# reedrosenbluth/LASS

Hardware: AMD Instinct MI355X
Metric: clips/sec (10s@16kHz) (higher is better)
Workload: dtype f32; 1 GPU; ResUNet30 separate() fp32, batch=16/GPU, 10s@16kHz clips, fixed precomputed condition embedding, seeded random-init weights (BASELINE configs[1]); samples_per_clip=160000, parallelism=clip-sharded x1

## Files before the change

### include/lass_hip.h

```cpp
#ifndef LASS_HIP_H
#define LASS_HIP_H

#include <stddef.h>
#include <stdint.h>

#ifdef __cplusplus
extern "C" {
#endif

typedef struct lass_ctx lass_ctx;

#define LASS_OK 0
#define LASS_ERR_ARG (-1)
#define LASS_ERR_HIP (-2)
#define LASS_ERR_STATE (-3)
#define LASS_ERR_WORKSPACE (-4)

#define LASS_F32 0
#define LASS_I64 1

#define LASS_COMPUTE_F32 0
#define LASS_COMPUTE_BF16 1
#define LASS_COMPUTE_BF16X3 2

int lass_version(void);

int lass_create(lass_ctx** out, int device_id);
int lass_create_multistft(lass_ctx** out, int device_id, int n_fft, int n_windows, const int* win_lengths,
                          int mask_window);
int lass_destroy(lass_ctx* ctx);

const char* lass_last_error(const lass_ctx* ctx);

int lass_set_param(lass_ctx* ctx, const char* name, const void* data, const int64_t* shape, int ndim, int dtype);

int lass_finalize(lass_ctx* ctx, int compute_mode);

int lass_workspace_bytes(const lass_ctx* ctx, int B, int L, size_t* bytes);

int lass_separate(lass_ctx* ctx, const float* mixture, const float* condition, float* out, int B, int L,
                  void* workspace, size_t workspace_bytes, void* stream);

int lass_graph_stats(const lass_ctx* ctx, long* captures, long* replays);
int lass_set_graph_replay(lass_ctx* ctx, int enabled);

int lass_separate_components(lass_ctx* ctx, const float* const* mag, const float* cos_mask, const float* sin_mask,
                             const float* condition, float* out, int B, int L, void* workspace, size_t workspace_bytes,
                             void* stream);


int lass_stft_magphase(lass_ctx* ctx, const float* wav, int B, int L, float* mag, float* cos_out, float* sin_out,
                       float* real_out, float* imag_out, void* stream);

int lass_multi_stft(lass_ctx* ctx, const float* wav, int B, int L, int hop, int n_windows, const int* win_lengths,
                    float* const* mag, float* const* cos_out, float* const* sin_out, void* stream);

int lass_stft_components(lass_ctx* ctx, const float* wav, int B, int L, int n_fft, int hop, int n_windows,
                         const int* win_lengths, float* const* mag, float* const* cos_out, float* const* sin_out,
                         void* stream);

int lass_istft(lass_ctx* ctx, const float* real, const float* imag, int B, int T, int L, float* wav,
               float* frames_ws, void* stream);
int lass_istft_nfft(lass_ctx* ctx, const float* real, const float* imag, int B, int T, int L, int n_fft, int win_length,
                    float* wav, void* stream);

int lass_film(lass_ctx* ctx, const float* condition, int B, float* shift, void* stream);
int lass_film_width(const lass_ctx* ctx);
int lass_film_offset(const lass_ctx* ctx, const char* site);
int lass_film_raw(lass_ctx* ctx, const float* condition, int B, float* film, void* stream);

int lass_convblock(lass_ctx* ctx, const char* prefix, const float* x, int B, int H, int W, const float* shift,
                   float* y, float* scratch, void* stream);

int lass_encoder_block(lass_ctx* ctx, const char* name, const float* x, int B, int H, int W, const float* shift, float* y,
                       float* pool, float* scratch, void* stream);

int lass_front_end(lass_ctx* ctx, const float* wav, int B, int L, float* mag, float* cos_out, float* sin_out, float* x0,
                   void* stream);

int lass_workspace_tensor(const lass_ctx* ctx, int B, int L, const char* name, size_t* offset, int64_t shape[4],
                          int64_t strides[4]);

int lass_upconv(lass_ctx* ctx, const char* name, const float* x, int B, int h, int w, const float* shift, float* y,
                void* stream);

int lass_mask_apply(lass_ctx* ctx, const float* x12, const float* mag, const float* cos_in, const float* sin_in,
                    int B, int T, int Tpad, float* out_real, float* out_imag, void* stream);

int lass_sdr_stats(lass_ctx* ctx, const float* ref, const float* est, int B, int L, double* stats, void* stream);

int lass_mix_at_snr(lass_ctx* ctx, float* source, const float* noise, const float* snr_db, float* mixture, int B, int L,
                    double* scratch, void* stream);

int lass_segment_mix(lass_ctx* ctx, const float* waveforms, int B, int L, const int* mix_num, const float* comp_db, int max_comp,
                     const float* noise_db, float* mixture, float* segment, double* scratch, void* stream);


typedef struct lass_text_ctx lass_text_ctx;

int lass_text_create(lass_text_ctx** out, int device_id);
int lass_text_destroy(lass_text_ctx* ctx);
const char* lass_text_last_error(const lass_text_ctx* ctx);
int lass_text_set_param(lass_text_ctx* ctx, const char* name, const void* data, const int64_t* shape, int ndim);
int lass_text_finalize(lass_text_ctx* ctx);
int lass_text_layers(const lass_text_ctx* ctx);
int lass_text_workspace_bytes(const lass_text_ctx* ctx, int N, int S, size_t* bytes);
int lass_text_encode(lass_text_ctx* ctx, const int64_t* input_ids, const int64_t* attention_mask, int N, int S,
                     float* out, float* pooler_out, void* workspace, size_t workspace_bytes, void* stream);


int lass_set_profiling(lass_ctx* ctx, int enabled);
int lass_profile_count(const lass_ctx* ctx);
int lass_profile_get(lass_ctx* ctx, int i, const char** name, double* ms, int* launches);
int lass_profile_reset(lass_ctx* ctx);

#ifdef __cplusplus
}
#endif
#endif
```

### lass_amd/_lib.py

```python
from __future__ import annotations

import ctypes
import os
from ctypes import POINTER, c_char_p, c_double, c_int, c_int64, c_long, c_size_t, c_void_p

_HERE = os.path.dirname(os.path.abspath(__file__))
LIB_PATH = os.environ.get("LASS_HIP_LIB") or os.path.join(_HERE, "csrc", "liblass_hip.so")

_lib = None

SYMBOLS = [
    ("lass_version", c_int, []),
    ("lass_create", c_int, [POINTER(c_void_p), c_int]),
    ("lass_create_multistft", c_int, [POINTER(c_void_p), c_int, c_int, c_int, POINTER(c_int), c_int]),
    ("lass_destroy", c_int, [c_void_p]),
    ("lass_last_error", c_char_p, [c_void_p]),
    ("lass_set_param", c_int, [c_void_p, c_char_p, c_void_p, POINTER(c_int64), c_int, c_int]),
    ("lass_finalize", c_int, [c_void_p, c_int]),
    ("lass_workspace_bytes", c_int, [c_void_p, c_int, c_int, POINTER(c_size_t)]),
    ("lass_separate", c_int, [c_void_p, c_void_p, c_void_p, c_void_p, c_int, c_int, c_void_p, c_size_t, c_void_p]),
    ("lass_stft_magphase", c_int, [c_void_p, c_void_p, c_int, c_int, c_void_p, c_void_p, c_void_p, c_void_p,
                                   c_void_p, c_void_p]),
    ("lass_mix_at_snr", c_int, [c_void_p, c_void_p, c_void_p, c_void_p, c_void_p, c_int, c_int, c_void_p, c_void_p]),
    ("lass_segment_mix", c_int, [c_void_p, c_void_p, c_int, c_int, c_void_p, c_void_p, c_int, c_void_p, c_void_p, c_void_p,
                                 c_void_p, c_void_p]),
    ("lass_multi_stft", c_int, [c_void_p, c_void_p, c_int, c_int, c_int, c_int, POINTER(c_int), POINTER(c_void_p),
                                POINTER(c_void_p), POINTER(c_void_p), c_void_p]),
    ("lass_graph_stats", c_int, [c_void_p, POINTER(c_long), POINTER(c_long)]),
    ("lass_set_graph_replay", c_int, [c_void_p, c_int]),
    ("lass_separate_components", c_int, [c_void_p, POINTER(c_void_p), c_void_p, c_void_p, c_void_p, c_void_p, c_int,
                                         c_int, c_void_p, c_size_t, c_void_p]),
    ("lass_stft_components", c_int, [c_void_p, c_void_p, c_int, c_int, c_int, c_int, c_int, POINTER(c_int),
                                     POINTER(c_void_p), POINTER(c_void_p), POINTER(c_void_p), c_void_p]),
    ("lass_istft_nfft", c_int, [c_void_p, c_void_p, c_void_p, c_int, c_int, c_int, c_int, c_int, c_void_p, c_void_p]),
    ("lass_istft", c_int, [c_void_p, c_void_p, c_void_p, c_int, c_int, c_int, c_void_p, c_void_p, c_void_p]),
    ("lass_film", c_int, [c_void_p, c_void_p, c_int, c_void_p, c_void_p]),
    ("lass_film_width", c_int, [c_void_p]),
    ("lass_film_offset", c_int, [c_void_p, c_char_p]),
    ("lass_film_raw", c_int, [c_void_p, c_void_p, c_int, c_void_p, c_void_p]),
    ("lass_convblock", c_int, [c_void_p, c_char_p, c_void_p, c_int, c_int, c_int, c_void_p, c_void_p, c_void_p,
                               c_void_p]),
    ("lass_encoder_block", c_int, [c_void_p, c_char_p, c_void_p, c_int, c_int, c_int, c_void_p, c_void_p, c_void_p,
                                   c_void_p, c_void_p]),
    ("lass_front_end", c_int, [c_void_p, c_void_p, c_int, c_int, c_void_p, c_void_p, c_void_p, c_void_p, c_void_p]),
    ("lass_workspace_tensor", c_int, [c_void_p, c_int, c_int, c_char_p, POINTER(c_size_t), POINTER(c_int64),
                                      POINTER(c_int64)]),
    ("lass_upconv", c_int, [c_void_p, c_char_p, c_void_p, c_int, c_int, c_int, c_void_p, c_void_p, c_void_p]),
    ("lass_mask_apply", c_int, [c_void_p, c_void_p, c_void_p, c_void_p, c_void_p, c_int, c_int, c_int, c_void_p,
                                c_void_p, c_void_p]),
    ("lass_sdr_stats", c_int, [c_void_p, c_void_p, c_void_p, c_int, c_int, c_void_p, c_void_p]),
    ("lass_text_create", c_int, [POINTER(c_void_p), c_int]),
    ("lass_text_destroy", c_int, [c_void_p]),
    ("lass_text_last_error", c_char_p, [c_void_p]),
    ("lass_text_set_param", c_int, [c_void_p, c_char_p, c_void_p, POINTER(c_int64), c_int]),
    ("lass_text_finalize", c_int, [c_void_p]),
    ("lass_text_layers", c_int, [c_void_p]),
    ("lass_text_workspace_bytes", c_int, [c_void_p, c_int, c_int, POINTER(c_size_t)]),
    ("lass_text_encode", c_int, [c_void_p, c_void_p, c_void_p, c_int, c_int, c_void_p, c_void_p, c_void_p, c_size_t,
                                 c_void_p]),
    ("lass_set_profiling", c_int, [c_void_p, c_int]),
    ("lass_profile_count", c_int, [c_void_p]),
    ("lass_profile_get", c_int, [c_void_p, c_int, POINTER(c_char_p), POINTER(c_double), POINTER(c_int)]),
    ("lass_profile_reset", c_int, [c_void_p]),
]


class LassError(RuntimeError):
    pass


def load():
    global _lib
    if _lib is not None:
        return _lib
    import torch

    if not os.path.exists(LIB_PATH):
        raise LassError(
            f"{LIB_PATH} is missing - build it with `python -c 'import __graft_entry__ as g; g.build()'` "
            "(hipcc --offload-arch=gfx950).  lass_amd has no CPU fallback.")
    lib = ctypes.CDLL(LIB_PATH, mode=ctypes.RTLD_GLOBAL)
    for name, res, args in SYMBOLS:
        fn = getattr(lib, name)
        fn.restype = res
        fn.argtypes = args
    _lib = lib
    return lib


def check(ctx, rc: int, what: str):
    if rc < 0:
        msg = load().lass_last_error(ctx)
        raise LassError(f"{what} failed ({rc}): {msg.decode() if msg else '?'}")
    return rc
```

### lass_amd/arch.py

```python
from __future__ import annotations

from dataclasses import dataclass
from typing import Dict, List, Tuple

N_FFT = 1024
HOP = 160
N_BINS = N_FFT // 2 + 1
F_CROP = N_BINS - 1
T_DOWN = 32
K_MASK = 3
BN_EPS = 1e-5
LEAKY = 0.01
PRE_CH = 32


@dataclass(frozen=True)
class EncSpec:
    name: str
    cin: int
    cout: int
    down: Tuple[int, int]


@dataclass(frozen=True)
class DecSpec:
    name: str
    cin: int
    cout: int
    up: Tuple[int, int]


ENCODERS: Tuple[EncSpec, ...] = (
    EncSpec("encoder_block1", 32, 32, (2, 2)),
    EncSpec("encoder_block2", 32, 64, (2, 2)),
    EncSpec("encoder_block3", 64, 128, (2, 2)),
    EncSpec("encoder_block4", 128, 256, (2, 2)),
    EncSpec("encoder_block5", 256, 384, (2, 2)),
    EncSpec("encoder_block6", 384, 384, (1, 2)),
    EncSpec("conv_block7a", 384, 384, (1, 1)),
)

DECODERS: Tuple[DecSpec, ...] = (
    DecSpec("decoder_block1", 384, 384, (1, 2)),
    DecSpec("decoder_block2", 384, 384, (2, 2)),
    DecSpec("decoder_block3", 384, 256, (2, 2)),
    DecSpec("decoder_block4", 256, 128, (2, 2)),
    DecSpec("decoder_block5", 128, 64, (2, 2)),
    DecSpec("decoder_block6", 64, 32, (2, 2)),
)


def frames_for(length: int) -> int:
    return 1 + length // HOP


def padded_frames(t: int) -> int:
    return ((t + T_DOWN - 1) // T_DOWN) * T_DOWN


def _bn(prefix: str, c: int) -> List[Tuple[str, Tuple[int, ...], str]]:
    return [
        (prefix + ".weight", (c,), "bn_weight"),
        (prefix + ".bias", (c,), "bn_bias"),
        (prefix + ".running_mean", (c,), "bn_mean"),
        (prefix + ".running_var", (c,), "bn_var"),
        (prefix + ".num_batches_tracked", (), "bn_nbt"),
    ]


def _conv_block_res(prefix: str, cin: int, cout: int):
    out = []
    out += _bn(prefix + ".bn1", cin)
    out += _bn(prefix + ".bn2", cout)
    out.append((prefix + ".conv1.weight", (cout, cin, 3, 3), "conv_w"))
    out.append((prefix + ".conv2.weight", (cout, cout, 3, 3), "conv_w"))
    if cin != cout:
        out.append((prefix + ".shortcut.weight", (cout, cin, 1, 1), "conv_w"))
        out.append((prefix + ".shortcut.bias", (cout,), "bias"))
    return out


def film_sites() -> List[Tuple[str, int, bool]]:
    sites: List[Tuple[str, int, bool]] = []
    for e in ENCODERS:
        sites.append((f"{e.name}->conv_block1->beta1", e.cin, True))
        sites.append((f"{e.name}->conv_block1->beta2", e.cout, True))
    for d in DECODERS:
        sites.append((f"{d.name}->beta1", d.cin, True))
        sites.append((f"{d.name}->beta2", d.cin, False))
        sites.append((f"{d.name}->conv_block2->beta1", 2 * d.cout, True))
        sites.append((f"{d.name}->conv_block2->beta2", d.cout, True))
    return sites


def param_specs(input_channels: int = 1, output_channels: int = 1, condition_size: int = 512):
    specs: List[Tuple[str, Tuple[int, ...], str]] = []
    specs += _bn("base.bn0", N_BINS)
    specs.append(("base.pre_conv.weight", (PRE_CH, input_channels, 1, 1), "conv_w"))
    specs.append(("base.pre_conv.bias", (PRE_CH,), "bias"))
    for e in ENCODERS:
        specs += _conv_block_res(f"base.{e.name}.conv_block1", e.cin, e.cout)
    for d in DECODERS:
        specs.append((f"base.{d.name}.conv1.weight", (d.cin, d.cout, d.up[0], d.up[1]), "tconv_w"))
        specs += _bn(f"base.{d.name}.bn1", d.cin)
        specs += _conv_block_res(f"base.{d.name}.conv_block2", 2 * d.cout, d.cout)
        specs += _bn(f"base.{d.name}.bn2", d.cin)
    specs.append(("base.after_conv.weight", (output_channels * K_MASK, PRE_CH, 1, 1), "conv_w"))
    specs.append(("base.after_conv.bias", (output_channels * K_MASK,), "bias"))
    for name, c, _used in film_sites():
        specs.append((f"film.{name}.weight", (c, condition_size), "linear_w"))
        specs.append((f"film.{name}.bias", (c,), "linear_b"))
    return specs


def conv_layer_table(t_pad: int, f: int = F_CROP) -> List[Dict]:
    rows: List[Dict] = []
    h, w = t_pad, f
    rows.append(dict(name="pre_conv", kind="1x1", cin=1, cout=PRE_CH, h=h, w=w, macs=h * w * PRE_CH))
    skips = []
    for e in ENCODERS:
        rows.append(dict(name=e.name + ".conv1", kind="3x3", cin=e.cin, cout=e.cout, h=h, w=w,
                         macs=h * w * 9 * e.cin * e.cout))
        rows.append(dict(name=e.name + ".conv2", kind="3x3", cin=e.cout, cout=e.cout, h=h, w=w,
                         macs=h * w * 9 * e.cout * e.cout))
        if e.cin != e.cout:
            rows.append(dict(name=e.name + ".shortcut", kind="1x1", cin=e.cin, cout=e.cout, h=h, w=w,
                             macs=h * w * e.cin * e.cout))
        skips.append((h, w))
        h, w = h // e.down[0], w // e.down[1]
    skips.pop()
    for d in DECODERS:
        rows.append(dict(name=d.name + ".up", kind="tconv", cin=d.cin, cout=d.cout, h=h, w=w,
                         macs=h * w * d.cin * d.cout * d.up[0] * d.up[1]))
        h, w = h * d.up[0], w * d.up[1]
        assert (h, w) == skips.pop()
        rows.append(dict(name=d.name + ".conv1", kind="3x3", cin=2 * d.cout, cout=d.cout, h=h, w=w,
                         macs=h * w * 9 * 2 * d.cout * d.cout))
        rows.append(dict(name=d.name + ".conv2", kind="3x3", cin=d.cout, cout=d.cout, h=h, w=w,
                         macs=h * w * 9 * d.cout * d.cout))
        rows.append(dict(name=d.name + ".shortcut", kind="1x1", cin=2 * d.cout, cout=d.cout, h=h, w=w,
                         macs=h * w * 2 * d.cout * d.cout))
    rows.append(dict(name="after_conv", kind="1x1", cin=PRE_CH, cout=K_MASK, h=h, w=w, macs=h * w * PRE_CH * K_MASK))
    return rows


def wino4_routed(rows: List[Dict], min_cin: int = 32) -> set:
    if min_cin <= 0:
        return set()
    with_shortcut = {r["name"].rsplit(".", 1)[0] for r in rows if r["name"].endswith(".shortcut")}
    out = set()
    for r in rows:
        if r["kind"] != "3x3":
            continue
        block, conv = r["name"].rsplit(".", 1)
        geom = r["w"] % 32 == 0 and ((r["w"] % 64 == 0 and r["h"] % 8 == 0) or r["h"] % 16 == 0)
        if not (geom and r["cin"] >= min_cin and r["cin"] % 8 == 0 and r["cout"] % 32 == 0):
            continue
        if conv == "conv1":
            out.add(r["name"])
        if conv == "conv2" and (block in with_shortcut or block.startswith("encoder_block1")):
            out.add(r["name"])
    return out


def conv_macs_per_clip(length: int) -> int:
    return sum(r["macs"] for r in conv_layer_table(padded_frames(frames_for(length))))


def conv3x3_bytes_per_clip(length: int, bytes_per_elem: int = 4) -> int:
    tp = padded_frames(frames_for(length))
    h, w = tp, F_CROP
    elems = 0
    for i, e in enumerate(ENCODERS):
        hw = h * w
        cin_read = 1 if i == 0 else e.cin
        elems += cin_read * hw + e.cout * hw
        elems += e.cout * hw + cin_read * hw + e.cout * hw
        if i < 6:
            elems += e.cout * (h // e.down[0]) * (w // e.down[1])
        h, w = h // e.down[0], w // e.down[1]
    for d in DECODERS:
        h, w = h * d.up[0], w * d.up[1]
        hw = h * w
        elems += 2 * d.cout * hw + d.cout * hw
        elems += d.cout * hw + 2 * d.cout * hw + d.cout * hw
    return elems * bytes_per_elem


MS_N_FFT = 2048
MS_WIN_LENGTHS: Tuple[int, ...] = (256, 512, 2048)
MS_MASK_WINDOW = 512
MS_N_BINS = MS_N_FFT // 2 + 1
MS_F_CROP = MS_N_BINS - 1


def ms_encoders(win_lengths=MS_WIN_LENGTHS) -> Tuple[EncSpec, ...]:
    fused = PRE_CH * len(win_lengths)
    return (EncSpec("encoder_block2", fused, 64, (2, 2)),) + ENCODERS[2:]


def ms_film_sites(win_lengths=MS_WIN_LENGTHS) -> List[Tuple[str, int, bool]]:
    fused = PRE_CH * len(win_lengths)
    sites: List[Tuple[str, int, bool]] = []
    for w in win_lengths:
        sites.append((f"encoder_block1s->{w}->conv_block1->beta1", PRE_CH, True))
        sites.append((f"encoder_block1s->{w}->conv_block1->beta2", PRE_CH, True))
    for e in ms_encoders(win_lengths):
        sites.append((f"{e.name}->conv_block1->beta1", e.cin, True))
        sites.append((f"{e.name}->conv_block1->beta2", e.cout, True))
    for d in DECODERS:
        cat = 2 * d.cout if d.name != "decoder_block6" else d.cout + fused
        sites.append((f"{d.name}->beta1", d.cin, True))
        sites.append((f"{d.name}->beta2", d.cin, False))
        sites.append((f"{d.name}->conv_block2->beta1", cat, True))
        sites.append((f"{d.name}->conv_block2->beta2", d.cout, True))
    return sites


def ms_param_specs(input_channels: int = 1, output_channels: int = 1, condition_size: int = 512,
                   win_lengths=MS_WIN_LENGTHS):
    fused = PRE_CH * len(win_lengths)
    specs: List[Tuple[str, Tuple[int, ...], str]] = []
    specs += _bn("base.bn0", MS_N_BINS)
    for w in win_lengths:
        specs.append((f"base.pre_convs.{w}.weight", (PRE_CH, input_channels, 1, 1), "conv_w"))
        specs.append((f"base.pre_convs.{w}.bias", (PRE_CH,), "bias"))
    for w in win_lengths:
        specs += _conv_block_res(f"base.encoder_block1s.{w}.conv_block1", PRE_CH, PRE_CH)
    for e in ms_encoders(win_lengths):
        specs += _conv_block_res(f"base.{e.name}.conv_block1", e.cin, e.cout)
    for d in DECODERS:
        cat = 2 * d.cout if d.name != "decoder_block6" else d.cout + fused
        specs.append((f"base.{d.name}.conv1.weight", (d.cin, d.cout, d.up[0], d.up[1]), "tconv_w"))
        specs += _bn(f"base.{d.name}.bn1", d.cin)
        specs += _conv_block_res(f"base.{d.name}.conv_block2", cat, d.cout)
        specs += _bn(f"base.{d.name}.bn2", d.cin)
    specs.append(("base.after_conv.weight", (output_channels * K_MASK, PRE_CH, 1, 1), "conv_w"))
    specs.append(("base.after_conv.bias", (output_channels * K_MASK,), "bias"))
    for name, c, _used in ms_film_sites(win_lengths):
        specs.append((f"film.{name}.weight", (c, condition_size), "linear_w"))
        specs.append((f"film.{name}.bias", (c,), "linear_b"))
    return specs


def ms_conv_layer_table(t_pad: int, win_lengths=MS_WIN_LENGTHS) -> List[Dict]:
    fused = PRE_CH * len(win_lengths)
    rows: List[Dict] = []
    h, w = t_pad, MS_F_CROP
    for wl in win_lengths:
        rows.append(dict(name=f"pre_convs.{wl}", kind="1x1", cin=1, cout=PRE_CH, h=h, w=w, macs=h * w * PRE_CH))
        for k in (1, 2):
            rows.append(dict(name=f"encoder_block1s.{wl}.conv{k}", kind="3x3", cin=PRE_CH, cout=PRE_CH, h=h, w=w,
                             macs=h * w * 9 * PRE_CH * PRE_CH))
    skips = [(h, w)]
    h, w = h // 2, w // 2
    for e in ms_encoders(win_lengths):
        rows.append(dict(name=e.name + ".conv1", kind="3x3", cin=e.cin, cout=e.cout, h=h, w=w, macs=h * w * 9 * e.cin * e.cout))
        rows.append(dict(name=e.name + ".conv2", kind="3x3", cin=e.cout, cout=e.cout, h=h, w=w, macs=h * w * 9 * e.cout * e.cout))
        if e.cin != e.cout:
            rows.append(dict(name=e.name + ".shortcut", kind="1x1", cin=e.cin, cout=e.cout, h=h, w=w, macs=h * w * e.cin * e.cout))
        skips.append((h, w))
        h, w = h // e.down[0], w // e.down[1]
    skips.pop()
    for d in DECODERS:
        cat = 2 * d.cout if d.name != "decoder_block6" else d.cout + fused
        rows.append(dict(name=d.name + ".up", kind="tconv", cin=d.cin, cout=d.cout, h=h, w=w,
                         macs=h * w * d.cin * d.cout * d.up[0] * d.up[1]))
        h, w = h * d.up[0], w * d.up[1]
        assert (h, w) == skips.pop()
        rows.append(dict(name=d.name + ".conv1", kind="3x3", cin=cat, cout=d.cout, h=h, w=w, macs=h * w * 9 * cat * d.cout))
        rows.append(dict(name=d.name + ".conv2", kind="3x3", cin=d.cout, cout=d.cout, h=h, w=w, macs=h * w * 9 * d.cout * d.cout))
        rows.append(dict(name=d.name + ".shortcut", kind="1x1", cin=cat, cout=d.cout, h=h, w=w, macs=h * w * cat * d.cout))
    rows.append(dict(name="after_conv", kind="1x1", cin=PRE_CH, cout=K_MASK, h=h, w=w, macs=h * w * PRE_CH * K_MASK))
    return rows
```

### lass_amd/csrc/api.hip

```cpp
#include <hip/hip_runtime.h>

#include <algorithm>
#include <cmath>
#include <cstdio>
#include <cstdlib>
#include <cstring>
#include <map>
#include <string>
#include <vector>

#include "../../include/lass_hip.h"
#include "kernels.h"

namespace {

struct EncSpec { const char* name; int cin, cout, dh, dw; };
struct DecSpec { const char* name; int cin, cout, uh, uw; };
const EncSpec kEnc[7] = {{"encoder_block1", 32, 32, 2, 2},   {"encoder_block2", 32, 64, 2, 2},
                         {"encoder_block3", 64, 128, 2, 2},  {"encoder_block4", 128, 256, 2, 2},
                         {"encoder_block5", 256, 384, 2, 2}, {"encoder_block6", 384, 384, 1, 2},
                         {"conv_block7a", 384, 384, 1, 1}};
const DecSpec kDec[6] = {{"decoder_block1", 384, 384, 1, 2}, {"decoder_block2", 384, 384, 2, 2},
                         {"decoder_block3", 384, 256, 2, 2}, {"decoder_block4", 256, 128, 2, 2},
                         {"decoder_block5", 128, 64, 2, 2},  {"decoder_block6", 64, 32, 2, 2}};
constexpr int kPreCh = 32;
constexpr float kBnEps = 1e-5f;
constexpr int kMaxBranches = LASS_MAX_STFT_WINDOWS;

struct Raw {
    float* d = nullptr;
    std::vector<int64_t> shape;
    size_t n = 0;
};

struct Site {
    std::string film;
    std::string bn;
    int C = 0;
    int off = 0;
};

struct ResBlock {
    std::string prefix;
    int cin = 0, cout = 0;
    int width = 0;
    int s1 = -1, s2 = -1;
    float *w1 = nullptr, *w2 = nullptr, *wsc = nullptr;
    float *u1 = nullptr, *u2 = nullptr, *usc = nullptr;
    float *u1f = nullptr, *u2f = nullptr;
    void *b1 = nullptr, *b2 = nullptr, *bsc16 = nullptr;
    void *b1l = nullptr, *b2l = nullptr, *bscl = nullptr;
    const float* bsc = nullptr;
};

struct ProfEntry {
    const char* name;
    double ms = 0;
    int launches = 0;
};

thread_local std::string g_create_err;

}

struct Geometry {
    int variant = 0;
    int nbr = 1;
    int wins[kMaxBranches] = {1024, 0, 0, 0};
    int nfft = 1024, nbins = 513, fcrop = 512;
    int mask_br = 0;
    int magphase_sem = 0;
};

struct lass_ctx {
    int device = 0;
    std::string err;
    Geometry g;
    EncSpec E[7];
    DecSpec D[6];
    int dec_cat[6] = {0};
    std::string pre_name[kMaxBranches];
    std::map<std::string, Raw> raw;
    bool finalized = false;
    float2* tw2k = nullptr;
    std::vector<Site> sites;
    std::map<std::string, int> site_idx;
    int n_shift = 0;
    float *film_W = nullptr, *film_b = nullptr, *bn_scale = nullptr, *bn_base = nullptr;
    float *bn0_s = nullptr, *bn0_h = nullptr;
    std::vector<ResBlock> enc, dec;
    int dec_site[6] = {0};
    void* up16[6] = {nullptr};
    void* up16l[6] = {nullptr};
    std::vector<void*> owned;
    int compute_mode = LASS_COMPUTE_F32;
    int wino4_mincin = 32;
    bool fuse_catb = true;
    bool fuse_block = true;
    bool fuse_up = true;
    void* up_sc16 = nullptr;
    bool use_graph = true;
    struct GraphKey {
        const void *mix = nullptr, *cond = nullptr, *out = nullptr, *ws = nullptr;
        int B = 0, L = 0;
        unsigned long gen = 0;
        bool operator==(const GraphKey& o) const {
            return mix == o.mix && cond == o.cond && out == o.out && ws == o.ws && B == o.B && L == o.L && gen == o.gen;
        }
    };
    struct GraphEntry {
        GraphKey key;
        hipGraphExec_t exec = nullptr;
        size_t need = 0;
        int seen = 0;
        unsigned long used = 0;
        bool split = false;
    };
    std::map<std::pair<int, int>, bool> last_split;
    static constexpr int kGraphSlots = 4;
    GraphEntry g_slots[kGraphSlots];
    unsigned long g_tick = 0;
    std::vector<hipGraphExec_t> g_retired;
    hipStream_t g_stream = nullptr;
    int split_batch = 1;
    hipStream_t s2 = nullptr;
    hipEvent_t ev_fork = nullptr, ev_join = nullptr;
    unsigned long gen = 0;
    long g_replays = 0, g_captures = 0;
    bool profiling = false;
    std::vector<ProfEntry> prof;
    std::vector<hipEvent_t> ev_pool;
    struct Pending { int cls; hipEvent_t a, b; };
    std::vector<Pending> pending;
    size_t ev_used = 0;
};

namespace {

#define HIP_TRY(ctx, expr)                                                                                     \
    do {                                                                                                       \
        hipError_t _e = (expr);                                                                                \
        if (_e != hipSuccess) {                                                                                \
            (ctx)->err = std::string(#expr) + ": " + hipGetErrorString(_e);                                     \
            return LASS_ERR_HIP;                                                                               \
        }                                                                                                      \
    } while (0)

int fail(lass_ctx* ctx, int code, const std::string& msg) {
    if (ctx) ctx->err = msg;
    return code;
}

bool starts_with(const std::string& s, const char* p) { return s.rfind(p, 0) == 0; }
bool ends_with(const std::string& s, const char* p) {
    const size_t n = strlen(p);
    return s.size() >= n && s.compare(s.size() - n, n, p) == 0;
}

std::string film_to_bn(const std::string& film) {
    std::string s = "base.";
    for (size_t i = 0; i < film.size(); ++i) {
        if (film[i] == '-' && i + 1 < film.size() && film[i + 1] == '>') {
            s += '.';
            ++i;
        } else {
            s += film[i];
        }
    }
    const size_t p = s.rfind("beta");
    s.replace(p, 4, "bn");
    return s;
}

int add_site(lass_ctx* c, const std::string& film, int C) {
    Site s;
    s.film = film;
    s.bn = film_to_bn(film);
    s.C = C;
    s.off = c->n_shift;
    c->n_shift += C;
    c->site_idx[film] = (int)c->sites.size();
    c->sites.push_back(s);
    return (int)c->sites.size() - 1;
}

const ResBlock& trunk_block(const lass_ctx* c, int i) { return c->enc[c->g.nbr - 1 + i]; }

void build_arch(lass_ctx* c) {
    const Geometry& g = c->g;
    c->sites.clear();
    c->site_idx.clear();
    c->n_shift = 0;
    c->enc.clear();
    c->dec.clear();
    for (int i = 0; i < 7; ++i) c->E[i] = kEnc[i];
    for (int i = 0; i < 6; ++i) c->D[i] = kDec[i];
    c->E[1].cin = kPreCh * g.nbr;
    for (int k = 0; k < g.nbr; ++k) {
        ResBlock rb;
        std::string film;
        if (g.variant == 0) {
            rb.prefix = "base.encoder_block1.conv_block1";
            film = "encoder_block1->conv_block1";
            c->pre_name[k] = "base.pre_conv";
        } else {
            const std::string w = std::to_string(g.wins[k]);
            rb.prefix = "base.encoder_block1s." + w + ".conv_block1";
            film = "encoder_block1s->" + w + "->conv_block1";
            c->pre_name[k] = "base.pre_convs." + w;
        }
        rb.cin = rb.cout = kPreCh;
        rb.width = g.fcrop;
        rb.s1 = add_site(c, film + "->beta1", kPreCh);
        rb.s2 = add_site(c, film + "->beta2", kPreCh);
        c->enc.push_back(rb);
    }
    for (int i = 1; i < 7; ++i) {
        const EncSpec& e = c->E[i];
        ResBlock rb;
        rb.prefix = std::string("base.") + e.name + ".conv_block1";
        rb.cin = e.cin;
        rb.cout = e.cout;
        rb.width = g.fcrop >> i;
        rb.s1 = add_site(c, std::string(e.name) + "->conv_block1->beta1", e.cin);
        rb.s2 = add_site(c, std::string(e.name) + "->conv_block1->beta2", e.cout);
        c->enc.push_back(rb);
    }
    for (int i = 0; i < 6; ++i) {
        const auto& d = c->D[i];
        const int e = 5 - i;
        c->dec_cat[i] = d.cout + c->E[e].cout * (e == 0 ? g.nbr : 1);
        c->dec_site[i] = add_site(c, std::string(d.name) + "->beta1", d.cin);
        ResBlock rb;
        rb.prefix = std::string("base.") + d.name + ".conv_block2";
        rb.cin = c->dec_cat[i];
        rb.cout = d.cout;
        rb.width = g.fcrop >> e;
        rb.s1 = add_site(c, std::string(d.name) + "->conv_block2->beta1", rb.cin);
        rb.s2 = add_site(c, std::string(d.name) + "->conv_block2->beta2", d.cout);
        c->dec.push_back(rb);
    }
}

std::vector<int64_t> expected_shape(const lass_ctx* c, const std::string& name) {
    auto bn_field = [](const std::string& n) {
        return ends_with(n, ".weight") || ends_with(n, ".bias") || ends_with(n, ".running_mean") ||
               ends_with(n, ".running_var");
    };
    if (starts_with(name, "base.bn0.") && bn_field(name)) return {c->g.nbins};
    for (int k = 0; k < c->g.nbr; ++k) {
        if (name == c->pre_name[k] + ".weight") return {kPreCh, 1, 1, 1};
        if (name == c->pre_name[k] + ".bias") return {kPreCh};
    }
    if (name == "base.after_conv.weight") return {3, kPreCh, 1, 1};
    if (name == "base.after_conv.bias") return {3};
    auto res_block = [&](const ResBlock& rb) -> std::vector<int64_t> {
        const std::string& p = rb.prefix;
        if (!starts_with(name, (p + ".").c_str())) return {};
        const std::string f = name.substr(p.size() + 1);
        if (starts_with(f, "bn1.") && bn_field(f)) return {rb.cin};
        if (starts_with(f, "bn2.") && bn_field(f)) return {rb.cout};
        if (f == "conv1.weight") return {rb.cout, rb.cin, 3, 3};
        if (f == "conv2.weight") return {rb.cout, rb.cout, 3, 3};
        if (rb.cin != rb.cout && f == "shortcut.weight") return {rb.cout, rb.cin, 1, 1};
        if (rb.cin != rb.cout && f == "shortcut.bias") return {rb.cout};
        return {};
    };
    for (const auto& rb : c->enc) {
        auto s = res_block(rb);
        if (!s.empty()) return s;
    }
    for (int i = 0; i < 6; ++i) {
        auto s = res_block(c->dec[i]);
        if (!s.empty()) return s;
        const DecSpec& d = c->D[i];
        const std::string p = std::string("base.") + d.name;
        if (name == p + ".conv1.weight") return {d.cin, d.cout, d.uh, d.uw};
        if (starts_with(name, (p + ".bn1.").c_str()) && bn_field(name)) return {d.cin};
    }
    if (starts_with(name, "film.")) {
        for (const auto& s : c->sites) {
            if (name == "film." + s.film + ".weight") return {s.C, LASS_COND};
            if (name == "film." + s.film + ".bias") return {s.C};
        }
    }
    return {};
}

bool ignorable(const std::string& name) {
    if (starts_with(name, "base.stft.") || starts_with(name, "base.istft.")) return true;
    if (ends_with(name, "num_batches_tracked")) return true;
    for (const auto& d : kDec) {
        if (starts_with(name, (std::string("base.") + d.name + ".bn2.").c_str())) return true;
        if (starts_with(name, (std::string("film.") + d.name + "->beta2.").c_str())) return true;
    }
    return false;
}

const float* rawp(const lass_ctx* c, const std::string& name) {
    auto it = c->raw.find(name);
    return it == c->raw.end() ? nullptr : it->second.d;
}

template <typename T>
int dev_alloc(lass_ctx* c, T** p, size_t count) {
    void* v = nullptr;
    HIP_TRY(c, hipMalloc(&v, count * sizeof(T)));
    c->owned.push_back(v);
    *p = (T*)v;
    return 0;
}

void free_owned(lass_ctx* c) {
    for (void* p : c->owned) (void)hipFree(p);
    c->owned.clear();
}

enum ProfClass { P_STFT = 0, P_FILM, P_PRECONV, P_CONV3X3, P_TCONV, P_POOL, P_MASK, P_ISTFT, P_COUNT };
const char* kProfNames[P_COUNT] = {"stft_magphase", "film", "pre_conv", "conv3x3_mfma", "tconv_mfma",
                                   "avg_pool",      "mask_apply", "istft"};

constexpr size_t kProfPairs = 512;

struct ProfScope {
    lass_ctx* c;
    hipStream_t s;
    int cls;
    hipEvent_t b = nullptr;
    bool on = false;
    ProfScope(lass_ctx* ctx, hipStream_t st, int k) : c(ctx), s(st), cls(k) {
        if (!c->profiling || c->ev_used + 2 > c->ev_pool.size()) return;
        hipEvent_t a = c->ev_pool[c->ev_used++];
        b = c->ev_pool[c->ev_used++];
        (void)hipEventRecord(a, s);
        c->pending.push_back({cls, a, b});
        on = true;
    }
    ~ProfScope() {
        if (on) (void)hipEventRecord(b, s);
    }
};

void prof_collect(lass_ctx* c) {
    for (auto& p : c->pending) {
        float ms = 0;
        if (hipEventElapsedTime(&ms, p.a, p.b) == hipSuccess) {
            c->prof[p.cls].ms += ms;
            c->prof[p.cls].launches += 1;
        }
    }
    c->pending.clear();
    c->ev_used = 0;
}

struct CatCopies {
    void* act;
    void* raw;
    int noct;
    const float* scale;
    const float* shift;
};

struct MaskHead {
    const float* mag;
    const float* cosv;
    const float* sinv;
    float* oreal;
    float* oimag;
    int T;
    int nbins;
};

struct PreConv {
    const float* x0;
    const float* w;
    const float* b;
};

struct UpFuse {
    const void* x_act;
    int cin, h, w;
    const void* w16;
    const void* wsc16;
};

struct BlockFusions {
    float* pool_out = nullptr;
    int pool_h = 2;
    long pool_bs = 0;
    int cofs = 0;
    const PreConv* pre = nullptr;
    const MaskHead* head = nullptr;
    const CatCopies* skip_out = nullptr;
    const CatCopies* cat_in = nullptr;
    const Site* act_out = nullptr;
    const CatCopies* pool_copies = nullptr;
    const UpFuse* up = nullptr;
};

constexpr int kShortcutGemmMinCin = 256;

int run_resblock(lass_ctx* c, const ResBlock& rb, const float* x, long x_bs, int B, int H, int W, const float* shift,
                 float* a2, float* out, long out_bs, hipStream_t st, const BlockFusions& f = BlockFusions()) {
    const PreConv* pre = f.pre;
    const CatCopies *skip_out = f.skip_out, *cat_in = f.cat_in, *pool_copies = f.pool_copies;
    const float* x0 = pre ? pre->x0 : nullptr;
    const Site& s1 = c->sites[rb.s1];
    const Site& s2 = c->sites[rb.s2];
    const long HW = (long)H * W;
    ConvArgs p;
    p.in = x; p.in_bs = x_bs; p.Cin = rb.cin; p.w = rb.w1; p.Nw = rb.cout; p.N = rb.cout;
    p.pro_scale = c->bn_scale + s1.off; p.pro_shift = shift + s1.off; p.pro_shift_bs = c->n_shift;
    p.epi_scale = c->bn_scale + s2.off; p.epi_shift = shift + s2.off; p.epi_shift_bs = c->n_shift;
    p.out = a2; p.out_bs = rb.cout * HW; p.B = B; p.H = H; p.W = W;
    if (x0) {
        p.in = x0; p.in_bs = HW;
        p.pre_w = pre->w; p.pre_b = pre->b;
    }
    p.w_wino = rb.u1; p.w_wino4 = rb.u1f;
    p.w_bf16 = rb.b1; p.w_bf16_lo = rb.b1l;
    const bool bf1 = c->compute_mode != LASS_COMPUTE_F32 && rb.b1 && rb.b2 && lass_bf16_supported(p) &&
                     (!x0 || W % 32 == 0) && rb.cout % 16 == 0 && (rb.cin == rb.cout || (rb.bsc16 && rb.cin % 16 == 0));
    void* a2_hi = a2;
    void* a2_lo = c->compute_mode == LASS_COMPUTE_BF16X3 ? (void*)((char*)a2 + (size_t)B * rb.cout * HW * 2) : nullptr;
    if (bf1) { p.out_bf16 = a2_hi; p.out_bf16_lo = a2_lo; }
    if ((skip_out || cat_in) && (!bf1 || c->compute_mode != LASS_COMPUTE_BF16))
        return fail(c, LASS_ERR_STATE, "blocked bf16 concat copies need the bf16 kernels");
    if (cat_in) p.in_bf16 = cat_in->act;
    const ConvKind k1 = x0 ? CONV1_ACT_PRE : CONV1_ACT, k2 = x0 ? CONV2_IDENT_PRE : CONV2_IDENT;
    const bool wino1 = !bf1 && rb.u1 && lass_wino_supported(p);
    auto launch_conv1 = [&]() -> int {
        ProfScope ps(c, st, P_CONV3X3);
        if (bf1)
            HIP_TRY(c, lass_launch_conv_bf16(k1, p, st));
        else if (wino1 && rb.u1f && lass_wino4_supported(k1, p))
            HIP_TRY(c, lass_launch_wino4(k1, p, st));
        else if (wino1)
            HIP_TRY(c, lass_launch_wino(k1, p, st));
        else
            HIP_TRY(c, lass_launch_conv(k1, p, st));
        return 0;
    };
    ConvArgs q;
    q.in = a2; q.in_bs = rb.cout * HW; q.Cin = rb.cout; q.w = rb.w2; q.Nw = rb.cout; q.N = rb.cout;
    q.out = out; q.out_bs = out_bs; q.B = B; q.H = H; q.W = W;
    q.pool_out = f.pool_out; q.pool_h = f.pool_h; q.pool_bs = f.pool_bs;
    q.w_wino = rb.u2; q.w2_wino = rb.usc; q.w_wino4 = rb.u2f;
    if (const MaskHead* mh = f.head) {
        q.out = nullptr;
        q.mask_w = rawp(c, "base.after_conv.weight"); q.mask_b = rawp(c, "base.after_conv.bias");
        q.mask_mag = mh->mag; q.mask_cos = mh->cosv; q.mask_sin = mh->sinv;
        q.mask_re = mh->oreal; q.mask_im = mh->oimag; q.mask_T = mh->T; q.mask_nbins = mh->nbins;
    }
    q.w_bf16 = rb.b2; q.w2_bf16 = rb.bsc16; q.w_bf16_lo = rb.b2l; q.w2_bf16_lo = rb.bscl;
    const bool bf2 = bf1;
    if (bf2) { q.in_bf16 = a2_hi; q.in_bf16_lo = a2_lo; }
    if (cat_in) q.in2_bf16 = cat_in->raw;
    if (pool_copies) {
        if (!bf2 || c->compute_mode != LASS_COMPUTE_BF16 || !f.pool_out || f.pool_h != 2)
            return fail(c, LASS_ERR_STATE, "blocked bf16 pooled copies need the bf16 kernels and the fused 2x2 pool");
        q.pool_out = nullptr;
        q.pool_bf16 = pool_copies->raw; q.pool_bf16_act = pool_copies->act;
        q.pool_oct0 = f.cofs / 8; q.pool_noct = pool_copies->noct;
        q.pool_act_scale = pool_copies->scale + f.cofs; q.pool_act_shift = pool_copies->shift + f.cofs; q.act_shift_bs = c->n_shift;
    }
    if (const Site* act_out = f.act_out) {
        if (!bf2 || c->compute_mode != LASS_COMPUTE_BF16) return fail(c, LASS_ERR_STATE, "activated bf16 output needs the bf16 kernels");
        q.out_bf16 = out; q.out = nullptr; q.out_oct0 = 0; q.out_noct = 0;
        q.epi_scale = c->bn_scale + act_out->off; q.epi_shift = shift + act_out->off; q.epi_shift_bs = c->n_shift;
    }
    if (skip_out) {
        q.out = nullptr;
        q.out_bf16 = skip_out->raw; q.out_bf16_act = skip_out->act;
        q.out_oct0 = (rb.cout + f.cofs) / 8; q.out_noct = skip_out->noct;
        q.act_scale = skip_out->scale + rb.cout + f.cofs; q.act_shift = skip_out->shift + rb.cout + f.cofs; q.act_shift_bs = c->n_shift;
    }
    const bool wino2 = !bf2 && rb.u2 && lass_wino_supported(q);
    if (rb.cin == rb.cout) {
        q.res = x; q.res_bs = x_bs;
        if (x0) {
            q.res = x0; q.res_bs = HW;
            q.pre_w = pre->w; q.pre_b = pre->b;
        }
    }
    if (bf2 && x0 && c->fuse_block && c->compute_mode == LASS_COMPUTE_BF16 && skip_out && rb.cin == rb.cout &&
        lass_enc1_fused_bf16_supported(p, q)) {
        ProfScope ps(c, st, P_CONV3X3);
        HIP_TRY(c, lass_launch_enc1_fused_bf16(p, q, st));
        return 0;
    }
    if (rb.cin != rb.cout) { q.in2 = x; q.in2_bs = x_bs; q.Cin2 = rb.cin; q.w2 = rb.wsc; q.bias = rb.bsc; }
    if (const UpFuse* up = f.up) {
        ConvArgs uq;
        uq.in_bf16 = up->x_act; uq.Cin = up->cin; uq.H = up->h; uq.W = up->w; uq.B = B;
        uq.w_bf16 = up->w16; uq.w2_bf16 = up->wsc16;
        if (!(bf2 && !x0 && c->fuse_block && c->compute_mode == LASS_COMPUTE_BF16 && cat_in && f.head && rb.cin != rb.cout &&
              lass_dec6u_fused_bf16_supported(p, q, uq)))
            return fail(c, LASS_ERR_STATE, "decoder_block6 with its transposed conv inside needs the fused bf16 kernel");
        ProfScope ps(c, st, P_CONV3X3);
        HIP_TRY(c, lass_launch_dec6u_fused_bf16(p, q, uq, st));
        return 0;
    }
    if (bf2 && !x0 && c->fuse_block && c->compute_mode == LASS_COMPUTE_BF16 && cat_in && f.head && rb.cin != rb.cout &&
        lass_dec6_fused_bf16_supported(p, q)) {
        ProfScope ps(c, st, P_CONV3X3);
        HIP_TRY(c, lass_launch_dec6_fused_bf16(p, q, st));
        return 0;
    }
    const bool sc_gemm = c->compute_mode == LASS_COMPUTE_F32 && !bf2 && rb.cin != rb.cout && !f.head && rb.cin >= kShortcutGemmMinCin &&
                         wino2 && rb.u2f && lass_wino4_supported(CONV2_SHORTCUT, q) && lass_pw_gemm_supported(CONV2_SHORTCUT, q);
    if (sc_gemm) {
        const auto overlaps = [&](const float* a, long a_bs, long a_n, const float* b, long b_bs, long b_n) {
            return a < b + (size_t)(B - 1) * b_bs + b_n && b < a + (size_t)(B - 1) * a_bs + a_n;
        };
        if (overlaps(out, out_bs, rb.cout * HW, x, x_bs, rb.cin * HW) || overlaps(out, out_bs, rb.cout * HW, a2, rb.cout * HW, rb.cout * HW))
            return fail(c, LASS_ERR_STATE, "a block's output must not overlap its input or its intermediate");
        ProfScope ps(c, st, P_CONV3X3);
        HIP_TRY(c, lass_launch_pw_gemm(CONV2_SHORTCUT, q, st));
    }
    if (int r1 = launch_conv1()) return r1;
    ProfScope ps(c, st, P_CONV3X3);
    if (sc_gemm) {
        ConvArgs r = q;
        r.in2 = nullptr; r.in2_bs = 0; r.Cin2 = 0; r.w2 = nullptr; r.bias = nullptr;
        r.res = out; r.res_bs = out_bs;
        if (!lass_wino4_supported(CONV2_IDENT, r)) return fail(c, LASS_ERR_STATE, "conv2 with the shortcut as residual");
        HIP_TRY(c, lass_launch_wino4(CONV2_IDENT, r, st));
    } else if (rb.cin == rb.cout) {
        if (bf2)
            HIP_TRY(c, lass_launch_conv_bf16(k2, q, st));
        else if (wino2 && x0 && rb.u2f && lass_wino4_supported(k2, q))
            HIP_TRY(c, lass_launch_wino4(k2, q, st));
        else if (wino2)
            HIP_TRY(c, lass_launch_wino(k2, q, st));
        else
            HIP_TRY(c, lass_launch_conv(k2, q, st));
    } else {
        if (bf2)
            HIP_TRY(c, lass_launch_conv_bf16(CONV2_SHORTCUT, q, st));
        else if (wino2 && rb.u2f && lass_wino4_supported(CONV2_SHORTCUT, q))
            HIP_TRY(c, lass_launch_wino4(CONV2_SHORTCUT, q, st));
        else if (wino2)
            HIP_TRY(c, lass_launch_wino(CONV2_SHORTCUT, q, st));
        else
            HIP_TRY(c, lass_launch_conv(CONV2_SHORTCUT, q, st));
    }
    return 0;
}

constexpr int kTconvGemmMinCin = 128;

int run_upconv(lass_ctx* c, int di, const float* x, int B, int h, int w, const float* shift, float* out, long out_bs,
               hipStream_t st, const CatCopies* cb = nullptr, bool x_is_act_bf16 = false) {
    const DecSpec& d = c->D[di];
    const Site& s = c->sites[c->dec_site[di]];
    ConvArgs p;
    p.in = x; p.in_bs = (long)d.cin * h * w; p.Cin = d.cin;
    p.w = rawp(c, std::string("base.") + d.name + ".conv1.weight");
    p.N = p.Nw = d.cout * d.uh * d.uw;
    p.pro_scale = c->bn_scale + s.off; p.pro_shift = shift + s.off; p.pro_shift_bs = c->n_shift;
    p.out = out; p.out_bs = out_bs; p.B = B; p.H = h; p.W = w; p.up_h = d.uh;
    p.w_bf16 = c->up16[di]; p.w_bf16_lo = c->up16l[di];
    if (x_is_act_bf16) {
        if (c->compute_mode != LASS_COMPUTE_BF16 || !p.w_bf16 || !lass_bf16_supported(p))
            return fail(c, LASS_ERR_STATE, "activated bf16 input needs the bf16 kernels");
        p.in_bf16 = x;
    }
    if (cb) {
        if (c->compute_mode != LASS_COMPUTE_BF16 || !p.w_bf16 || !lass_bf16_supported(p))
            return fail(c, LASS_ERR_STATE, "blocked bf16 concat copies need the bf16 kernels");
        p.out = nullptr;
        p.out_bf16 = cb->raw; p.out_bf16_act = cb->act; p.out_oct0 = 0; p.out_noct = cb->noct;
        p.act_scale = cb->scale; p.act_shift = cb->shift; p.act_shift_bs = c->n_shift;
    }
    ProfScope ps(c, st, P_TCONV);
    if (c->compute_mode != LASS_COMPUTE_F32 && p.w_bf16 && lass_bf16_supported(p))
        HIP_TRY(c, lass_launch_conv_bf16(TCONV_ACT, p, st));
    else if (c->compute_mode == LASS_COMPUTE_F32 && d.cin >= kTconvGemmMinCin && lass_pw_gemm_supported(TCONV_ACT, p))
        HIP_TRY(c, lass_launch_pw_gemm(TCONV_ACT, p, st));
    else
        HIP_TRY(c, lass_launch_conv(TCONV_ACT, p, st));
    return 0;
}

struct Plan {
    int B, L, T, Tp;
    size_t total = 0;
    size_t mag, cosv, sinv, x0[kMaxBranches], shift, a2, cat[6], pool[6], center, decout[6], oreal, oimag;
    int eh[7], ew[7];
};

size_t bump(size_t& total, size_t floats) {
    const size_t off = total;
    total += (floats * sizeof(float) + 255) / 256 * 256;
    return off;
}

int make_plan(const lass_ctx* c, int B, int L, Plan* pl) {
    const Geometry& g = c->g;
    if (B <= 0 || L <= g.nfft / 2) return LASS_ERR_ARG;
    pl->B = B; pl->L = L;
    pl->T = 1 + L / LASS_HOP;
    pl->Tp = (pl->T + 31) / 32 * 32;
    const size_t clip_max = (size_t)c->dec_cat[5] * pl->Tp * g.fcrop * sizeof(float);
    if (clip_max > 0xFFFF0000ull) return LASS_ERR_ARG;
    size_t& t = pl->total;
    t = 0;
    const size_t spec = (size_t)B * pl->T * g.nbins;
    pl->mag = bump(t, spec); pl->cosv = bump(t, spec); pl->sinv = bump(t, spec);
    for (int k = 0; k < g.nbr; ++k) pl->x0[k] = bump(t, (size_t)B * pl->Tp * g.fcrop);
    pl->shift = bump(t, (size_t)B * c->n_shift);
    int h = pl->Tp, w = g.fcrop;
    size_t a2max = 0;
    for (int i = 0; i < 7; ++i) {
        pl->eh[i] = h; pl->ew[i] = w;
        const size_t o = (size_t)B * c->E[i].cout * h * w;
        if (o > a2max) a2max = o;
        h /= c->E[i].dh; w /= c->E[i].dw;
        if (i < 6) pl->pool[i] = bump(t, (size_t)B * c->E[i].cout * (i == 0 ? g.nbr : 1) * h * w);
    }
    pl->center = bump(t, (size_t)B * c->E[6].cout * pl->eh[6] * pl->ew[6]);
    for (int d = 0; d < 6; ++d) {
        const int e = 5 - d;
        const size_t hw = (size_t)pl->eh[e] * pl->ew[e];
        pl->cat[d] = bump(t, (size_t)B * c->dec_cat[d] * hw);
        pl->decout[d] = bump(t, (size_t)B * c->D[d].cout * hw);
    }
    pl->a2 = bump(t, a2max);
    pl->oreal = bump(t, spec); pl->oimag = bump(t, spec);
    return 0;
}

int use_device(lass_ctx* c) {
    if (!c) return LASS_ERR_ARG;
    HIP_TRY(c, hipSetDevice(c->device));
    return 0;
}

int check_ready(lass_ctx* c) {
    if (!c) return LASS_ERR_ARG;
    if (!c->finalized) return fail(c, LASS_ERR_STATE, "lass_finalize has not been called (or a parameter changed since)");
    return use_device(c);
}

void drop_graphs(lass_ctx* c) {
    for (auto& e : c->g_slots) {
        if (e.exec) (void)hipGraphExecDestroy(e.exec);
        e = lass_ctx::GraphEntry();
    }
    for (hipGraphExec_t x : c->g_retired) (void)hipGraphExecDestroy(x);
    c->g_retired.clear();
}

bool split_halves(const lass_ctx* c, int B) { return c->split_batch > 0 && !c->profiling && B >= 8 && (B % 2) == 0; }

const ResBlock* find_block(const lass_ctx* c, const std::string& prefix) {
    for (const auto& rb : c->enc) if (rb.prefix == prefix) return &rb;
    for (const auto& rb : c->dec) if (rb.prefix == prefix) return &rb;
    return nullptr;
}

}

extern "C" {

int lass_version(void) { return 10300; }

const char* lass_last_error(const lass_ctx* ctx) { return ctx ? ctx->err.c_str() : g_create_err.c_str(); }

static int create_impl(lass_ctx** out, int device_id, const Geometry& geom) {
    if (!out) return LASS_ERR_ARG;
    *out = nullptr;
    int ndev = 0;
    hipError_t e = hipGetDeviceCount(&ndev);
    if (e != hipSuccess || ndev <= 0) {
        g_create_err = std::string("no HIP device available: ") + hipGetErrorString(e) +
                       " (liblass_hip has no CPU fallback)";
        return LASS_ERR_HIP;
    }
    if (device_id < 0 || device_id >= ndev) {
        g_create_err = "device_id out of range";
        return LASS_ERR_ARG;
    }
    hipDeviceProp_t prop;
    e = hipGetDeviceProperties(&prop, device_id);
    if (e != hipSuccess) {
        g_create_err = std::string("hipGetDeviceProperties: ") + hipGetErrorString(e);
        return LASS_ERR_HIP;
    }
    if (std::string(prop.gcnArchName).rfind("gfx950", 0) != 0) {
        g_create_err = std::string("device is ") + prop.gcnArchName + "; liblass_hip is built for gfx950 only";
        return LASS_ERR_HIP;
    }
    lass_ctx* c = new lass_ctx();
    c->device = device_id;
    c->g = geom;
    if (const char* e = getenv("LASS_FUSE_CATB")) c->fuse_catb = atoi(e) != 0;
    if (const char* e = getenv("LASS_FUSE_BLOCK")) c->fuse_block = atoi(e) != 0;
    if (const char* e = getenv("LASS_FUSE_UP")) c->fuse_up = atoi(e) != 0;
    if (const char* e = getenv("LASS_WINO4")) c->wino4_mincin = atoi(e);
    if (const char* e = getenv("LASS_SPLIT")) c->split_batch = std::max(0, std::min(2, atoi(e)));
    if (const char* e = getenv("LASS_GRAPH")) c->use_graph = atoi(e) != 0;
    c->prof.resize(P_COUNT);
    for (int i = 0; i < P_COUNT; ++i) c->prof[i].name = kProfNames[i];
    build_arch(c);
    if (hipSetDevice(device_id) != hipSuccess) {
        g_create_err = "hipSetDevice failed";
        delete c;
        return LASS_ERR_HIP;
    }
    std::vector<float2> tw2k(2048);
    for (int k = 0; k < 2048; ++k) {
        const double a = 2.0 * M_PI * k / 2048.0;
        tw2k[k] = make_float2((float)std::cos(a), (float)std::sin(a));
    }
    if (hipMalloc((void**)&c->tw2k, sizeof(float2) * 2048) != hipSuccess ||
        hipMemcpy(c->tw2k, tw2k.data(), sizeof(float2) * 2048, hipMemcpyHostToDevice) != hipSuccess) {
        g_create_err = "allocating FFT tables failed";
        delete c;
        return LASS_ERR_HIP;
    }
    *out = c;
    return 0;
}

int lass_create(lass_ctx** out, int device_id) { return create_impl(out, device_id, Geometry()); }

int lass_create_multistft(lass_ctx** out, int device_id, int n_fft, int n_windows, const int* win_lengths,
                          int mask_window) {
    if (!out) return LASS_ERR_ARG;
    *out = nullptr;
    Geometry g;
    g.variant = 1;
    g.magphase_sem = 1;
    if (n_fft != 2048 || n_windows < 1 || n_windows > kMaxBranches || !win_lengths) {
        g_create_err = "lass_create_multistft: n_fft must be 2048 and 1 <= n_windows <= 4";
        return LASS_ERR_ARG;
    }
    g.nfft = n_fft; g.nbins = n_fft / 2 + 1; g.fcrop = n_fft / 2; g.nbr = n_windows; g.mask_br = -1;
    for (int k = 0; k < n_windows; ++k) {
        const int w = win_lengths[k];
        if (w < 32 || w > n_fft || (2048 % w) != 0) {
            g_create_err = "lass_create_multistft: window lengths must be powers of two in [32, n_fft]";
            return LASS_ERR_ARG;
        }
        for (int j = 0; j < k; ++j)
            if (g.wins[j] == w) {
                g_create_err = "lass_create_multistft: duplicate window length";
                return LASS_ERR_ARG;
            }
        g.wins[k] = w;
        if (w == mask_window) g.mask_br = k;
    }
    if (g.mask_br < 0) {
        g_create_err = "lass_create_multistft: mask_window is not one of the analysis windows";
        return LASS_ERR_ARG;
    }
    return create_impl(out, device_id, g);
}

int lass_destroy(lass_ctx* c) {
    if (!c) return LASS_ERR_ARG;
    (void)hipSetDevice(c->device);
    free_owned(c);
    for (auto& kv : c->raw) (void)hipFree(kv.second.d);
    for (auto e : c->ev_pool) (void)hipEventDestroy(e);
    (void)hipDeviceSynchronize();
    drop_graphs(c);
    if (c->g_stream) (void)hipStreamDestroy(c->g_stream);
    if (c->s2) (void)hipStreamDestroy(c->s2);
    if (c->ev_join) (void)hipEventDestroy(c->ev_join);
    if (c->ev_fork) (void)hipEventDestroy(c->ev_fork);
    (void)hipFree(c->tw2k);
    delete c;
    return 0;
}

int lass_set_param(lass_ctx* c, const char* name_c, const void* data, const int64_t* shape, int ndim, int dtype) {
    if (!c || !name_c || !data || ndim < 0 || (ndim > 0 && !shape)) return fail(c, LASS_ERR_ARG, "bad argument");
    const std::string name(name_c);
    std::vector<int64_t> want = expected_shape(c, name);
    if (want.empty()) {
        if (ignorable(name)) return 1;
        return fail(c, LASS_ERR_ARG, "unknown parameter '" + name + "'");
    }
    if (dtype != LASS_F32) return fail(c, LASS_ERR_ARG, "parameter '" + name + "' must be float32");
    std::vector<int64_t> got(shape, shape + ndim);
    if (got != want) {
        std::string m = "shape mismatch for '" + name + "': got (";
        for (auto v : got) m += std::to_string(v) + ",";
        m += ") want (";
        for (auto v : want) m += std::to_string(v) + ",";
        return fail(c, LASS_ERR_ARG, m + ")");
    }
    size_t n = 1;
    for (auto v : want) n *= (size_t)v;
    HIP_TRY(c, hipSetDevice(c->device));
    Raw& r = c->raw[name];
    if (!r.d) HIP_TRY(c, hipMalloc((void**)&r.d, n * sizeof(float)));
    r.shape = want;
    r.n = n;
    HIP_TRY(c, hipMemcpy(r.d, data, n * sizeof(float), hipMemcpyDefault));
    c->finalized = false;
    return 0;
}

int lass_finalize(lass_ctx* c, int compute_mode) {
    if (!c) return LASS_ERR_ARG;
    if (compute_mode != LASS_COMPUTE_F32 && compute_mode != LASS_COMPUTE_BF16 && compute_mode != LASS_COMPUTE_BF16X3)
        return fail(c, LASS_ERR_ARG, "unsupported compute mode");
    c->last_split.clear();
    c->compute_mode = compute_mode;
    HIP_TRY(c, hipSetDevice(c->device));
    HIP_TRY(c, hipDeviceSynchronize());
    drop_graphs(c);
    free_owned(c);
    c->finalized = false;
    hipStream_t st = nullptr;
    auto need = [&](const std::string& n) -> const float* {
        const float* p = rawp(c, n);
        if (!p && c->err.empty()) c->err = "missing parameter '" + n + "'";
        return p;
    };
    c->err.clear();
    if (dev_alloc(c, &c->bn_scale, c->n_shift) || dev_alloc(c, &c->bn_base, c->n_shift) ||
        dev_alloc(c, &c->film_W, (size_t)c->n_shift * LASS_COND) || dev_alloc(c, &c->film_b, c->n_shift) ||
        dev_alloc(c, &c->bn0_s, c->g.nbins) || dev_alloc(c, &c->bn0_h, c->g.nbins))
        return LASS_ERR_HIP;
    for (const auto& s : c->sites) {
        const float *g = need(s.bn + ".weight"), *b = need(s.bn + ".bias"), *m = need(s.bn + ".running_mean"),
                    *v = need(s.bn + ".running_var"), *fw = need("film." + s.film + ".weight"),
                    *fb = need("film." + s.film + ".bias");
        if (!g || !b || !m || !v || !fw || !fb) return LASS_ERR_STATE;
        HIP_TRY(c, lass_launch_bnfold(g, b, m, v, s.C, kBnEps, c->bn_scale + s.off, c->bn_base + s.off, st));
        HIP_TRY(c, hipMemcpyAsync(c->film_W + (size_t)s.off * LASS_COND, fw, (size_t)s.C * LASS_COND * sizeof(float),
                                  hipMemcpyDeviceToDevice, st));
        HIP_TRY(c, hipMemcpyAsync(c->film_b + s.off, fb, s.C * sizeof(float), hipMemcpyDeviceToDevice, st));
    }
    {
        const float *g = need("base.bn0.weight"), *b = need("base.bn0.bias"), *m = need("base.bn0.running_mean"),
                    *v = need("base.bn0.running_var");
        if (!g || !b || !m || !v) return LASS_ERR_STATE;
        HIP_TRY(c, lass_launch_bnfold(g, b, m, v, c->g.nbins, kBnEps, c->bn0_s, c->bn0_h, st));
    }
    for (int k = 0; k < c->g.nbr; ++k)
        if (!need(c->pre_name[k] + ".weight") || !need(c->pre_name[k] + ".bias")) return LASS_ERR_STATE;
    if (!need("base.after_conv.weight") || !need("base.after_conv.bias")) return LASS_ERR_STATE;
    auto prep = [&](ResBlock& rb) -> int {
        const float *w1 = need(rb.prefix + ".conv1.weight"), *w2 = need(rb.prefix + ".conv2.weight");
        if (!w1 || !w2) return LASS_ERR_STATE;
        if (dev_alloc(c, &rb.w1, (size_t)rb.cout * rb.cin * 9) || dev_alloc(c, &rb.w2, (size_t)rb.cout * rb.cout * 9))
            return LASS_ERR_HIP;
        HIP_TRY(c, lass_launch_relayout_conv(w1, rb.cout, rb.cin, 9, rb.w1, st));
        HIP_TRY(c, lass_launch_relayout_conv(w2, rb.cout, rb.cout, 9, rb.w2, st));
        rb.u1 = rb.u2 = rb.usc = nullptr;
        rb.u1f = rb.u2f = nullptr;
        rb.b1 = rb.b2 = rb.bsc16 = rb.b1l = rb.b2l = rb.bscl = nullptr;
        const bool bfm = c->compute_mode == LASS_COMPUTE_BF16 || c->compute_mode == LASS_COMPUTE_BF16X3;
        const bool split = c->compute_mode == LASS_COMPUTE_BF16X3;
        if (bfm && rb.cin % 16 == 0 && rb.cout % 16 == 0) {
            unsigned short *t1 = nullptr, *t2 = nullptr;
            if (dev_alloc(c, &t1, (size_t)rb.cout * rb.cin * 9) || dev_alloc(c, &t2, (size_t)rb.cout * rb.cout * 9))
                return LASS_ERR_HIP;
            HIP_TRY(c, lass_launch_weights_bf16(w1, rb.cout, rb.cin, 9, t1, 0, 0, st));
            HIP_TRY(c, lass_launch_weights_bf16(w2, rb.cout, rb.cout, 9, t2, 0, 0, st));
            rb.b1 = t1; rb.b2 = t2;
            if (split) {
                unsigned short *l1 = nullptr, *l2 = nullptr;
                if (dev_alloc(c, &l1, (size_t)rb.cout * rb.cin * 9) || dev_alloc(c, &l2, (size_t)rb.cout * rb.cout * 9))
                    return LASS_ERR_HIP;
                HIP_TRY(c, lass_launch_weights_bf16(w1, rb.cout, rb.cin, 9, l1, 1, 0, st));
                HIP_TRY(c, lass_launch_weights_bf16(w2, rb.cout, rb.cout, 9, l2, 1, 0, st));
                rb.b1l = l1; rb.b2l = l2;
            }
        }
        if (c->compute_mode == LASS_COMPUTE_F32) {
            if (dev_alloc(c, &rb.u1, (size_t)16 * rb.cout * rb.cin) || dev_alloc(c, &rb.u2, (size_t)16 * rb.cout * rb.cout))
                return LASS_ERR_HIP;
            HIP_TRY(c, lass_launch_wino_weights(w1, rb.cout, rb.cin, rb.u1, st));
            HIP_TRY(c, lass_launch_wino_weights(w2, rb.cout, rb.cout, rb.u2, st));
            const bool w4_level = rb.width % 32 == 0;
            if (w4_level && c->wino4_mincin > 0 && rb.cin >= c->wino4_mincin && rb.cin % 8 == 0 && rb.cout % 32 == 0) {
                if (dev_alloc(c, &rb.u1f, (size_t)36 * rb.cout * rb.cin)) return LASS_ERR_HIP;
                HIP_TRY(c, lass_launch_wino4_weights(w1, rb.cout, rb.cin, rb.u1f, st));
            }
            if (w4_level && c->wino4_mincin > 0 && rb.cout >= c->wino4_mincin && (rb.cin != rb.cout || rb.cout == kPreCh) && rb.cout % 32 == 0 &&
                rb.cin % 8 == 0) {
                if (dev_alloc(c, &rb.u2f, (size_t)36 * rb.cout * rb.cout)) return LASS_ERR_HIP;
                HIP_TRY(c, lass_launch_wino4_weights(w2, rb.cout, rb.cout, rb.u2f, st));
            }
        }
        rb.wsc = nullptr;
        rb.bsc = nullptr;
        if (rb.cin != rb.cout) {
            const float *ws = need(rb.prefix + ".shortcut.weight"), *bs = need(rb.prefix + ".shortcut.bias");
            if (!ws || !bs) return LASS_ERR_STATE;
            if (dev_alloc(c, &rb.wsc, (size_t)rb.cout * rb.cin)) return LASS_ERR_HIP;
            HIP_TRY(c, lass_launch_relayout_conv(ws, rb.cout, rb.cin, 1, rb.wsc, st));
            rb.bsc = bs;
            if (bfm && rb.b1) {
                unsigned short* t3 = nullptr;
                if (dev_alloc(c, &t3, (size_t)rb.cout * rb.cin)) return LASS_ERR_HIP;
                HIP_TRY(c, lass_launch_weights_bf16(ws, rb.cout, rb.cin, 1, t3, 0, 0, st));
                rb.bsc16 = t3;
                if (split) {
                    unsigned short* l3 = nullptr;
                    if (dev_alloc(c, &l3, (size_t)rb.cout * rb.cin)) return LASS_ERR_HIP;
                    HIP_TRY(c, lass_launch_weights_bf16(ws, rb.cout, rb.cin, 1, l3, 1, 0, st));
                    rb.bscl = l3;
                }
            }
            if (c->compute_mode == LASS_COMPUTE_F32) {
                if (dev_alloc(c, &rb.usc, (size_t)4 * rb.cout * rb.cin)) return LASS_ERR_HIP;
                HIP_TRY(c, lass_launch_wino_shortcut_weights(ws, rb.cout, rb.cin, rb.usc, st));
            }
        }
        return 0;
    };
    for (auto& rb : c->enc) { int r = prep(rb); if (r) return r; }
    for (auto& rb : c->dec) { int r = prep(rb); if (r) return r; }
    for (int i = 0; i < 6; ++i) {
        const auto& d = c->D[i];
        const float* wu = need(std::string("base.") + d.name + ".conv1.weight");
        if (!wu) return LASS_ERR_STATE;
        c->up16[i] = c->up16l[i] = nullptr;
        if (c->compute_mode != LASS_COMPUTE_F32 && d.cin % 16 == 0) {
            const int N = d.cout * d.uh * d.uw;
            unsigned short *t = nullptr, *l = nullptr;
            if (dev_alloc(c, &t, (size_t)N * d.cin)) return LASS_ERR_HIP;
            HIP_TRY(c, lass_launch_weights_bf16(wu, N, d.cin, 1, t, 0, 1, st));
            c->up16[i] = t;
            if (c->compute_mode == LASS_COMPUTE_BF16X3) {
                if (dev_alloc(c, &l, (size_t)N * d.cin)) return LASS_ERR_HIP;
                HIP_TRY(c, lass_launch_weights_bf16(wu, N, d.cin, 1, l, 1, 1, st));
                c->up16l[i] = l;
            }
        }
    }
    c->up_sc16 = nullptr;
    {
        const DecSpec& d = c->D[5];
        const ResBlock& rb = c->dec[5];
        if (c->compute_mode == LASS_COMPUTE_BF16 && c->g.variant == 0 && d.cin == 64 && d.cout == 32 && d.uh == 2 && d.uw == 2 &&
            rb.cin == 64 && rb.cout == 32 && c->up16[5]) {
            const float* wu = need(std::string("base.") + d.name + ".conv1.weight");
            const float* ws = need(rb.prefix + ".shortcut.weight");
            if (!wu || !ws) return LASS_ERR_STATE;
            float* tmp = nullptr;
            unsigned short* t16 = nullptr;
            if (dev_alloc(c, &tmp, (size_t)4 * rb.cout * d.cin) || dev_alloc(c, &t16, (size_t)4 * rb.cout * d.cin)) return LASS_ERR_HIP;
            HIP_TRY(c, lass_launch_compose_up_shortcut(ws, wu, d.cin, d.cout, rb.cin, rb.cout, tmp, st));
            HIP_TRY(c, lass_launch_weights_bf16(tmp, 4 * rb.cout, d.cin, 1, t16, 0, 0, st));
            c->up_sc16 = t16;
        }
    }
    HIP_TRY(c, hipStreamSynchronize(st));
    c->finalized = true;
    ++c->gen;
    return 0;
}

int lass_workspace_bytes(const lass_ctx* c, int B, int L, size_t* bytes) {
    if (!c || !bytes) return LASS_ERR_ARG;
    Plan pl;
    if (make_plan(c, B, L, &pl)) return LASS_ERR_ARG;
    *bytes = pl.total;
    if (split_halves(c, B)) {
        Plan ph;
        if (make_plan(c, B / 2, L, &ph)) return LASS_ERR_ARG;
        const size_t both = 2 * ((ph.total + 255) / 256 * 256);
        if (both > *bytes) *bytes = both;
    }
    return 0;
}

int lass_film_width(const lass_ctx* c) { return c ? c->n_shift : LASS_ERR_ARG; }

int lass_film_offset(const lass_ctx* c, const char* site) {
    if (!c || !site) return -1;
    auto it = c->site_idx.find(site);
    return it == c->site_idx.end() ? -1 : c->sites[it->second].off;
}

int lass_film(lass_ctx* c, const float* cond, int B, float* shift, void* stream) {
    int r = check_ready(c);
    if (r) return r;
    if (!cond || !shift || B <= 0) return fail(c, LASS_ERR_ARG, "lass_film: bad argument");
    HIP_TRY(c, lass_launch_film(cond, B, c->film_W, c->film_b, c->bn_base, c->n_shift, shift, (hipStream_t)stream));
    return 0;
}

int lass_film_raw(lass_ctx* c, const float* cond, int B, float* film, void* stream) {
    int r = check_ready(c);
    if (r) return r;
    if (!cond || !film || B <= 0) return fail(c, LASS_ERR_ARG, "lass_film_raw: bad argument");
    HIP_TRY(c, lass_launch_film(cond, B, c->film_W, c->film_b, nullptr, c->n_shift, film, (hipStream_t)stream));
    return 0;
}

int lass_stft_magphase(lass_ctx* c, const float* wav, int B, int L, float* mag, float* cos_out, float* sin_out,
                       float* real_out, float* imag_out, void* stream) {
    if (!c || !wav || B <= 0 || L <= LASS_NFFT / 2) return fail(c, LASS_ERR_ARG, "lass_stft_magphase: bad argument");
    if (int r = use_device(c)) return r;
    const int T = 1 + L / LASS_HOP;
    StftBranch br;
    br.wlen = LASS_NFFT; br.mag = mag; br.cosv = cos_out; br.sinv = sin_out; br.real = real_out; br.imag = imag_out;
    HIP_TRY(c, lass_launch_stft2(wav, B, L, LASS_NFFT, LASS_HOP, T, T, 1, &br, 0, nullptr, nullptr, c->tw2k,
                                 (hipStream_t)stream));
    return 0;
}

int lass_stft_components(lass_ctx* c, const float* wav, int B, int L, int n_fft, int hop, int n_windows,
                         const int* win_lengths, float* const* mag, float* const* cos_out, float* const* sin_out,
                         void* stream) {
    if (!c || !wav || !win_lengths || !mag || !cos_out || !sin_out || B <= 0 || hop <= 0 || n_windows <= 0 ||
        n_windows > LASS_MAX_STFT_WINDOWS || (n_fft != 1024 && n_fft != 2048) || L <= n_fft / 2)
        return fail(c, LASS_ERR_ARG, "lass_stft_components: bad argument (n_fft 1024 or 2048, at most 4 windows, L > n_fft/2)");
    StftBranch br[LASS_MAX_STFT_WINDOWS];
    for (int i = 0; i < n_windows; ++i) {
        const int w = win_lengths[i];
        if (w < 32 || w > n_fft || (2048 % w) != 0)
            return fail(c, LASS_ERR_ARG, "lass_stft_components: window lengths must be powers of two in [32, n_fft]");
        if (!mag[i] || !cos_out[i] || !sin_out[i]) return fail(c, LASS_ERR_ARG, "lass_stft_components: null output");
        br[i].wlen = w; br[i].mag = mag[i]; br[i].cosv = cos_out[i]; br[i].sinv = sin_out[i];
    }
    if (int r = use_device(c)) return r;
    const int T = 1 + L / hop;
    HIP_TRY(c, lass_launch_stft2(wav, B, L, n_fft, hop, T, T, n_windows, br, 1, nullptr, nullptr, c->tw2k,
                                 (hipStream_t)stream));
    return 0;
}

int lass_multi_stft(lass_ctx* c, const float* wav, int B, int L, int hop, int n_windows, const int* win_lengths,
                    float* const* mag, float* const* cos_out, float* const* sin_out, void* stream) {
    if (!c || !wav || !win_lengths || !mag || !cos_out || !sin_out || B <= 0 || hop <= 0 || n_windows <= 0 ||
        n_windows > LASS_MAX_STFT_WINDOWS)
        return fail(c, LASS_ERR_ARG, "lass_multi_stft: bad argument");
    for (int i = 0; i < n_windows; ++i) {
        const int N = win_lengths[i];
        if (N != 256 && N != 512 && N != 1024 && N != 2048)
            return fail(c, LASS_ERR_ARG, "lass_multi_stft: window lengths must be 256, 512, 1024 or 2048");
        if (L <= N / 2) return fail(c, LASS_ERR_ARG, "lass_multi_stft: waveform shorter than the reflect padding");
        if (!mag[i] || !cos_out[i] || !sin_out[i]) return fail(c, LASS_ERR_ARG, "lass_multi_stft: null output");
    }
    if (int r = use_device(c)) return r;
    HIP_TRY(c, lass_launch_multi_stft(wav, B, L, hop, n_windows, win_lengths, c->tw2k, mag, cos_out, sin_out,
                                      (hipStream_t)stream));
    return 0;
}

int lass_istft(lass_ctx* c, const float* real, const float* imag, int B, int T, int L, float* wav, float* frames_ws,
               void* stream) {
    (void)frames_ws;
    return lass_istft_nfft(c, real, imag, B, T, L, LASS_NFFT, LASS_NFFT, wav, stream);
}

int lass_istft_nfft(lass_ctx* c, const float* real, const float* imag, int B, int T, int L, int n_fft, int win_length,
                    float* wav, void* stream) {
    if (!c || !real || !imag || !wav || B <= 0 || T <= 0 || L <= 0 || (n_fft != 1024 && n_fft != 2048) ||
        win_length < 32 || win_length > n_fft || (2048 % win_length) != 0 ||
        (long)L + n_fft / 2 > (long)(T - 1) * LASS_HOP + n_fft)
        return fail(c, LASS_ERR_ARG, "lass_istft: bad argument");
    if (int r = use_device(c)) return r;
    HIP_TRY(c, lass_launch_istft2(real, imag, B, T, L, n_fft, win_length, LASS_HOP, c->tw2k, wav, (hipStream_t)stream));
    return 0;
}

int lass_convblock(lass_ctx* c, const char* prefix, const float* x, int B, int H, int W, const float* shift, float* y,
                   float* scratch, void* stream) {
    int r = check_ready(c);
    if (r) return r;
    if (!prefix || !x || !shift || !y || !scratch) return fail(c, LASS_ERR_ARG, "lass_convblock: bad argument");
    const ResBlock* rb = find_block(c, prefix);
    if (!rb) return fail(c, LASS_ERR_ARG, std::string("lass_convblock: unknown block '") + prefix + "'");
    const long HW = (long)H * W;
    return run_resblock(c, *rb, x, rb->cin * HW, B, H, W, shift, scratch, y, rb->cout * HW, (hipStream_t)stream);
}

int lass_encoder_block(lass_ctx* c, const char* name, const float* x, int B, int H, int W, const float* shift, float* y,
                       float* pool, float* scratch, void* stream) {
    int r = check_ready(c);
    if (r) return r;
    if (!name || !x || !shift || !y || !scratch || B <= 0 || H <= 0 || W <= 0)
        return fail(c, LASS_ERR_ARG, "lass_encoder_block: bad argument");
    for (size_t bi = 0; bi < c->enc.size(); ++bi) {
        const ResBlock& rb = c->enc[bi];
        if (rb.prefix != std::string(name) + ".conv_block1") continue;
        const EncSpec& e = c->E[bi < (size_t)c->g.nbr ? 0 : bi - c->g.nbr + 1];
        const long HW = (long)H * W;
        const bool pooled = e.dw == 2;
        if (pooled && (!pool || W % 2 != 0)) return fail(c, LASS_ERR_ARG, "lass_encoder_block: pool output needed, W even");
        const bool fuse = pooled && (H % e.dh) == 0;
        hipStream_t st = (hipStream_t)stream;
        BlockFusions f;
        if (fuse) { f.pool_out = pool; f.pool_h = e.dh; }
        r = run_resblock(c, rb, x, rb.cin * HW, B, H, W, shift, scratch, y, rb.cout * HW, st, f);
        if (r) return r;
        if (pooled && !fuse) HIP_TRY(c, lass_launch_pool(y, rb.cout * HW, B, rb.cout, H, W, e.dh, e.dw, pool, st));
        return 0;
    }
    return fail(c, LASS_ERR_ARG, std::string("lass_encoder_block: unknown encoder '") + name + "'");
}

int lass_front_end(lass_ctx* c, const float* wav, int B, int L, float* mag, float* cos_out, float* sin_out, float* x0,
                   void* stream) {
    int r = check_ready(c);
    if (r) return r;
    const Geometry& g = c->g;
    if (!wav || !x0 || B <= 0 || L <= g.nfft / 2) return fail(c, LASS_ERR_ARG, "lass_front_end: bad argument");
    const int T = 1 + L / LASS_HOP, Tp = (T + 31) / 32 * 32;
    StftBranch br[kMaxBranches];
    for (int k = 0; k < g.nbr; ++k) {
        br[k].wlen = g.wins[k];
        br[k].x0 = x0 + (size_t)k * B * Tp * g.fcrop;
        if (k == g.mask_br) { br[k].mag = mag; br[k].cosv = cos_out; br[k].sinv = sin_out; }
    }
    HIP_TRY(c, lass_launch_stft2(wav, B, L, g.nfft, LASS_HOP, T, Tp, g.nbr, br, g.magphase_sem, c->bn0_s, c->bn0_h,
                                 c->tw2k, (hipStream_t)stream));
    return 0;
}

int lass_workspace_tensor(const lass_ctx* c, int B, int L, const char* name_c, size_t* offset, int64_t shape[4],
                          int64_t strides[4]) {
    if (!c || !name_c || !offset || !shape || !strides) return LASS_ERR_ARG;
    if (auto it = c->last_split.find({B, L}); it != c->last_split.end() && it->second) return LASS_ERR_STATE;
    Plan pl;
    if (make_plan(c, B, L, &pl)) return LASS_ERR_ARG;
    const Geometry& g = c->g;
    const std::string name(name_c);
    auto put = [&](size_t off, int64_t C, int64_t H, int64_t W, int64_t bs) {
        *offset = off;
        shape[0] = B; shape[1] = C; shape[2] = H; shape[3] = W;
        strides[0] = bs; strides[1] = H * W; strides[2] = W; strides[3] = 1;
        return 0;
    };
    const int64_t spec = (int64_t)pl.T * g.nbins;
    if (name == "mag") return put(pl.mag, 1, pl.T, g.nbins, spec);
    if (name == "cos") return put(pl.cosv, 1, pl.T, g.nbins, spec);
    if (name == "sin") return put(pl.sinv, 1, pl.T, g.nbins, spec);
    if (name == "out_real") return put(pl.oreal, 1, pl.T, g.nbins, spec);
    if (name == "out_imag") return put(pl.oimag, 1, pl.T, g.nbins, spec);
    for (int k = 0; k < g.nbr; ++k)
        if (name == (g.variant == 0 ? std::string("x0") : "x0." + std::to_string(g.wins[k])))
            return put(pl.x0[k], 1, pl.Tp, g.fcrop, (int64_t)pl.Tp * g.fcrop);
    for (int i = 0; i < 7; ++i) {
        const EncSpec& e = c->E[i];
        const int64_t H = pl.eh[i], W = pl.ew[i];
        const int64_t C = (int64_t)e.cout * (i == 0 ? g.nbr : 1);
        if (name == e.name) {
            if (i == 6) return put(pl.center, C, H, W, C * H * W);
            const int d = 5 - i;
            return put(pl.cat[d] + (size_t)c->D[d].cout * H * W * sizeof(float), C, H, W, (int64_t)c->dec_cat[d] * H * W);
        }
        if (i < 6 && name == std::string(e.name) + ".pool")
            return put(pl.pool[i], C, H / e.dh, W / e.dw, C * (H / e.dh) * (W / e.dw));
    }
    for (int d = 0; d < 6; ++d) {
        const int64_t H = pl.eh[5 - d], W = pl.ew[5 - d], C = c->D[d].cout;
        if (name == std::string(c->D[d].name) + ".up") return put(pl.cat[d], C, H, W, (int64_t)c->dec_cat[d] * H * W);
        if (name == c->D[d].name) return put(pl.decout[d], C, H, W, C * H * W);
    }
    return LASS_ERR_ARG;
}

int lass_upconv(lass_ctx* c, const char* name, const float* x, int B, int h, int w, const float* shift, float* y,
                void* stream) {
    int r = check_ready(c);
    if (r) return r;
    if (!name || !x || !shift || !y) return fail(c, LASS_ERR_ARG, "lass_upconv: bad argument");
    for (int i = 0; i < 6; ++i)
        if (std::string("base.") + c->D[i].name == name)
            return run_upconv(c, i, x, B, h, w, shift, y, (long)c->D[i].cout * h * c->D[i].uh * w * c->D[i].uw,
                              (hipStream_t)stream);
    return fail(c, LASS_ERR_ARG, std::string("lass_upconv: unknown decoder '") + name + "'");
}

int lass_mask_apply(lass_ctx* c, const float* x12, const float* mag, const float* cos_in, const float* sin_in, int B,
                    int T, int Tpad, float* out_real, float* out_imag, void* stream) {
    int r = check_ready(c);
    if (r) return r;
    if (!x12 || !mag || !cos_in || !sin_in || !out_real || !out_imag)
        return fail(c, LASS_ERR_ARG, "lass_mask_apply: bad argument");
    HIP_TRY(c, lass_launch_mask(x12, rawp(c, "base.after_conv.weight"), rawp(c, "base.after_conv.bias"), mag, cos_in,
                                sin_in, B, T, Tpad, c->g.fcrop, out_real, out_imag, (hipStream_t)stream));
    return 0;
}

int lass_sdr_stats(lass_ctx* c, const float* ref, const float* est, int B, int L, double* stats, void* stream) {
    if (!c || !ref || !est || !stats || B <= 0 || L <= 0) return fail(c, LASS_ERR_ARG, "lass_sdr_stats: bad argument");
    if (int r = use_device(c)) return r;
    HIP_TRY(c, lass_launch_sdr(ref, est, B, L, stats, (hipStream_t)stream));
    return 0;
}

int lass_mix_at_snr(lass_ctx* c, float* source, const float* noise, const float* snr_db, float* mixture, int B, int L,
                    double* scratch, void* stream) {
    if (!c || !source || !noise || !snr_db || !mixture || !scratch || B <= 0 || L <= 0)
        return fail(c, LASS_ERR_ARG, "lass_mix_at_snr: bad argument");
    if (int r = use_device(c)) return r;
    HIP_TRY(c, lass_launch_mix_at_snr(source, noise, snr_db, mixture, B, L, scratch, (hipStream_t)stream));
    return 0;
}

int lass_segment_mix(lass_ctx* c, const float* waveforms, int B, int L, const int* mix_num, const float* comp_db, int max_comp,
                     const float* noise_db, float* mixture, float* segment, double* scratch, void* stream) {
    if (!c || !waveforms || !mix_num || !comp_db || !noise_db || !mixture || !segment || !scratch || B <= 0 || L <= 0)
        return fail(c, LASS_ERR_ARG, "lass_segment_mix: bad argument");
    if (max_comp < 1 || max_comp > 7) return fail(c, LASS_ERR_ARG, "lass_segment_mix: max_comp (max_mix_num - 1) must be 1 ... 7");
    if (mixture == waveforms || segment == waveforms || mixture == segment)
        return fail(c, LASS_ERR_ARG, "lass_segment_mix: waveforms, mixture and segment must be three different buffers");
    if (int r = use_device(c)) return r;
    HIP_TRY(c, lass_launch_segment_mix(waveforms, B, L, mix_num, comp_db, max_comp, noise_db, mixture, segment, scratch,
                                       (hipStream_t)stream));
    return 0;
}

struct Components {
    const float* mag[kMaxBranches];
    const float* cosv;
    const float* sinv;
};

static int separate_impl(lass_ctx* c, const float* mixture, const Components* comp, const float* condition, float* out,
                         int B, int L, void* workspace, size_t workspace_bytes, void* stream, const char* who) {
    int r = check_ready(c);
    if (r) return r;
    const Geometry& g = c->g;
    if ((!mixture && !comp) || !condition || !out || !workspace) return fail(c, LASS_ERR_ARG, std::string(who) + ": null pointer");
    Plan pl;
    if (make_plan(c, B, L, &pl))
        return fail(c, LASS_ERR_ARG, std::string(who) + ": need B >= 1 and " + std::to_string(g.nfft / 2) +
                                         " < L, with decoder_block6's concat (" + std::to_string(c->dec_cat[5]) +
                                         " ch x frames x " + std::to_string(g.fcrop) +
                                         " bins, f32) below 4 GiB per clip (longer clips: ResUNet30.chunk_inference)");
    if (workspace_bytes < pl.total)
        return fail(c, LASS_ERR_WORKSPACE, "workspace too small: need " + std::to_string(pl.total) + " bytes");
    if (((uintptr_t)workspace & 255) != 0) return fail(c, LASS_ERR_ARG, "workspace must be 256-byte aligned");
    hipStream_t st = (hipStream_t)stream;
    char* ws = (char*)workspace;
    auto F = [&](size_t off) { return (float*)(ws + off); };
    const int T = pl.T, Tp = pl.Tp, nbr = g.nbr;
    float* shift = F(pl.shift);
    const float *mag_m = F(pl.mag), *cos_m = F(pl.cosv), *sin_m = F(pl.sinv);
    if (mixture) {
        ProfScope ps(c, st, P_STFT);
        StftBranch br[kMaxBranches];
        for (int k = 0; k < nbr; ++k) {
            br[k].wlen = g.wins[k];
            br[k].x0 = F(pl.x0[k]);
            if (k == g.mask_br) { br[k].mag = F(pl.mag); br[k].cosv = F(pl.cosv); br[k].sinv = F(pl.sinv); }
        }
        HIP_TRY(c, lass_launch_stft2(mixture, B, L, g.nfft, LASS_HOP, T, Tp, nbr, br, g.magphase_sem, c->bn0_s, c->bn0_h,
                                     c->tw2k, st));
    } else {
        ProfScope ps(c, st, P_STFT);
        for (int k = 0; k < nbr; ++k) {
            if (!comp->mag[k]) return fail(c, LASS_ERR_ARG, std::string(who) + ": null magnitude");
            HIP_TRY(c, lass_launch_x0_from_mag(comp->mag[k], B, T, Tp, g.fcrop, c->bn0_s, c->bn0_h, F(pl.x0[k]), st));
        }
        if (!comp->cosv || !comp->sinv) return fail(c, LASS_ERR_ARG, std::string(who) + ": null phase");
        mag_m = comp->mag[g.mask_br]; cos_m = comp->cosv; sin_m = comp->sinv;
    }
    {
        ProfScope ps(c, st, P_FILM);
        HIP_TRY(c, lass_launch_film(condition, B, c->film_W, c->film_b, c->bn_base, c->n_shift, shift, st));
    }
    CatCopies cb[6];
    bool use_cb[6] = {false, false, false, false, false, false};
    for (int d = 1; d < 6; ++d) {
        const int e = 5 - d;
        const ResBlock& rd = c->dec[d];
        const ResBlock& re = c->enc[nbr - 1 + e];
        const long hw = (long)pl.eh[e] * pl.ew[e];
        use_cb[d] = c->fuse_catb && c->compute_mode == LASS_COMPUTE_BF16 && c->D[d].uh == 2 && c->D[d].uw == 2 &&
                    rd.cout % 16 == 0 && rd.b1 && rd.b2 && rd.bsc16 && c->up16[d] && re.b1 && re.b2;
        cb[d].act = F(pl.cat[d]);
        cb[d].raw = (char*)F(pl.cat[d]) + (size_t)B * rd.cin * hw * 2;
        cb[d].noct = rd.cin / 8;
        cb[d].scale = c->bn_scale + c->sites[rd.s1].off;
        cb[d].shift = shift + c->sites[rd.s1].off;
    }
    CatCopies pc[4];
    bool use_pc[4] = {false, false, false, false};
    for (int i = 0; i < 4; ++i) {
        const ResBlock& nx = c->enc[nbr - 1 + i + 1];
        const long hwo = (long)pl.eh[i + 1] * pl.ew[i + 1];
        use_pc[i] = c->fuse_catb && c->compute_mode == LASS_COMPUTE_BF16 && c->E[i].dh == 2 && pl.ew[i] % 32 == 0 &&
                    use_cb[5 - i] && use_cb[5 - (i + 1)] && nx.cin != nx.cout && nx.cin % 16 == 0 && nx.b1 && nx.b2 && nx.bsc16;
        pc[i].act = F(pl.pool[i]);
        pc[i].raw = (char*)F(pl.pool[i]) + (size_t)B * nx.cin * hwo * 2;
        pc[i].noct = nx.cin / 8;
        pc[i].scale = c->bn_scale + c->sites[nx.s1].off;
        pc[i].shift = shift + c->sites[nx.s1].off;
    }
    const float* x = nullptr;
    for (int i = 0; i < 7; ++i) {
        const int H = pl.eh[i], W = pl.ew[i];
        const long HW = (long)H * W;
        const EncSpec& e = c->E[i];
        const int nb = i == 0 ? nbr : 1;
        float* o = nullptr;
        long o_bs = 0;
        for (int k = 0; k < nb; ++k) {
            const ResBlock& rb = c->enc[i == 0 ? k : nbr - 1 + i];
            BlockFusions f;
            f.cofs = k * e.cout;
            if (i < 6) {
                const int d = 5 - i;
                o = F(pl.cat[d]) + (size_t)(c->D[d].cout + f.cofs) * HW;
                o_bs = (long)c->dec_cat[d] * HW;
                const long Ho = H / e.dh, Wo = W / e.dw;
                f.pool_out = F(pl.pool[i]) + (size_t)f.cofs * Ho * Wo;
                f.pool_h = e.dh;
                f.pool_bs = (long)e.cout * nb * Ho * Wo;
            } else {
                o = F(pl.center);
                o_bs = rb.cout * HW;
            }
            PreConv pre{};
            if (i == 0) {
                pre = PreConv{F(pl.x0[k]), rawp(c, c->pre_name[k] + ".weight"), rawp(c, c->pre_name[k] + ".bias")};
                f.pre = &pre;
            }
            if (i < 5 && use_cb[5 - i]) f.skip_out = &cb[5 - i];
            if (i >= 1 && i <= 4 && use_pc[i - 1]) f.cat_in = &pc[i - 1];
            if (i < 4 && use_pc[i]) f.pool_copies = &pc[i];
            r = run_resblock(c, rb, x, rb.cin * HW, B, H, W, shift, F(pl.a2), o, o_bs, st, f);
            if (r) return r;
        }
        x = i < 6 ? F(pl.pool[i]) : o;
    }
    bool x_act = false;
    for (int d = 0; d < 6; ++d) {
        const int e = 5 - d;
        const int H = pl.eh[e], W = pl.ew[e];
        const long HW = (long)H * W;
        const int h = H / c->D[d].uh, w = W / c->D[d].uw;
        const ResBlock& rb = c->dec[d];
        BlockFusions f;
        const UpFuse upf{x, c->D[d].cin, h, w, c->up16[d], c->up_sc16};
        const bool fuse_up = d == 5 && c->fuse_up && c->fuse_block && use_cb[d] && x_act && c->up_sc16 &&
                             c->compute_mode == LASS_COMPUTE_BF16 && rb.cout == 32 && rb.cin == 64 && W == g.fcrop && W % 32 == 0 &&
                             H % 2 == 0 && (unsigned long long)H * W * 8ull < 0x10000000ull;
        if (fuse_up) {
            f.up = &upf;
        } else {
            r = run_upconv(c, d, x, B, h, w, shift, F(pl.cat[d]), rb.cin * HW, st, use_cb[d] ? &cb[d] : nullptr, x_act);
            if (r) return r;
        }
        x_act = d < 5 && c->fuse_catb && c->compute_mode == LASS_COMPUTE_BF16 && rb.b1 && rb.b2 && rb.bsc16 &&
                rb.cout % 16 == 0 && c->up16[d + 1];
        if (x_act) f.act_out = &c->sites[c->dec_site[d + 1]];
        if (use_cb[d]) f.cat_in = &cb[d];
        const MaskHead head{mag_m, cos_m, sin_m, F(pl.oreal), F(pl.oimag), T, g.nbins};
        if (d == 5) f.head = &head;
        r = run_resblock(c, rb, F(pl.cat[d]), rb.cin * HW, B, H, W, shift, F(pl.a2), F(pl.decout[d]), rb.cout * HW, st, f);
        if (r) return r;
        x = F(pl.decout[d]);
    }
    {
        ProfScope ps(c, st, P_ISTFT);
        HIP_TRY(c, lass_launch_istft2(F(pl.oreal), F(pl.oimag), B, T, L, g.nfft, g.wins[g.mask_br], LASS_HOP, c->tw2k, out, st));
    }
    return 0;
}

static int separate_any(lass_ctx* c, const float* mixture, const float* condition, float* out, int B, int L, void* workspace,
                        size_t workspace_bytes, hipStream_t stream, bool capturing) {
    Plan ph;
    if (!c->finalized || !split_halves(c, B) || !mixture || !condition || !out || !workspace || (!capturing && c->split_batch < 2) ||
        make_plan(c, B / 2, L, &ph) || 2 * ((ph.total + 255) / 256 * 256) > workspace_bytes) {
        c->last_split[{B, L}] = false;
        return separate_impl(c, mixture, nullptr, condition, out, B, L, workspace, workspace_bytes, stream, "lass_separate");
    }
    c->last_split[{B, L}] = true;
    HIP_TRY(c, hipSetDevice(c->device));
    if (!c->ev_fork) HIP_TRY(c, hipEventCreateWithFlags(&c->ev_fork, hipEventDisableTiming));
    if (!c->s2) {
        HIP_TRY(c, hipStreamCreateWithFlags(&c->s2, hipStreamNonBlocking));
        HIP_TRY(c, hipEventCreateWithFlags(&c->ev_join, hipEventDisableTiming));
    }
    const int h = B / 2;
    const size_t half_ws = (ph.total + 255) / 256 * 256;
    HIP_TRY(c, hipEventRecord(c->ev_fork, stream));
    HIP_TRY(c, hipStreamWaitEvent(c->s2, c->ev_fork, 0));
    int r = separate_impl(c, mixture, nullptr, condition, out, h, L, workspace, half_ws, stream, "lass_separate");
    const int r2 = separate_impl(c, mixture + (size_t)h * L, nullptr, condition + (size_t)h * LASS_COND, out + (size_t)h * L, h, L,
                                 (char*)workspace + half_ws, half_ws, c->s2, "lass_separate");
    if (!r) r = r2;
    HIP_TRY(c, hipEventRecord(c->ev_join, c->s2));
    HIP_TRY(c, hipStreamWaitEvent(stream, c->ev_join, 0));
    return r;
}

int lass_separate(lass_ctx* c, const float* mixture, const float* condition, float* out, int B, int L, void* workspace,
                  size_t workspace_bytes, void* stream) {
    if (!c) return LASS_ERR_ARG;
    if (!mixture) return fail(c, LASS_ERR_ARG, "lass_separate: null pointer");
    lass_ctx::GraphKey key;
    key.mix = mixture; key.cond = condition; key.out = out; key.ws = workspace; key.B = B; key.L = L; key.gen = c->gen;
    if (c->use_graph && !c->profiling && c->finalized) {
        ++c->g_tick;
        lass_ctx::GraphEntry* slot = nullptr;
        for (auto& e : c->g_slots)
            if (e.seen > 0 && e.key == key) slot = &e;
        if (!slot) {
            for (auto& e : c->g_slots)
                if (!slot || (!e.exec && slot->exec) || (!e.exec == !slot->exec && e.used < slot->used)) slot = &e;
            if (slot->exec) {
                c->g_retired.push_back(slot->exec);
                if (c->g_retired.size() > 8) {
                    HIP_TRY(c, hipSetDevice(c->device));
                    HIP_TRY(c, hipDeviceSynchronize());
                    for (hipGraphExec_t x : c->g_retired) (void)hipGraphExecDestroy(x);
                    c->g_retired.clear();
                }
            }
            *slot = lass_ctx::GraphEntry();
            slot->key = key;
        }
        slot->used = c->g_tick;
        ++slot->seen;
        if (slot->exec) {
            if (workspace_bytes < slot->need)
                return fail(c, LASS_ERR_WORKSPACE, "workspace too small: need " + std::to_string(slot->need) + " bytes");
            HIP_TRY(c, hipSetDevice(c->device));
            HIP_TRY(c, hipGraphLaunch(slot->exec, (hipStream_t)stream));
            ++c->g_replays;
            c->last_split[{B, L}] = slot->split;
            return 0;
        }
        if (slot->seen >= 3) {
            {
                int r0 = check_ready(c);
                if (r0) return r0;
                Plan pl0;
                if (!condition || !out || !workspace || make_plan(c, B, L, &pl0) || workspace_bytes < pl0.total ||
                    ((uintptr_t)workspace & 255) != 0)
                    return separate_any(c, mixture, condition, out, B, L, workspace, workspace_bytes, (hipStream_t)stream, false);
                slot->need = pl0.total;
                if (split_halves(c, B)) {
                    Plan ph0;
                    if (!make_plan(c, B / 2, L, &ph0) && 2 * ((ph0.total + 255) / 256 * 256) <= workspace_bytes)
                        slot->need = std::max(slot->need, 2 * ((ph0.total + 255) / 256 * 256));
                }
            }
            HIP_TRY(c, hipSetDevice(c->device));
            if (!c->g_stream) HIP_TRY(c, hipStreamCreateWithFlags(&c->g_stream, hipStreamNonBlocking));
            bool ok = false;
            if (hipStreamBeginCapture(c->g_stream, hipStreamCaptureModeThreadLocal) == hipSuccess) {
                const int r = separate_any(c, mixture, condition, out, B, L, workspace, workspace_bytes, c->g_stream, true);
                hipGraph_t graph = nullptr;
                const hipError_t e = hipStreamEndCapture(c->g_stream, &graph);
                if (r == 0 && e == hipSuccess && graph && hipGraphInstantiate(&slot->exec, graph, nullptr, nullptr, 0) == hipSuccess) {
                    ok = true;
                    if (auto it = c->last_split.find({B, L}); it != c->last_split.end()) slot->split = it->second;
                } else {
                    slot->exec = nullptr;
                }
                if (graph) (void)hipGraphDestroy(graph);
            }
            if (ok) {
                ++c->g_captures;
                HIP_TRY(c, hipGraphLaunch(slot->exec, (hipStream_t)stream));
                return 0;
            }
            (void)hipGetLastError();
            c->use_graph = false;
            c->err.clear();
        }
    }
    return separate_any(c, mixture, condition, out, B, L, workspace, workspace_bytes, (hipStream_t)stream, false);
}

int lass_set_graph_replay(lass_ctx* c, int enabled) {
    if (!c) return LASS_ERR_ARG;
    c->use_graph = enabled != 0;
    return 0;
}

int lass_graph_stats(const lass_ctx* c, long* captures, long* replays) {
    if (!c) return LASS_ERR_ARG;
    if (captures) *captures = c->g_captures;
    if (replays) *replays = c->g_replays;
    return c->use_graph ? 1 : 0;
}

int lass_separate_components(lass_ctx* c, const float* const* mag, const float* cos_mask, const float* sin_mask,
                             const float* condition, float* out, int B, int L, void* workspace, size_t workspace_bytes,
                             void* stream) {
    if (!c) return LASS_ERR_ARG;
    if (!mag || !cos_mask || !sin_mask) return fail(c, LASS_ERR_ARG, "lass_separate_components: null pointer");
    Components comp;
    for (int k = 0; k < kMaxBranches; ++k) comp.mag[k] = k < c->g.nbr ? mag[k] : nullptr;
    comp.cosv = cos_mask; comp.sinv = sin_mask;
    return separate_impl(c, nullptr, &comp, condition, out, B, L, workspace, workspace_bytes, stream,
                         "lass_separate_components");
}

int lass_set_profiling(lass_ctx* c, int enabled) {
    if (!c) return LASS_ERR_ARG;
    if (enabled && c->ev_pool.size() < 2 * kProfPairs) {
        HIP_TRY(c, hipSetDevice(c->device));
        c->pending.reserve(kProfPairs);
        while (c->ev_pool.size() < 2 * kProfPairs) {
            hipEvent_t e;
            HIP_TRY(c, hipEventCreate(&e));
            c->ev_pool.push_back(e);
        }
    }
    c->profiling = enabled != 0;
    return 0;
}
int lass_profile_count(const lass_ctx* c) { return c ? P_COUNT : LASS_ERR_ARG; }
int lass_profile_get(lass_ctx* c, int i, const char** name, double* ms, int* launches) {
    if (!c || i < 0 || i >= P_COUNT) return LASS_ERR_ARG;
    prof_collect(c);
    if (name) *name = c->prof[i].name;
    if (ms) *ms = c->prof[i].ms;
    if (launches) *launches = c->prof[i].launches;
    return 0;
}
int lass_profile_reset(lass_ctx* c) {
    if (!c) return LASS_ERR_ARG;
    prof_collect(c);
    for (auto& p : c->prof) { p.ms = 0; p.launches = 0; }
    return 0;
}

}
```

### lass_amd/csrc/kernels.h

```cpp
#pragma once
#include <hip/hip_runtime.h>
#include <stddef.h>
#include <stdint.h>

constexpr int LASS_NFFT = 1024;
constexpr int LASS_HOP = 160;
constexpr int LASS_NBINS = 513;
constexpr int LASS_FCROP = 512;
constexpr int LASS_COND = 512;
constexpr int LASS_MAX_STFT_WINDOWS = 4;

struct ConvArgs {
    const float* in = nullptr;
    long in_bs = 0;
    int Cin = 0;
    const float* w = nullptr;
    int Nw = 0;
    const float* pro_scale = nullptr;
    const float* pro_shift = nullptr;
    int pro_shift_bs = 0;
    const float* in2 = nullptr;
    long in2_bs = 0;
    int Cin2 = 0;
    const float* w2 = nullptr;
    const float* bias = nullptr;
    const float* res = nullptr;
    long res_bs = 0;
    const float* epi_scale = nullptr;
    const float* epi_shift = nullptr;
    int epi_shift_bs = 0;
    float* out = nullptr;
    long out_bs = 0;
    int B = 0, H = 0, W = 0;
    int N = 0;
    int up_h = 1;
    const float* w_wino = nullptr;
    const float* w2_wino = nullptr;
    const float* w_wino4 = nullptr;
    const void* w_bf16 = nullptr;
    const void* w2_bf16 = nullptr;
    const void* w_bf16_lo = nullptr;
    const void* w2_bf16_lo = nullptr;
    void* out_bf16 = nullptr;
    void* out_bf16_lo = nullptr;
    const void* in_bf16 = nullptr;
    const void* in_bf16_lo = nullptr;
    void* out_bf16_act = nullptr;
    const float* act_scale = nullptr;
    const float* act_shift = nullptr;
    int act_shift_bs = 0;
    int out_oct0 = 0;
    int out_noct = 0;
    const void* in2_bf16 = nullptr;
    void* pool_bf16 = nullptr;
    void* pool_bf16_act = nullptr;
    int pool_oct0 = 0;
    int pool_noct = 0;
    const float* pool_act_scale = nullptr;
    const float* pool_act_shift = nullptr;
    const float* pre_w = nullptr;
    const float* pre_b = nullptr;
    const float* mask_w = nullptr;
    const float* mask_b = nullptr;
    const float* mask_mag = nullptr;
    const float* mask_cos = nullptr;
    const float* mask_sin = nullptr;
    float* mask_re = nullptr;
    float* mask_im = nullptr;
    int mask_T = 0;
    int mask_nbins = LASS_NBINS;
    float* pool_out = nullptr;
    long pool_bs = 0;
    int pool_h = 2;
    int gx = 0, gy = 0;
    int xcd_map = 0;
};

enum ConvKind { CONV1_ACT = 0, CONV2_IDENT = 1, CONV2_SHORTCUT = 2, TCONV_ACT = 3, CONV1_ACT_PRE = 4, CONV2_IDENT_PRE = 5 };

hipError_t lass_launch_conv(ConvKind kind, const ConvArgs& p, hipStream_t stream);

bool lass_wino_supported(const ConvArgs& p);
hipError_t lass_launch_wino(ConvKind kind, const ConvArgs& p, hipStream_t stream);
hipError_t lass_launch_wino_weights(const float* w, int Cout, int Cin, float* U, hipStream_t stream);
hipError_t lass_launch_wino_shortcut_weights(const float* w, int Cout, int Cin, float* U, hipStream_t stream);

bool lass_wino4_supported(ConvKind kind, const ConvArgs& p);
hipError_t lass_launch_wino4(ConvKind kind, const ConvArgs& p, hipStream_t stream);
hipError_t lass_launch_wino4_weights(const float* w, int Cout, int Cin, float* U, hipStream_t stream);

bool lass_pw_gemm_supported(ConvKind kind, const ConvArgs& p);
hipError_t lass_launch_pw_gemm(ConvKind kind, const ConvArgs& p, hipStream_t stream);

bool lass_bf16_supported(const ConvArgs& p);
hipError_t lass_launch_conv_bf16(ConvKind kind, const ConvArgs& p, hipStream_t stream);
hipError_t lass_launch_weights_bf16(const float* w, int Cout, int Cin, int taps, void* dst, int lo, int transposed,
                                    hipStream_t stream);

bool lass_enc1_fused_bf16_supported(const ConvArgs& p, const ConvArgs& q);
hipError_t lass_launch_enc1_fused_bf16(const ConvArgs& p, const ConvArgs& q, hipStream_t stream);
bool lass_dec6_fused_bf16_supported(const ConvArgs& p, const ConvArgs& q);
hipError_t lass_launch_dec6_fused_bf16(const ConvArgs& p, const ConvArgs& q, hipStream_t stream);

bool lass_dec6u_fused_bf16_supported(const ConvArgs& p, const ConvArgs& q, const ConvArgs& u);
hipError_t lass_launch_dec6u_fused_bf16(const ConvArgs& p, const ConvArgs& q, const ConvArgs& u, hipStream_t stream);
hipError_t lass_launch_compose_up_shortcut(const float* wsc, const float* wt, int Cin, int Cup, int Ccat, int Nsc, float* out,
                                           hipStream_t stream);

hipError_t lass_launch_multi_stft(const float* wav, int B, int L, int hop, int nwin, const int* n_fft,
                                  const float2* tw2k, float* const* mag, float* const* cosv, float* const* sinv,
                                  hipStream_t stream);
struct StftBranch {
    int wlen = 0;
    float *mag = nullptr, *cosv = nullptr, *sinv = nullptr, *real = nullptr, *imag = nullptr, *x0 = nullptr;
};
hipError_t lass_launch_stft2(const float* wav, int B, int L, int n_fft, int hop, int T, int Tpad, int nbr,
                             const StftBranch* br, int magphase_sem, const float* s0, const float* h0,
                             const float2* tw2k, hipStream_t stream);
hipError_t lass_launch_istft2(const float* real, const float* imag, int B, int T, int L, int n_fft, int wlen, int hop,
                              const float2* tw2k, float* wav, hipStream_t stream);

hipError_t lass_launch_film(const float* cond, int B, const float* Wf, const float* bf, const float* base, int n,
                            float* out, hipStream_t stream);
hipError_t lass_launch_pool(const float* in, long in_bs, int B, int C, int H, int W, int ph, int pw, float* out,
                            hipStream_t stream);
hipError_t lass_launch_mask(const float* x12, const float* wa, const float* ba, const float* mag, const float* cosv,
                            const float* sinv, int B, int T, int Tpad, int fcrop, float* out_real, float* out_imag,
                            hipStream_t stream);
hipError_t lass_launch_x0_from_mag(const float* mag, int B, int T, int Tpad, int fcrop, const float* s0,
                                   const float* h0, float* x0, hipStream_t stream);
hipError_t lass_launch_sdr(const float* ref, const float* est, int B, int L, double* stats, hipStream_t stream);
hipError_t lass_launch_mix_at_snr(float* source, const float* noise, const float* snr_db, float* mixture, int B, int L,
                                  double* ws, hipStream_t stream);
hipError_t lass_launch_segment_mix(const float* waveforms, int B, int L, const int* mix_num, const float* comp_db, int max_comp,
                                   const float* noise_db, float* mixture, float* segment, double* ws, hipStream_t stream);
hipError_t lass_launch_relayout_conv(const float* src, int Cout, int Cin, int taps, float* dst, hipStream_t stream);
hipError_t lass_launch_bnfold(const float* g, const float* beta, const float* mean, const float* var, int C, float eps,
                              float* scale, float* base, hipStream_t stream);
```

### lass_amd/csrc/wino4.hip

```cpp
#include <hip/hip_runtime.h>
#include "kernels.h"
#include "pixel_ops.h"
#include "wino_common.h"

namespace {

constexpr int F_PRO = 1, F_PHASEB = 2, F_BIAS = 4, F_RES = 8, F_EPIACT = 16, F_PRECONV = 64, F_RESPRE = 128, F_MASK = 1024;
constexpr int NTHREADS = 256;
constexpr int KC = 8;
constexpr int NXI = 36;
constexpr int U_F = NXI * 256;
constexpr int V_F = NXI * 4 * 32 * 2;

typedef float f32x2v __attribute__((ext_vector_type(2)));

__device__ __forceinline__ void bt6(const float (&d)[6], float (&r)[6]) {
    const float t0 = fmaf(-4.f, d[2], d[4]);
    const float t1 = fmaf(-4.f, d[1], d[3]);
    const float t2 = d[4] - d[2];
    const float u = d[3] - d[1];
    r[0] = fmaf(4.f, d[0], fmaf(-5.f, d[2], d[4]));
    r[1] = t0 + t1;
    r[2] = t0 - t1;
    r[3] = fmaf(2.f, u, t2);
    r[4] = fmaf(-2.f, u, t2);
    r[5] = fmaf(4.f, d[1], fmaf(-5.f, d[3], d[5]));
}

__device__ __forceinline__ void at6(const float (&m)[6], float (&y)[4]) {
    const float s12 = m[1] + m[2], d12 = m[1] - m[2], s34 = m[3] + m[4], d34 = m[3] - m[4];
    y[0] = m[0] + s12 + s34;
    y[1] = fmaf(2.f, d34, d12);
    y[2] = fmaf(4.f, s34, s12);
    y[3] = fmaf(8.f, d34, d12) + m[5];
}

template <int TC, int FLAGS>
__global__ __launch_bounds__(NTHREADS, 2) void wino4_kernel(ConvArgs p) {
    constexpr bool PRO = (FLAGS & F_PRO) != 0, EPI = (FLAGS & F_EPIACT) != 0, SC = (FLAGS & F_PHASEB) != 0;
    constexpr bool PRE = (FLAGS & F_PRECONV) != 0;
    constexpr bool RESPRE = (FLAGS & F_RESPRE) != 0;
    constexpr bool MASK = (FLAGS & F_MASK) != 0;
    constexpr bool RES = (FLAGS & F_RES) != 0;
    static_assert(!SC || (FLAGS & F_BIAS) != 0, "the shortcut conv has a bias");
    static_assert(!PRE || PRO, "pre_conv is folded into the prologue's affine");
    static_assert(!RESPRE || ((FLAGS & F_RES) != 0 && !SC && !EPI), "conv2 with the identity residual");
    static_assert(!MASK || SC, "the output head sits behind decoder_block6's conv2 + shortcut");
    static_assert(!RES || (!SC && !EPI), "conv2 with a residual in place of the fused shortcut");
    constexpr int TR = 32 / TC;
    constexpr int OR_ = 4 * TR, OC = 4 * TC;
    constexpr int NCO = 32;
    __shared__ __attribute__((aligned(16))) float lds[U_F + V_F + 2 * NCO + (MASK ? 100 : 0)];
    float* lu = lds;
    float* lv = lds + U_F;
    float* lds_es = lv + V_F;
    float* lds_eh = lds_es + NCO;
    float* lds_mw = lds_eh + NCO;

    const int tid = threadIdx.x;
    const int lane = tid & 63, wave = __builtin_amdgcn_readfirstlane(tid >> 6);
    const int wco = wave >> 1, wwt = wave & 1;
    int bx_, by_, b;
    block_coords(p, bx_, by_, b);
    const int n0 = by_ * NCO;
    const int tiles_x = p.W / OC;
    const int y0 = (bx_ / tiles_x) * OR_, x0 = (bx_ % tiles_x) * OC;
    const int HW = p.H * p.W;
    const float* in_b = p.in + (size_t)b * p.in_bs;
    const float* sc = PRO ? p.pro_scale : nullptr;
    const float* sh = PRO ? p.pro_shift + (size_t)b * p.pro_shift_bs : nullptr;

    if (EPI && tid < NCO) {
        lds_es[tid] = p.epi_scale[n0 + tid];
        lds_eh[tid] = p.epi_shift[(size_t)b * p.epi_shift_bs + n0 + tid];
    }
    if (SC && tid < NCO) lds_es[tid] = p.bias[n0 + tid];
    if (RESPRE && tid < 32) {
        lds_es[tid] = p.pre_w[n0 + tid];
        lds_eh[tid] = p.pre_b[n0 + tid];
    }
    if (MASK && tid < 99) lds_mw[tid] = tid < 96 ? p.mask_w[tid] : p.mask_b[tid - 96];

    f32x4 acc[NXI];
#pragma unroll
    for (int xi = 0; xi < NXI; ++xi)
#pragma unroll
        for (int r = 0; r < 4; ++r) acc[xi][r] = 0.f;

    const int kq = lane >> 4, l15 = lane & 15;
    const float* afrag = lu + (wco >> 1) * U_F + (wco & 1) * 128 + (kq * 16 + l15) * 2;
    const float* bfrag = lv + (kq * 32 + ((wwt * 16 + l15) ^ ((kq & 1) << 4))) * 2;
    const unsigned slab_pitch = (unsigned)(p.Nw / 32) * (unsigned)(U_F * 4);
    const unsigned slab_n0 = (unsigned)(n0 / 32) * (unsigned)(U_F * 4);
    const unsigned lu_addr = (unsigned)(size_t)(__attribute__((address_space(3))) float*)lu;
    const unsigned ulane = (unsigned)lane * 16u;
    const v4i32 uw = make_rsrc_words(p.w_wino4, (unsigned)(NXI * p.Cin * p.Nw) * 4u);

    const int pt = tid & 31, c8 = (tid & 255) >> 5;
    const int pty = pt / TC, ptx = pt % TC;
    const int gy0 = y0 + 4 * pty - 1, gx0 = x0 + 4 * ptx - 1;
    const bool left = gx0 < 0, right = gx0 + 5 >= p.W;
    unsigned vo_c[6], vo_l[6], vo_r[6], rowok = 0;
#pragma unroll
    for (int i = 0; i < 6; ++i) {
        const int gy = gy0 + i;
        const int row = (PRE ? 0 : c8 * HW) + min(max(gy, 0), p.H - 1) * p.W;
        vo_c[i] = 4u * (unsigned)(row + gx0 + 1);
        vo_l[i] = 4u * (unsigned)(row + (left ? 0 : gx0));
        vo_r[i] = 4u * (unsigned)(row + (right ? p.W - 1 : gx0 + 5));
        rowok |= (gy >= 0 && gy < p.H ? 1u : 0u) << i;
    }
    const __amdgpu_buffer_rsrc_t in_rsrc =
        __builtin_amdgcn_make_buffer_rsrc(const_cast<float*>(in_b), 0, (int)((unsigned)(PRE ? 1 : p.Cin) * (unsigned)HW * 4u), 0x00020000);
    const bool edge = left || right || rowok != 0x3fu;
    float4 pc[6];
    float pl[6], pr[6], ps = 1.f, ph = 0.f;
    const unsigned tvo = (unsigned)c8 * 4u;
    const auto tab_rsrc = [&](const float* t, int n) {
        return __builtin_amdgcn_make_buffer_rsrc(const_cast<float*>(t), 0, n * 4, 0x00020000);
    };
    const __amdgpu_buffer_rsrc_t sc_rsrc = tab_rsrc(PRO ? sc : p.in, p.Cin), sh_rsrc = tab_rsrc(PRO ? sh : p.in, p.Cin);
    const __amdgpu_buffer_rsrc_t pw_rsrc = tab_rsrc(PRE ? p.pre_w : p.in, 32), pb_rsrc = tab_rsrc(PRE ? p.pre_b : p.in, 32);
    auto pload = [&](int ch) {
        const unsigned soff = PRE ? 0u : (unsigned)(ch * KC * HW) * 4u;
        if (!PRE || ch == 0)
#pragma unroll
        for (int i = 0; i < 6; ++i) {
            pc[i] = __builtin_bit_cast(float4, __builtin_amdgcn_raw_buffer_load_b128(in_rsrc, (int)vo_c[i], (int)soff, 0));
            pl[i] = __builtin_bit_cast(float, __builtin_amdgcn_raw_buffer_load_b32(in_rsrc, (int)vo_l[i], (int)soff, 0));
            pr[i] = __builtin_bit_cast(float, __builtin_amdgcn_raw_buffer_load_b32(in_rsrc, (int)vo_r[i], (int)soff, 0));
        }
        const unsigned toff = (unsigned)(ch * KC) * 4u;
        if (PRO) {
            ps = __builtin_bit_cast(float, __builtin_amdgcn_raw_buffer_load_b32(sc_rsrc, (int)tvo, (int)toff, 0));
            ph = __builtin_bit_cast(float, __builtin_amdgcn_raw_buffer_load_b32(sh_rsrc, (int)tvo, (int)toff, 0));
        }
        if (PRE) {
            const float pw = __builtin_bit_cast(float, __builtin_amdgcn_raw_buffer_load_b32(pw_rsrc, (int)tvo, (int)toff, 0));
            const float pb = __builtin_bit_cast(float, __builtin_amdgcn_raw_buffer_load_b32(pb_rsrc, (int)tvo, (int)toff, 0));
            ph = fmaf(pb, ps, ph);
            ps = pw * ps;
        }
    };
    constexpr int NLOAD = (PRE ? 0 : 6 * 3) + (PRO ? 2 : 0) + (PRE ? 2 : 0);
    float* vdst = lv + ((c8 & 3) * 32 + (pt ^ ((c8 & 1) << 4))) * 2 + (c8 >> 2);
    auto pprocess = [&]() {
        float d[6][6];
#pragma unroll
        for (int i = 0; i < 6; ++i) {
            const float v[6] = {pl[i], pc[i].x, pc[i].y, pc[i].z, pc[i].w, pr[i]};
#pragma unroll
            for (int jx = 0; jx < 6; ++jx) d[i][jx] = PRO ? leaky(fmaf(v[jx], ps, ph)) : v[jx];
        }
        if (__builtin_amdgcn_ballot_w64(edge) != 0) {
            const bool r0 = (rowok & 1u) != 0, r5 = (rowok & 32u) != 0;
#pragma unroll
            for (int jx = 0; jx < 6; ++jx) {
                d[0][jx] = r0 ? d[0][jx] : 0.f;
                d[5][jx] = r5 ? d[5][jx] : 0.f;
            }
#pragma unroll
            for (int i = 0; i < 6; ++i) {
                d[i][0] = left ? 0.f : d[i][0];
                d[i][5] = right ? 0.f : d[i][5];
            }
        }
        float tt[6][6];
#pragma unroll
        for (int jx = 0; jx < 6; ++jx) {
            const float col[6] = {d[0][jx], d[1][jx], d[2][jx], d[3][jx], d[4][jx], d[5][jx]};
            float r[6];
            bt6(col, r);
#pragma unroll
            for (int i = 0; i < 6; ++i) tt[i][jx] = r[i];
        }
#pragma unroll
        for (int i = 0; i < 6; ++i) {
            float r[6];
            bt6(tt[i], r);
#pragma unroll
            for (int jx = 0; jx < 6; ++jx) vdst[(i * 6 + jx) * 256] = r[jx];
        }
    };

    const int nch = p.Cin / KC;
    pload(0);
    lds_barrier();
    for (int ch = 0; ch < nch; ++ch) {
        lds_barrier();
        __builtin_amdgcn_s_setprio(2);
#pragma unroll
        for (int i = 0; i < 6; ++i) {
            asm volatile("" : "+v"(pc[i].x), "+v"(pc[i].y), "+v"(pc[i].z), "+v"(pc[i].w), "+v"(pl[i]), "+v"(pr[i]));
        }
        if (PRO) asm volatile("" : "+v"(ps), "+v"(ph));
#pragma unroll
        for (int i = 0; i < 9; ++i) {
            const unsigned piece = (unsigned)(wave * 9 + i) * 1024u;
            lds_dma_16B(uw, ulane, (unsigned)ch * slab_pitch + slab_n0 + piece, lu_addr + piece);
        }
        __builtin_amdgcn_sched_barrier(0);
        pprocess();
        __builtin_amdgcn_sched_barrier(0);
        const bool pf = ch + 1 < nch;
        if (pf) pload(ch + 1);
        __builtin_amdgcn_sched_barrier(0);
        if (pf)
            wait_vmcnt<NLOAD>();
        else
            wait_vmcnt<0>();
        lds_barrier();
        __builtin_amdgcn_s_setprio(0);
        constexpr int PFD = 2;
        f32x2v av[PFD + 1][2], bv[PFD + 1][2];
        auto rd = [&](int s) {
#pragma unroll
            for (int q = 0; q < 2; ++q) {
                av[s % (PFD + 1)][q] = *reinterpret_cast<const f32x2v*>(afrag + (2 * s + q) * 256);
                bv[s % (PFD + 1)][q] = *reinterpret_cast<const f32x2v*>(bfrag + (2 * s + q) * 256);
            }
        };
#pragma unroll
        for (int s = 0; s < PFD; ++s) rd(s);
#pragma unroll
        for (int s = 0; s < NXI / 2; ++s) {
            if (s + PFD < NXI / 2) rd(s + PFD);
            __builtin_amdgcn_sched_barrier(0);
            const f32x2v a0 = av[s % (PFD + 1)][0], a1 = av[s % (PFD + 1)][1];
            const f32x2v b0 = bv[s % (PFD + 1)][0], b1 = bv[s % (PFD + 1)][1];
            acc[2 * s] = __builtin_amdgcn_mfma_f32_16x16x4f32(a0.x, b0.x, acc[2 * s], 0, 0, 0);
            acc[2 * s + 1] = __builtin_amdgcn_mfma_f32_16x16x4f32(a1.x, b1.x, acc[2 * s + 1], 0, 0, 0);
            acc[2 * s] = __builtin_amdgcn_mfma_f32_16x16x4f32(a0.y, b0.y, acc[2 * s], 0, 0, 0);
            acc[2 * s + 1] = __builtin_amdgcn_mfma_f32_16x16x4f32(a1.y, b1.y, acc[2 * s + 1], 0, 0, 0);
            __builtin_amdgcn_sched_barrier(0);
        }
    }

    const int ot = wwt * 16 + l15;
    const int oy = y0 + 4 * (ot / TC), ox = x0 + 4 * (ot % TC);
    f32x4 ysp[16];
#pragma unroll
    for (int r = 0; r < 4; ++r) {
        const int nl = wco * 16 + kq * 4 + r;
        float tmp[4][6];
#pragma unroll
        for (int jx = 0; jx < 6; ++jx) {
            const float m[6] = {acc[0 + jx][r], acc[6 + jx][r], acc[12 + jx][r], acc[18 + jx][r], acc[24 + jx][r], acc[30 + jx][r]};
            float y[4];
            at6(m, y);
#pragma unroll
            for (int a = 0; a < 4; ++a) tmp[a][jx] = y[a];
        }
        const float es = (EPI || SC) ? lds_es[nl] : 0.f, eh = EPI ? lds_eh[nl] : 0.f;
#pragma unroll
        for (int a = 0; a < 4; ++a) {
            float y[4];
            at6(tmp[a], y);
#pragma unroll
            for (int c = 0; c < 4; ++c) {
                float v = y[c];
                if (EPI) v = leaky(fmaf(v, es, eh));
                if (SC) v += es;
                ysp[a * 4 + c][r] = v;
            }
        }
    }
    if constexpr (RESPRE) {
        const float* xr = p.res + (size_t)b * p.res_bs + (size_t)min(oy, p.H - 4) * p.W + ox;
        float4 xv[4];
#pragma unroll
        for (int a = 0; a < 4; ++a) xv[a] = *reinterpret_cast<const float4*>(xr + (size_t)a * p.W);
#pragma unroll
        for (int r = 0; r < 4; ++r) {
            const float pw = lds_es[wco * 16 + kq * 4 + r], pb = lds_eh[wco * 16 + kq * 4 + r];
#pragma unroll
            for (int a = 0; a < 4; ++a) {
                ysp[a * 4 + 0][r] += fmaf(xv[a].x, pw, pb);
                ysp[a * 4 + 1][r] += fmaf(xv[a].y, pw, pb);
                ysp[a * 4 + 2][r] += fmaf(xv[a].z, pw, pb);
                ysp[a * 4 + 3][r] += fmaf(xv[a].w, pw, pb);
            }
        }
    }
    if constexpr (RES && !RESPRE) {
        float4 rv[4][4];
#pragma unroll
        for (int r = 0; r < 4; ++r) {
            const float* rr = p.res + (size_t)b * p.res_bs + (size_t)(n0 + wco * 16 + kq * 4 + r) * HW + (size_t)min(oy, p.H - 4) * p.W + ox;
#pragma unroll
            for (int a = 0; a < 4; ++a) rv[r][a] = *reinterpret_cast<const float4*>(rr + (size_t)a * p.W);
        }
#pragma unroll
        for (int r = 0; r < 4; ++r)
#pragma unroll
            for (int a = 0; a < 4; ++a) {
                ysp[a * 4 + 0][r] += rv[r][a].x;
                ysp[a * 4 + 1][r] += rv[r][a].y;
                ysp[a * 4 + 2][r] += rv[r][a].z;
                ysp[a * 4 + 3][r] += rv[r][a].w;
            }
    }
    if constexpr (SC) {
        const float* x2 = p.in2 + (size_t)b * p.in2_bs + (size_t)min(oy, p.H - 4) * p.W + ox;
        const float* wsc = p.w2 + n0 + wco * 16 + l15;
        const int nks = p.Cin2 / 4;
        constexpr int NSB = 4;
        float4 xb[NSB][4];
        float wa[NSB];
        auto ldk = [&](int ks, int buf) {
            const float* xp = x2 + (size_t)(4 * ks + kq) * HW;
#pragma unroll
            for (int a = 0; a < 4; ++a) xb[buf][a] = *reinterpret_cast<const float4*>(xp + (size_t)a * p.W);
            wa[buf] = wsc[(size_t)(4 * ks + kq) * p.Nw];
        };
        auto mmk = [&](int buf) {
#pragma unroll
            for (int a = 0; a < 4; ++a) {
                ysp[a * 4 + 0] = __builtin_amdgcn_mfma_f32_16x16x4f32(wa[buf], xb[buf][a].x, ysp[a * 4 + 0], 0, 0, 0);
                ysp[a * 4 + 1] = __builtin_amdgcn_mfma_f32_16x16x4f32(wa[buf], xb[buf][a].y, ysp[a * 4 + 1], 0, 0, 0);
                ysp[a * 4 + 2] = __builtin_amdgcn_mfma_f32_16x16x4f32(wa[buf], xb[buf][a].z, ysp[a * 4 + 2], 0, 0, 0);
                ysp[a * 4 + 3] = __builtin_amdgcn_mfma_f32_16x16x4f32(wa[buf], xb[buf][a].w, ysp[a * 4 + 3], 0, 0, 0);
            }
        };
        ldk(0, 0);
        ldk(1, 1);
        ldk(2, 2);
        for (int ks = 0; ks < nks; ks += NSB) {
#pragma unroll
            for (int u = 0; u < NSB; ++u) {
                ldk(min(ks + u + 3, nks - 1), (u + 3) % NSB);
                __builtin_amdgcn_sched_barrier(0);
                mmk(u);
                __builtin_amdgcn_sched_barrier(0);
            }
        }
    }
    if constexpr (MASK) {
        float* part = lds;
        lds_barrier();
#pragma unroll
        for (int q = 0; q < 3; ++q) {
            float w4[4];
#pragma unroll
            for (int r = 0; r < 4; ++r) w4[r] = lds_mw[q * 32 + wco * 16 + kq * 4 + r];
#pragma unroll
            for (int a = 0; a < 4; ++a) {
                float4 o;
                float* op = &o.x;
#pragma unroll
                for (int c = 0; c < 4; ++c) {
                    const f32x4 v = ysp[a * 4 + c];
                    op[c] = v[0] * w4[0] + v[1] * w4[1] + v[2] * w4[2] + v[3] * w4[3];
                }
                *reinterpret_cast<float4*>(part + ((wco * 4 + kq) * 3 + q) * 512 + ot * 16 + a * 4) = o;
            }
        }
        lds_barrier();
        const int px = tid * 2;
        const int mt = px >> 4, ms = px & 15;
        const int my = y0 + 4 * (mt / TC) + (ms >> 2), mx = x0 + 4 * (mt % TC) + (ms & 3);
        float lg[3][2];
#pragma unroll
        for (int q = 0; q < 3; ++q) {
            float2 sum = make_float2(lds_mw[96 + q], lds_mw[96 + q]);
#pragma unroll
            for (int src = 0; src < 8; ++src) {
                const float2 v = *reinterpret_cast<const float2*>(part + (src * 3 + q) * 512 + px);
                sum.x += v.x;
                sum.y += v.y;
            }
            lg[q][0] = sum.x;
            lg[q][1] = sum.y;
        }
        if (my < p.mask_T) {
            mask_pixel(p, b, my, mx, lg[0][0], lg[1][0], lg[2][0]);
            mask_pixel(p, b, my, mx + 1, lg[0][1], lg[1][1], lg[2][1]);
        }
        return;
    }
#pragma unroll
    for (int r = 0; r < 4; ++r) {
        const int n = n0 + wco * 16 + kq * 4 + r;
        float* dst = p.out + (size_t)b * p.out_bs + (size_t)n * HW + (size_t)oy * p.W + ox;
#pragma unroll
        for (int a = 0; a < 4; ++a) {
            const float4 o = make_float4(ysp[a * 4 + 0][r], ysp[a * 4 + 1][r], ysp[a * 4 + 2][r], ysp[a * 4 + 3][r]);
            if (oy + a < p.H) *reinterpret_cast<float4*>(dst + (size_t)a * p.W) = o;
        }
        if ((SC || RES) && p.pool_out) {
            const int Ho = p.H / 2, Wo = p.W / 2;
            float* pd = p.pool_out + (size_t)b * (p.pool_bs ? (size_t)p.pool_bs : (size_t)p.N * Ho * Wo) + (size_t)n * Ho * Wo +
                        (size_t)(oy >> 1) * Wo + (ox >> 1);
#pragma unroll
            for (int i = 0; i < 2; ++i) {
                float2 o;
                float s0 = ysp[(2 * i) * 4 + 0][r] + ysp[(2 * i) * 4 + 1][r];
                s0 += ysp[(2 * i + 1) * 4 + 0][r];
                s0 += ysp[(2 * i + 1) * 4 + 1][r];
                float s1 = ysp[(2 * i) * 4 + 2][r] + ysp[(2 * i) * 4 + 3][r];
                s1 += ysp[(2 * i + 1) * 4 + 2][r];
                s1 += ysp[(2 * i + 1) * 4 + 3][r];
                o.x = s0 * 0.25f;
                o.y = s1 * 0.25f;
                if (oy + 2 * i + 1 < p.H) *reinterpret_cast<float2*>(pd + (size_t)i * Wo) = o;
            }
        }
    }
}

__global__ __launch_bounds__(256) void wino4_weights_kernel(const float* __restrict__ w, int Cout, int Cin, float* __restrict__ U) {
    const long i = (long)blockIdx.x * 256 + threadIdx.x;
    if (i >= (long)Cout * Cin) return;
    const int co = (int)(i % Cout), ci = (int)(i / Cout);
    const float* g = w + ((size_t)co * Cin + ci) * 9;
    const double G[6][3] = {{0.25, 0, 0},           {-1.0 / 6, -1.0 / 6, -1.0 / 6}, {-1.0 / 6, 1.0 / 6, -1.0 / 6},
                            {1.0 / 24, 1.0 / 12, 1.0 / 6}, {1.0 / 24, -1.0 / 12, 1.0 / 6},  {0, 0, 1}};
    double t[6][3];
    for (int a = 0; a < 6; ++a)
        for (int c = 0; c < 3; ++c) t[a][c] = G[a][0] * (double)g[0 * 3 + c] + G[a][1] * (double)g[1 * 3 + c] + G[a][2] * (double)g[2 * 3 + c];
    float* slab = U + ((size_t)(ci / 8) * (Cout / 32) + co / 32) * U_F;
    const int e = (((co & 31) >> 4) * 4 + (ci & 3)) * 32 + (co & 15) * 2 + ((ci & 7) >> 2);
    for (int a = 0; a < 6; ++a)
        for (int c = 0; c < 6; ++c) {
            const double u = t[a][0] * G[c][0] + t[a][1] * G[c][1] + t[a][2] * G[c][2];
            slab[(a * 6 + c) * 256 + e] = (float)u;
        }
}

template <int TC, int FLAGS>
hipError_t launch_wino4_tc(const ConvArgs& p0, hipStream_t stream) {
    ConvArgs p = p0;
    constexpr int OR_ = 4 * (32 / TC), OC = 4 * TC;
    p.gx = (p.W / OC) * ((p.H + OR_ - 1) / OR_);
    p.gy = p.N / 32;
    p.xcd_map = ((long)p.gx * p.B) % 8 == 0;
    hipLaunchKernelGGL((wino4_kernel<TC, FLAGS>), dim3((unsigned)((long)p.gx * p.gy * p.B)), dim3(NTHREADS), 0, stream, p);
    return hipGetLastError();
}

template <int FLAGS>
hipError_t launch_wino4(const ConvArgs& p, hipStream_t stream) {
    if (p.W % 64 == 0 && p.H % 8 == 0) return launch_wino4_tc<16, FLAGS>(p, stream);
    if (p.H % 16 == 0) return launch_wino4_tc<8, FLAGS>(p, stream);
    return hipErrorInvalidValue;
}

}

bool lass_wino4_supported(ConvKind kind, const ConvArgs& p) {
    if (!(p.w_wino4 && ((p.W % 64 == 0 && p.H % 8 == 0) || (p.W % 32 == 0 && p.H % 16 == 0)) && p.Cin % KC == 0 && p.N % 32 == 0 &&
          p.Nw % 32 == 0 && (unsigned long long)p.Cin * p.H * p.W * 4ull < 0xFFFF0000ull))
        return false;
    switch (kind) {
        case CONV1_ACT:
            return true;
        case CONV1_ACT_PRE:
            return p.pre_w && p.pre_b && p.Cin == 32;
        case CONV2_IDENT_PRE:
            return p.res && p.pre_w && p.pre_b && p.N == 32 && p.Nw == 32 && (!p.pool_out || p.pool_h == 2);
        case CONV2_IDENT:
            return p.res && !p.mask_re && (!p.pool_out || p.pool_h == 2);
        case CONV2_SHORTCUT:
            if (!(p.in2 && p.w2 && p.bias && p.Cin2 % 16 == 0 && (!p.pool_out || p.pool_h == 2))) return false;
            if (p.mask_re)
                return p.N == 32 && p.Nw == 32 && p.W + 1 == p.mask_nbins && p.mask_w && p.mask_b && p.mask_mag && p.mask_cos && p.mask_sin &&
                       p.mask_im && p.mask_T > 0 && p.mask_T <= p.H && !p.pool_out;
            return true;
        default:
            return false;
    }
}

hipError_t lass_launch_wino4(ConvKind kind, const ConvArgs& p, hipStream_t stream) {
    if (!lass_wino4_supported(kind, p) || !p.in || (!p.out && !p.mask_re)) return hipErrorInvalidValue;
    switch (kind) {
        case CONV1_ACT:
        case CONV1_ACT_PRE:
            if (!p.pro_scale || !p.pro_shift || !p.epi_scale || !p.epi_shift) return hipErrorInvalidValue;
            return kind == CONV1_ACT ? launch_wino4<F_PRO | F_EPIACT>(p, stream) : launch_wino4<F_PRO | F_EPIACT | F_PRECONV>(p, stream);
        case CONV2_IDENT:
            return launch_wino4<F_RES>(p, stream);
        case CONV2_IDENT_PRE:
            return launch_wino4<F_RES | F_RESPRE>(p, stream);
        case CONV2_SHORTCUT:
            return p.mask_re ? launch_wino4<F_PHASEB | F_BIAS | F_MASK>(p, stream) : launch_wino4<F_PHASEB | F_BIAS>(p, stream);
        default:
            return hipErrorInvalidValue;
    }
}

hipError_t lass_launch_wino4_weights(const float* w, int Cout, int Cin, float* U, hipStream_t stream) {
    const long n = (long)Cout * Cin;
    hipLaunchKernelGGL(wino4_weights_kernel, dim3((unsigned)((n + 255) / 256)), dim3(256), 0, stream, w, Cout, Cin, U);
    return hipGetLastError();
}
```

Before: 1017 clips/s.

## Extend Winograd F(4,3) conv to narrow-width levels with split-K partial sums

Enables the Winograd F(4x4,3x3) MFMA conv path for feature maps whose width is 16 mod 32 (the deep, narrow ResUNet levels). These convs are split along input channels into 4 partial-sum slices written to a new workspace region, which a later pass reduces with the epilogue. The intent is to raise occupancy and parallelism on small spatial grids with many channels, where the old path fell back to the slower F(2,3) Winograd kernel. In exchange it adds workspace, extra partial-sum memory traffic and a reduction step, plus a runtime knob for the split count.

New measurement: 1037 clips/s (median of 6 runs). +1.9%, better.

```diff
diff --git a/include/lass_hip.h b/include/lass_hip.h
--- a/include/lass_hip.h
+++ b/include/lass_hip.h
@@ -43,6 +43,7 @@
 
 int lass_graph_stats(const lass_ctx* ctx, long* captures, long* replays);
 int lass_set_graph_replay(lass_ctx* ctx, int enabled);
+int lass_set_wino4_splits(lass_ctx* ctx, int splits);
 
 int lass_separate_components(lass_ctx* ctx, const float* const* mag, const float* cos_mask, const float* sin_mask,
                              const float* condition, float* out, int B, int L, void* workspace, size_t workspace_bytes,
diff --git a/lass_amd/_lib.py b/lass_amd/_lib.py
--- a/lass_amd/_lib.py
+++ b/lass_amd/_lib.py
@@ -28,6 +28,7 @@
                                 POINTER(c_void_p), POINTER(c_void_p), c_void_p]),
     ("lass_graph_stats", c_int, [c_void_p, POINTER(c_long), POINTER(c_long)]),
     ("lass_set_graph_replay", c_int, [c_void_p, c_int]),
+    ("lass_set_wino4_splits", c_int, [c_void_p, c_int]),
     ("lass_separate_components", c_int, [c_void_p, POINTER(c_void_p), c_void_p, c_void_p, c_void_p, c_void_p, c_int,
                                          c_int, c_void_p, c_size_t, c_void_p]),
     ("lass_stft_components", c_int, [c_void_p, c_void_p, c_int, c_int, c_int, c_int, c_int, POINTER(c_int),
diff --git a/lass_amd/arch.py b/lass_amd/arch.py
--- a/lass_amd/arch.py
+++ b/lass_amd/arch.py
@@ -148,13 +148,20 @@
     if min_cin <= 0:
         return set()
     with_shortcut = {r["name"].rsplit(".", 1)[0] for r in rows if r["name"].endswith(".shortcut")}
+    block_cin = {r["name"].rsplit(".", 1)[0]: r["cin"] for r in rows if r["name"].endswith(".conv1")}
     out = set()
     for r in rows:
         if r["kind"] != "3x3":
             continue
         block, conv = r["name"].rsplit(".", 1)
         geom = r["w"] % 32 == 0 and ((r["w"] % 64 == 0 and r["h"] % 8 == 0) or r["h"] % 16 == 0)
-        if not (geom and r["cin"] >= min_cin and r["cin"] % 8 == 0 and r["cout"] % 32 == 0):
+        narrow = r["w"] % 32 == 16 and r["h"] % 32 == 0
+        if not ((geom or narrow) and r["cin"] >= min_cin and r["cin"] % 8 == 0 and r["cout"] % 32 == 0):
+            continue
+        if narrow:
+            cin1 = block_cin.get(block, r["cin"])
+            if r["w"] == 16 and r["cout"] % 64 == 0 and cin1 % 16 == 0 and min(cin1, r["cout"]) >= min_cin and not block.startswith("encoder_block1"):
+                out.add(r["name"])
             continue
         if conv == "conv1":
             out.add(r["name"])
diff --git a/lass_amd/csrc/api.hip b/lass_amd/csrc/api.hip
--- a/lass_amd/csrc/api.hip
+++ b/lass_amd/csrc/api.hip
@@ -95,6 +95,9 @@
     std::vector<void*> owned;
     int compute_mode = LASS_COMPUTE_F32;
     int wino4_mincin = 32;
+    int ksplit_force = 0;
+    float* stage_part = nullptr;
+    size_t stage_part_floats = 0;
     bool fuse_catb = true;
     bool fuse_block = true;
     bool fuse_up = true;
@@ -396,7 +399,17 @@
     const Site* act_out = nullptr;
     const CatCopies* pool_copies = nullptr;
     const UpFuse* up = nullptr;
+    float* kpart = nullptr;
 };
+
+constexpr int kWino4Splits = 4;
+int wino4_splits(const lass_ctx* c, const ResBlock& rb, int B, int H, int W) {
+    (void)B;
+    if (c->compute_mode != LASS_COMPUTE_F32 || c->wino4_mincin <= 0 || !lass_wino4_narrow(H, W) || rb.width % 32 != 16) return 0;
+    if (rb.cin < c->wino4_mincin || rb.cout < c->wino4_mincin || rb.cin % 8 != 0 || rb.cout % 32 != 0) return 0;
+    return c->ksplit_force ? c->ksplit_force : kWino4Splits;
+}
+size_t wino4_split_floats(const ResBlock& rb, int S, int B, int H, int W) { return S > 1 ? (size_t)S * B * rb.cout * H * W : 0; }
 
 constexpr int kShortcutGemmMinCin = 256;
 
@@ -429,12 +442,26 @@
     if (cat_in) p.in_bf16 = cat_in->act;
     const ConvKind k1 = x0 ? CONV1_ACT_PRE : CONV1_ACT, k2 = x0 ? CONV2_IDENT_PRE : CONV2_IDENT;
     const bool wino1 = !bf1 && rb.u1 && lass_wino_supported(p);
+    const int ksplit = bf1 || x0 ? 0 : wino4_splits(c, rb, B, H, W);
+    const bool w4_geom = rb.width % 32 == 0 ? !lass_wino4_narrow(H, W) : ksplit > 0;
+    if (ksplit > 1) {
+        if (!f.kpart) return fail(c, LASS_ERR_STATE, "split-K needs its partial workspace");
+        const auto overlaps = [&](const float* a, size_t a_n, const float* b, long b_bs, long b_n) {
+            return a < b + (size_t)(B - 1) * b_bs + b_n && b < a + a_n;
+        };
+        const size_t kn = wino4_split_floats(rb, ksplit, B, H, W);
+        if (overlaps(f.kpart, kn, x, x_bs, rb.cin * HW) || overlaps(f.kpart, kn, a2, rb.cout * HW, rb.cout * HW) ||
+            overlaps(f.kpart, kn, out, out_bs, rb.cout * HW))
+            return fail(c, LASS_ERR_STATE, "the split-K partials must not overlap the block's input, intermediate or output");
+    }
+    Wino4Split sk;
+    if (ksplit > 1) { sk.n = ksplit; sk.part = f.kpart; }
     auto launch_conv1 = [&]() -> int {
         ProfScope ps(c, st, P_CONV3X3);
         if (bf1)
             HIP_TRY(c, lass_launch_conv_bf16(k1, p, st));
-        else if (wino1 && rb.u1f && lass_wino4_supported(k1, p))
-            HIP_TRY(c, lass_launch_wino4(k1, p, st));
+        else if (wino1 && rb.u1f && w4_geom && lass_wino4_supported(k1, p, sk))
+            HIP_TRY(c, lass_launch_wino4(k1, p, st, sk));
         else if (wino1)
             HIP_TRY(c, lass_launch_wino(k1, p, st));
         else
@@ -445,7 +472,7 @@
     q.in = a2; q.in_bs = rb.cout * HW; q.Cin = rb.cout; q.w = rb.w2; q.Nw = rb.cout; q.N = rb.cout;
     q.out = out; q.out_bs = out_bs; q.B = B; q.H = H; q.W = W;
     q.pool_out = f.pool_out; q.pool_h = f.pool_h; q.pool_bs = f.pool_bs;
-    q.w_wino = rb.u2; q.w2_wino = rb.usc; q.w_wino4 = rb.u2f;
+    q.w_wino = rb.u2; q.w2_wino = rb.usc; q.w_wino4 = w4_geom ? rb.u2f : nullptr;
     if (const MaskHead* mh = f.head) {
         q.out = nullptr;
         q.mask_w = rawp(c, "base.after_conv.weight"); q.mask_b = rawp(c, "base.after_conv.bias");
@@ -508,7 +535,7 @@
         return 0;
     }
     const bool sc_gemm = c->compute_mode == LASS_COMPUTE_F32 && !bf2 && rb.cin != rb.cout && !f.head && rb.cin >= kShortcutGemmMinCin &&
-                         wino2 && rb.u2f && lass_wino4_supported(CONV2_SHORTCUT, q) && lass_pw_gemm_supported(CONV2_SHORTCUT, q);
+                         wino2 && q.w_wino4 && (ksplit > 0 || lass_wino4_supported(CONV2_SHORTCUT, q)) && lass_pw_gemm_supported(CONV2_SHORTCUT, q);
     if (sc_gemm) {
         const auto overlaps = [&](const float* a, long a_bs, long a_n, const float* b, long b_bs, long b_n) {
             return a < b + (size_t)(B - 1) * b_bs + b_n && b < a + (size_t)(B - 1) * a_bs + a_n;
@@ -524,13 +551,13 @@
         ConvArgs r = q;
         r.in2 = nullptr; r.in2_bs = 0; r.Cin2 = 0; r.w2 = nullptr; r.bias = nullptr;
         r.res = out; r.res_bs = out_bs;
-        if (!lass_wino4_supported(CONV2_IDENT, r)) return fail(c, LASS_ERR_STATE, "conv2 with the shortcut as residual");
-        HIP_TRY(c, lass_launch_wino4(CONV2_IDENT, r, st));
+        if (!lass_wino4_supported(CONV2_IDENT, r, sk)) return fail(c, LASS_ERR_STATE, "conv2 with the shortcut as residual");
+        HIP_TRY(c, lass_launch_wino4(CONV2_IDENT, r, st, sk));
     } else if (rb.cin == rb.cout) {
         if (bf2)
             HIP_TRY(c, lass_launch_conv_bf16(k2, q, st));
-        else if (wino2 && x0 && rb.u2f && lass_wino4_supported(k2, q))
-            HIP_TRY(c, lass_launch_wino4(k2, q, st));
+        else if (wino2 && (x0 || ksplit > 0) && q.w_wino4 && lass_wino4_supported(k2, q, sk))
+            HIP_TRY(c, lass_launch_wino4(k2, q, st, sk));
         else if (wino2)
             HIP_TRY(c, lass_launch_wino(k2, q, st));
         else
@@ -538,7 +565,7 @@
     } else {
         if (bf2)
             HIP_TRY(c, lass_launch_conv_bf16(CONV2_SHORTCUT, q, st));
-        else if (wino2 && rb.u2f && lass_wino4_supported(CONV2_SHORTCUT, q))
+        else if (wino2 && q.w_wino4 && lass_wino4_supported(CONV2_SHORTCUT, q))
             HIP_TRY(c, lass_launch_wino4(CONV2_SHORTCUT, q, st));
         else if (wino2)
             HIP_TRY(c, lass_launch_wino(CONV2_SHORTCUT, q, st));
@@ -587,6 +614,8 @@
     int B, L, T, Tp;
     size_t total = 0;
     size_t mag, cosv, sinv, x0[kMaxBranches], shift, a2, cat[6], pool[6], center, decout[6], oreal, oimag;
+    size_t kpart = 0;
+    bool has_kpart = false;
     int eh[7], ew[7];
 };
 
@@ -628,6 +657,17 @@
     }
     pl->a2 = bump(t, a2max);
     pl->oreal = bump(t, spec); pl->oimag = bump(t, spec);
+    size_t kmax = 0;
+    for (int i = 1; i < 7; ++i) {
+        const ResBlock& rb = trunk_block(c, i);
+        kmax = std::max(kmax, wino4_split_floats(rb, wino4_splits(c, rb, B, pl->eh[i], pl->ew[i]), B, pl->eh[i], pl->ew[i]));
+    }
+    for (int d = 0; d < 6; ++d) {
+        const ResBlock& rb = c->dec[d];
+        kmax = std::max(kmax, wino4_split_floats(rb, wino4_splits(c, rb, B, pl->eh[5 - d], pl->ew[5 - d]), B, pl->eh[5 - d], pl->ew[5 - d]));
+    }
+    pl->has_kpart = kmax > 0;
+    if (kmax) pl->kpart = bump(t, kmax);
     return 0;
 }
 
@@ -653,6 +693,19 @@
 }
 
 bool split_halves(const lass_ctx* c, int B) { return c->split_batch > 0 && !c->profiling && B >= 8 && (B % 2) == 0; }
+
+int stage_kpart(lass_ctx* c, const ResBlock& rb, int B, int H, int W, BlockFusions* f) {
+    const size_t need = wino4_split_floats(rb, wino4_splits(c, rb, B, H, W), B, H, W);
+    if (need > c->stage_part_floats) {
+        if (c->stage_part) HIP_TRY(c, hipFree(c->stage_part));
+        c->stage_part = nullptr;
+        c->stage_part_floats = 0;
+        HIP_TRY(c, hipMalloc((void**)&c->stage_part, need * sizeof(float)));
+        c->stage_part_floats = need;
+    }
+    if (need) f->kpart = c->stage_part;
+    return 0;
+}
 
 const ResBlock* find_block(const lass_ctx* c, const std::string& prefix) {
     for (const auto& rb : c->enc) if (rb.prefix == prefix) return &rb;
@@ -772,6 +825,7 @@
     if (c->ev_join) (void)hipEventDestroy(c->ev_join);
     if (c->ev_fork) (void)hipEventDestroy(c->ev_fork);
     (void)hipFree(c->tw2k);
+    (void)hipFree(c->stage_part);
     delete c;
     return 0;
 }
@@ -879,13 +933,13 @@
                 return LASS_ERR_HIP;
             HIP_TRY(c, lass_launch_wino_weights(w1, rb.cout, rb.cin, rb.u1, st));
             HIP_TRY(c, lass_launch_wino_weights(w2, rb.cout, rb.cout, rb.u2, st));
-            const bool w4_level = rb.width % 32 == 0;
-            if (w4_level && c->wino4_mincin > 0 && rb.cin >= c->wino4_mincin && rb.cin % 8 == 0 && rb.cout % 32 == 0) {
+            const bool w4_level = rb.width % 32 == 0, w4_narrow = rb.width % 32 == 16;
+            if ((w4_level || w4_narrow) && c->wino4_mincin > 0 && rb.cin >= c->wino4_mincin && rb.cin % 8 == 0 && rb.cout % 32 == 0) {
                 if (dev_alloc(c, &rb.u1f, (size_t)36 * rb.cout * rb.cin)) return LASS_ERR_HIP;
                 HIP_TRY(c, lass_launch_wino4_weights(w1, rb.cout, rb.cin, rb.u1f, st));
             }
-            if (w4_level && c->wino4_mincin > 0 && rb.cout >= c->wino4_mincin && (rb.cin != rb.cout || rb.cout == kPreCh) && rb.cout % 32 == 0 &&
-                rb.cin % 8 == 0) {
+            if (c->wino4_mincin > 0 && rb.cout >= c->wino4_mincin && rb.cout % 32 == 0 && rb.cin % 8 == 0 &&
+                (w4_level ? rb.cin != rb.cout || rb.cout == kPreCh : w4_narrow && rb.cin >= c->wino4_mincin)) {
                 if (dev_alloc(c, &rb.u2f, (size_t)36 * rb.cout * rb.cout)) return LASS_ERR_HIP;
                 HIP_TRY(c, lass_launch_wino4_weights(w2, rb.cout, rb.cout, rb.u2f, st));
             }
@@ -1074,7 +1128,9 @@
     const ResBlock* rb = find_block(c, prefix);
     if (!rb) return fail(c, LASS_ERR_ARG, std::string("lass_convblock: unknown block '") + prefix + "'");
     const long HW = (long)H * W;
-    return run_resblock(c, *rb, x, rb->cin * HW, B, H, W, shift, scratch, y, rb->cout * HW, (hipStream_t)stream);
+    BlockFusions f;
+    if ((r = stage_kpart(c, *rb, B, H, W, &f))) return r;
+    return run_resblock(c, *rb, x, rb->cin * HW, B, H, W, shift, scratch, y, rb->cout * HW, (hipStream_t)stream, f);
 }
 
 int lass_encoder_block(lass_ctx* c, const char* name, const float* x, int B, int H, int W, const float* shift, float* y,
@@ -1094,6 +1150,7 @@
         hipStream_t st = (hipStream_t)stream;
         BlockFusions f;
         if (fuse) { f.pool_out = pool; f.pool_h = e.dh; }
+        if ((r = stage_kpart(c, rb, B, H, W, &f))) return r;
         r = run_resblock(c, rb, x, rb.cin * HW, B, H, W, shift, scratch, y, rb.cout * HW, st, f);
         if (r) return r;
         if (pooled && !fuse) HIP_TRY(c, lass_launch_pool(y, rb.cout * HW, B, rb.cout, H, W, e.dh, e.dw, pool, st));
@@ -1325,6 +1382,7 @@
             if (i < 5 && use_cb[5 - i]) f.skip_out = &cb[5 - i];
             if (i >= 1 && i <= 4 && use_pc[i - 1]) f.cat_in = &pc[i - 1];
             if (i < 4 && use_pc[i]) f.pool_copies = &pc[i];
+            if (pl.has_kpart) f.kpart = F(pl.kpart);
             r = run_resblock(c, rb, x, rb.cin * HW, B, H, W, shift, F(pl.a2), o, o_bs, st, f);
             if (r) return r;
         }
@@ -1354,6 +1412,7 @@
         if (use_cb[d]) f.cat_in = &cb[d];
         const MaskHead head{mag_m, cos_m, sin_m, F(pl.oreal), F(pl.oimag), T, g.nbins};
         if (d == 5) f.head = &head;
+        if (pl.has_kpart) f.kpart = F(pl.kpart);
         r = run_resblock(c, rb, F(pl.cat[d]), rb.cin * HW, B, H, W, shift, F(pl.a2), F(pl.decout[d]), rb.cout * HW, st, f);
         if (r) return r;
         x = F(pl.decout[d]);
@@ -1479,6 +1538,13 @@
     return 0;
 }
 
+int lass_set_wino4_splits(lass_ctx* c, int splits) {
+    if (!c || (splits != 0 && splits != 1 && splits != 2 && splits != 4)) return fail(c, LASS_ERR_ARG, "lass_set_wino4_splits: 0, 1, 2 or 4");
+    c->ksplit_force = splits;
+    ++c->gen;
+    return 0;
+}
+
 int lass_graph_stats(const lass_ctx* c, long* captures, long* replays) {
     if (!c) return LASS_ERR_ARG;
     if (captures) *captures = c->g_captures;
diff --git a/lass_amd/csrc/kernels.h b/lass_amd/csrc/kernels.h
--- a/lass_amd/csrc/kernels.h
+++ b/lass_amd/csrc/kernels.h
@@ -76,6 +76,12 @@
     int xcd_map = 0;
 };
 
+inline bool lass_wino4_narrow(int H, int W) { return W % 32 == 16 && H % 32 == 0; }
+struct Wino4Split {
+    int n = 1;
+    float* part = nullptr;
+};
+
 enum ConvKind { CONV1_ACT = 0, CONV2_IDENT = 1, CONV2_SHORTCUT = 2, TCONV_ACT = 3, CONV1_ACT_PRE = 4, CONV2_IDENT_PRE = 5 };
 
 hipError_t lass_launch_conv(ConvKind kind, const ConvArgs& p, hipStream_t stream);
@@ -85,8 +91,8 @@
 hipError_t lass_launch_wino_weights(const float* w, int Cout, int Cin, float* U, hipStream_t stream);
 hipError_t lass_launch_wino_shortcut_weights(const float* w, int Cout, int Cin, float* U, hipStream_t stream);
 
-bool lass_wino4_supported(ConvKind kind, const ConvArgs& p);
-hipError_t lass_launch_wino4(ConvKind kind, const ConvArgs& p, hipStream_t stream);
+bool lass_wino4_supported(ConvKind kind, const ConvArgs& p, const Wino4Split& sk = Wino4Split());
+hipError_t lass_launch_wino4(ConvKind kind, const ConvArgs& p, hipStream_t stream, const Wino4Split& sk = Wino4Split());
 hipError_t lass_launch_wino4_weights(const float* w, int Cout, int Cin, float* U, hipStream_t stream);
 
 bool lass_pw_gemm_supported(ConvKind kind, const ConvArgs& p);
diff --git a/lass_amd/csrc/wino4.hip b/lass_amd/csrc/wino4.hip
--- a/lass_amd/csrc/wino4.hip
+++ b/lass_amd/csrc/wino4.hip
@@ -6,6 +6,7 @@
 namespace {
 
 constexpr int F_PRO = 1, F_PHASEB = 2, F_BIAS = 4, F_RES = 8, F_EPIACT = 16, F_PRECONV = 64, F_RESPRE = 128, F_MASK = 1024;
+constexpr int F_SPLITK = 2048;
 constexpr int NTHREADS = 256;
 constexpr int KC = 8;
 constexpr int NXI = 36;
@@ -37,373 +38,66 @@
 
 template <int TC, int FLAGS>
 __global__ __launch_bounds__(NTHREADS, 2) void wino4_kernel(ConvArgs p) {
-    constexpr bool PRO = (FLAGS & F_PRO) != 0, EPI = (FLAGS & F_EPIACT) != 0, SC = (FLAGS & F_PHASEB) != 0;
-    constexpr bool PRE = (FLAGS & F_PRECONV) != 0;
-    constexpr bool RESPRE = (FLAGS & F_RESPRE) != 0;
-    constexpr bool MASK = (FLAGS & F_MASK) != 0;
-    constexpr bool RES = (FLAGS & F_RES) != 0;
-    static_assert(!SC || (FLAGS & F_BIAS) != 0, "the shortcut conv has a bias");
-    static_assert(!PRE || PRO, "pre_conv is folded into the prologue's affine");
-    static_assert(!RESPRE || ((FLAGS & F_RES) != 0 && !SC && !EPI), "conv2 with the identity residual");
-    static_assert(!MASK || SC, "the output head sits behind decoder_block6's conv2 + shortcut");
-    static_assert(!RES || (!SC && !EPI), "conv2 with a residual in place of the fused shortcut");
-    constexpr int TR = 32 / TC;
-    constexpr int OR_ = 4 * TR, OC = 4 * TC;
-    constexpr int NCO = 32;
-    __shared__ __attribute__((aligned(16))) float lds[U_F + V_F + 2 * NCO + (MASK ? 100 : 0)];
-    float* lu = lds;
-    float* lv = lds + U_F;
-    float* lds_es = lv + V_F;
-    float* lds_eh = lds_es + NCO;
-    float* lds_mw = lds_eh + NCO;
-
-    const int tid = threadIdx.x;
-    const int lane = tid & 63, wave = __builtin_amdgcn_readfirstlane(tid >> 6);
-    const int wco = wave >> 1, wwt = wave & 1;
-    int bx_, by_, b;
-    block_coords(p, bx_, by_, b);
-    const int n0 = by_ * NCO;
-    const int tiles_x = p.W / OC;
-    const int y0 = (bx_ / tiles_x) * OR_, x0 = (bx_ % tiles_x) * OC;
-    const int HW = p.H * p.W;
-    const float* in_b = p.in + (size_t)b * p.in_bs;
-    const float* sc = PRO ? p.pro_scale : nullptr;
-    const float* sh = PRO ? p.pro_shift + (size_t)b * p.pro_shift_bs : nullptr;
-
-    if (EPI && tid < NCO) {
-        lds_es[tid] = p.epi_scale[n0 + tid];
-        lds_eh[tid] = p.epi_shift[(size_t)b * p.epi_shift_bs + n0 + tid];
-    }
-    if (SC && tid < NCO) lds_es[tid] = p.bias[n0 + tid];
-    if (RESPRE && tid < 32) {
-        lds_es[tid] = p.pre_w[n0 + tid];
-        lds_eh[tid] = p.pre_b[n0 + tid];
-    }
-    if (MASK && tid < 99) lds_mw[tid] = tid < 96 ? p.mask_w[tid] : p.mask_b[tid - 96];
-
-    f32x4 acc[NXI];
-#pragma unroll
-    for (int xi = 0; xi < NXI; ++xi)
-#pragma unroll
-        for (int r = 0; r < 4; ++r) acc[xi][r] = 0.f;
-
-    const int kq = lane >> 4, l15 = lane & 15;
-    const float* afrag = lu + (wco >> 1) * U_F + (wco & 1) * 128 + (kq * 16 + l15) * 2;
-    const float* bfrag = lv + (kq * 32 + ((wwt * 16 + l15) ^ ((kq & 1) << 4))) * 2;
-    const unsigned slab_pitch = (unsigned)(p.Nw / 32) * (unsigned)(U_F * 4);
-    const unsigned slab_n0 = (unsigned)(n0 / 32) * (unsigned)(U_F * 4);
-    const unsigned lu_addr = (unsigned)(size_t)(__attribute__((address_space(3))) float*)lu;
-    const unsigned ulane = (unsigned)lane * 16u;
-    const v4i32 uw = make_rsrc_words(p.w_wino4, (unsigned)(NXI * p.Cin * p.Nw) * 4u);
-
-    const int pt = tid & 31, c8 = (tid & 255) >> 5;
-    const int pty = pt / TC, ptx = pt % TC;
-    const int gy0 = y0 + 4 * pty - 1, gx0 = x0 + 4 * ptx - 1;
-    const bool left = gx0 < 0, right = gx0 + 5 >= p.W;
-    unsigned vo_c[6], vo_l[6], vo_r[6], rowok = 0;
-#pragma unroll
-    for (int i = 0; i < 6; ++i) {
-        const int gy = gy0 + i;
-        const int row = (PRE ? 0 : c8 * HW) + min(max(gy, 0), p.H - 1) * p.W;
-        vo_c[i] = 4u * (unsigned)(row + gx0 + 1);
-        vo_l[i] = 4u * (unsigned)(row + (left ? 0 : gx0));
-        vo_r[i] = 4u * (unsigned)(row + (right ? p.W - 1 : gx0 + 5));
-        rowok |= (gy >= 0 && gy < p.H ? 1u : 0u) << i;
-    }
-    const __amdgpu_buffer_rsrc_t in_rsrc =
-        __builtin_amdgcn_make_buffer_rsrc(const_cast<float*>(in_b), 0, (int)((unsigned)(PRE ? 1 : p.Cin) * (unsigned)HW * 4u), 0x00020000);
-    const bool edge = left || right || rowok != 0x3fu;
-    float4 pc[6];
-    float pl[6], pr[6], ps = 1.f, ph = 0.f;
-    const unsigned tvo = (unsigned)c8 * 4u;
-    const auto tab_rsrc = [&](const float* t, int n) {
-        return __builtin_amdgcn_make_buffer_rsrc(const_cast<float*>(t), 0, n * 4, 0x00020000);
-    };
-    const __amdgpu_buffer_rsrc_t sc_rsrc = tab_rsrc(PRO ? sc : p.in, p.Cin), sh_rsrc = tab_rsrc(PRO ? sh : p.in, p.Cin);
-    const __amdgpu_buffer_rsrc_t pw_rsrc = tab_rsrc(PRE ? p.pre_w : p.in, 32), pb_rsrc = tab_rsrc(PRE ? p.pre_b : p.in, 32);
-    auto pload = [&](int ch) {
-        const unsigned soff = PRE ? 0u : (unsigned)(ch * KC * HW) * 4u;
-        if (!PRE || ch == 0)
-#pragma unroll
-        for (int i = 0; i < 6; ++i) {
-            pc[i] = __builtin_bit_cast(float4, __builtin_amdgcn_raw_buffer_load_b128(in_rsrc, (int)vo_c[i], (int)soff, 0));
-            pl[i] = __builtin_bit_cast(float, __builtin_amdgcn_raw_buffer_load_b32(in_rsrc, (int)vo_l[i], (int)soff, 0));
-            pr[i] = __builtin_bit_cast(float, __builtin_amdgcn_raw_buffer_load_b32(in_rsrc, (int)vo_r[i], (int)soff, 0));
-        }
-        const unsigned toff = (unsigned)(ch * KC) * 4u;
-        if (PRO) {
-            ps = __builtin_bit_cast(float, __builtin_amdgcn_raw_buffer_load_b32(sc_rsrc, (int)tvo, (int)toff, 0));
-            ph = __builtin_bit_cast(float, __builtin_amdgcn_raw_buffer_load_b32(sh_rsrc, (int)tvo, (int)toff, 0));
-        }
-        if (PRE) {
-            const float pw = __builtin_bit_cast(float, __builtin_amdgcn_raw_buffer_load_b32(pw_rsrc, (int)tvo, (int)toff, 0));
-            const float pb = __builtin_bit_cast(float, __builtin_amdgcn_raw_buffer_load_b32(pb_rsrc, (int)tvo, (int)toff, 0));
-            ph = fmaf(pb, ps, ph);
-            ps = pw * ps;
-        }
-    };
-    constexpr int NLOAD = (PRE ? 0 : 6 * 3) + (PRO ? 2 : 0) + (PRE ? 2 : 0);
-    float* vdst = lv + ((c8 & 3) * 32 + (pt ^ ((c8 & 1) << 4))) * 2 + (c8 >> 2);
-    auto pprocess = [&]() {
-        float d[6][6];
-#pragma unroll
-        for (int i = 0; i < 6; ++i) {
-            const float v[6] = {pl[i], pc[i].x, pc[i].y, pc[i].z, pc[i].w, pr[i]};
-#pragma unroll
-            for (int jx = 0; jx < 6; ++jx) d[i][jx] = PRO ? leaky(fmaf(v[jx], ps, ph)) : v[jx];
-        }
-        if (__builtin_amdgcn_ballot_w64(edge) != 0) {
-            const bool r0 = (rowok & 1u) != 0, r5 = (rowok & 32u) != 0;
-#pragma unroll
-            for (int jx = 0; jx < 6; ++jx) {
-                d[0][jx] = r0 ? d[0][jx] : 0.f;
-                d[5][jx] = r5 ? d[5][jx] : 0.f;
-            }
-#pragma unroll
-            for (int i = 0; i < 6; ++i) {
-                d[i][0] = left ? 0.f : d[i][0];
-                d[i][5] = right ? 0.f : d[i][5];
-            }
-        }
-        float tt[6][6];
-#pragma unroll
-        for (int jx = 0; jx < 6; ++jx) {
-            const float col[6] = {d[0][jx], d[1][jx], d[2][jx], d[3][jx], d[4][jx], d[5][jx]};
-            float r[6];
-            bt6(col, r);
-#pragma unroll
-            for (int i = 0; i < 6; ++i) tt[i][jx] = r[i];
-        }
-#pragma unroll
-        for (int i = 0; i < 6; ++i) {
-            float r[6];
-            bt6(tt[i], r);
-#pragma unroll
-            for (int jx = 0; jx < 6; ++jx) vdst[(i * 6 + jx) * 256] = r[jx];
-        }
-    };
-
-    const int nch = p.Cin / KC;
-    pload(0);
-    lds_barrier();
-    for (int ch = 0; ch < nch; ++ch) {
-        lds_barrier();
-        __builtin_amdgcn_s_setprio(2);
-#pragma unroll
-        for (int i = 0; i < 6; ++i) {
-            asm volatile("" : "+v"(pc[i].x), "+v"(pc[i].y), "+v"(pc[i].z), "+v"(pc[i].w), "+v"(pl[i]), "+v"(pr[i]));
-        }
-        if (PRO) asm volatile("" : "+v"(ps), "+v"(ph));
-#pragma unroll
-        for (int i = 0; i < 9; ++i) {
-            const unsigned piece = (unsigned)(wave * 9 + i) * 1024u;
-            lds_dma_16B(uw, ulane, (unsigned)ch * slab_pitch + slab_n0 + piece, lu_addr + piece);
-        }
-        __builtin_amdgcn_sched_barrier(0);
-        pprocess();
-        __builtin_amdgcn_sched_barrier(0);
-        const bool pf = ch + 1 < nch;
-        if (pf) pload(ch + 1);
-        __builtin_amdgcn_sched_barrier(0);
-        if (pf)
-            wait_vmcnt<NLOAD>();
-        else
-            wait_vmcnt<0>();
-        lds_barrier();
-        __builtin_amdgcn_s_setprio(0);
-        constexpr int PFD = 2;
-        f32x2v av[PFD + 1][2], bv[PFD + 1][2];
-        auto rd = [&](int s) {
-#pragma unroll
-            for (int q = 0; q < 2; ++q) {
-                av[s % (PFD + 1)][q] = *reinterpret_cast<const f32x2v*>(afrag + (2 * s + q) * 256);
-                bv[s % (PFD + 1)][q] = *reinterpret_cast<const f32x2v*>(bfrag + (2 * s + q) * 256);
-            }
-        };
-#pragma unroll
-        for (int s = 0; s < PFD; ++s) rd(s);
-#pragma unroll
-        for (int s = 0; s < NXI / 2; ++s) {
-            if (s + PFD < NXI / 2) rd(s + PFD);
-            __builtin_amdgcn_sched_barrier(0);
-            const f32x2v a0 = av[s % (PFD + 1)][0], a1 = av[s % (PFD + 1)][1];
-            const f32x2v b0 = bv[s % (PFD + 1)][0], b1 = bv[s % (PFD + 1)][1];
-            acc[2 * s] = __builtin_amdgcn_mfma_f32_16x16x4f32(a0.x, b0.x, acc[2 * s], 0, 0, 0);
-            acc[2 * s + 1] = __builtin_amdgcn_mfma_f32_16x16x4f32(a1.x, b1.x, acc[2 * s + 1], 0, 0, 0);
-            acc[2 * s] = __builtin_amdgcn_mfma_f32_16x16x4f32(a0.y, b0.y, acc[2 * s], 0, 0, 0);
-            acc[2 * s + 1] = __builtin_amdgcn_mfma_f32_16x16x4f32(a1.y, b1.y, acc[2 * s + 1], 0, 0, 0);
-            __builtin_amdgcn_sched_barrier(0);
-        }
-    }
-
-    const int ot = wwt * 16 + l15;
-    const int oy = y0 + 4 * (ot / TC), ox = x0 + 4 * (ot % TC);
-    f32x4 ysp[16];
-#pragma unroll
-    for (int r = 0; r < 4; ++r) {
-        const int nl = wco * 16 + kq * 4 + r;
-        float tmp[4][6];
-#pragma unroll
-        for (int jx = 0; jx < 6; ++jx) {
-            const float m[6] = {acc[0 + jx][r], acc[6 + jx][r], acc[12 + jx][r], acc[18 + jx][r], acc[24 + jx][r], acc[30 + jx][r]};
-            float y[4];
-            at6(m, y);
-#pragma unroll
-            for (int a = 0; a < 4; ++a) tmp[a][jx] = y[a];
-        }
-        const float es = (EPI || SC) ? lds_es[nl] : 0.f, eh = EPI ? lds_eh[nl] : 0.f;
-#pragma unroll
-        for (int a = 0; a < 4; ++a) {
-            float y[4];
-            at6(tmp[a], y);
-#pragma unroll
-            for (int c = 0; c < 4; ++c) {
-                float v = y[c];
-                if (EPI) v = leaky(fmaf(v, es, eh));
-                if (SC) v += es;
-                ysp[a * 4 + c][r] = v;
-            }
-        }
-    }
-    if constexpr (RESPRE) {
-        const float* xr = p.res + (size_t)b * p.res_bs + (size_t)min(oy, p.H - 4) * p.W + ox;
-        float4 xv[4];
-#pragma unroll
-        for (int a = 0; a < 4; ++a) xv[a] = *reinterpret_cast<const float4*>(xr + (size_t)a * p.W);
-#pragma unroll
-        for (int r = 0; r < 4; ++r) {
-            const float pw = lds_es[wco * 16 + kq * 4 + r], pb = lds_eh[wco * 16 + kq * 4 + r];
-#pragma unroll
-            for (int a = 0; a < 4; ++a) {
-                ysp[a * 4 + 0][r] += fmaf(xv[a].x, pw, pb);
-                ysp[a * 4 + 1][r] += fmaf(xv[a].y, pw, pb);
-                ysp[a * 4 + 2][r] += fmaf(xv[a].z, pw, pb);
-                ysp[a * 4 + 3][r] += fmaf(xv[a].w, pw, pb);
-            }
-        }
-    }
-    if constexpr (RES && !RESPRE) {
-        float4 rv[4][4];
-#pragma unroll
-        for (int r = 0; r < 4; ++r) {
-            const float* rr = p.res + (size_t)b * p.res_bs + (size_t)(n0 + wco * 16 + kq * 4 + r) * HW + (size_t)min(oy, p.H - 4) * p.W + ox;
-#pragma unroll
-            for (int a = 0; a < 4; ++a) rv[r][a] = *reinterpret_cast<const float4*>(rr + (size_t)a * p.W);
-        }
-#pragma unroll
-        for (int r = 0; r < 4; ++r)
-#pragma unroll
-            for (int a = 0; a < 4; ++a) {
-                ysp[a * 4 + 0][r] += rv[r][a].x;
-                ysp[a * 4 + 1][r] += rv[r][a].y;
-                ysp[a * 4 + 2][r] += rv[r][a].z;
-                ysp[a * 4 + 3][r] += rv[r][a].w;
-            }
-    }
-    if constexpr (SC) {
-        const float* x2 = p.in2 + (size_t)b * p.in2_bs + (size_t)min(oy, p.H - 4) * p.W + ox;
-        const float* wsc = p.w2 + n0 + wco * 16 + l15;
-        const int nks = p.Cin2 / 4;
-        constexpr int NSB = 4;
-        float4 xb[NSB][4];
-        float wa[NSB];
-        auto ldk = [&](int ks, int buf) {
-            const float* xp = x2 + (size_t)(4 * ks + kq) * HW;
-#pragma unroll
-            for (int a = 0; a < 4; ++a) xb[buf][a] = *reinterpret_cast<const float4*>(xp + (size_t)a * p.W);
-            wa[buf] = wsc[(size_t)(4 * ks + kq) * p.Nw];
-        };
-        auto mmk = [&](int buf) {
-#pragma unroll
-            for (int a = 0; a < 4; ++a) {
-                ysp[a * 4 + 0] = __builtin_amdgcn_mfma_f32_16x16x4f32(wa[buf], xb[buf][a].x, ysp[a * 4 + 0], 0, 0, 0);
-                ysp[a * 4 + 1] = __builtin_amdgcn_mfma_f32_16x16x4f32(wa[buf], xb[buf][a].y, ysp[a * 4 + 1], 0, 0, 0);
-                ysp[a * 4 + 2] = __builtin_amdgcn_mfma_f32_16x16x4f32(wa[buf], xb[buf][a].z, ysp[a * 4 + 2], 0, 0, 0);
-                ysp[a * 4 + 3] = __builtin_amdgcn_mfma_f32_16x16x4f32(wa[buf], xb[buf][a].w, ysp[a * 4 + 3], 0, 0, 0);
-            }
-        };
-        ldk(0, 0);
-        ldk(1, 1);
-        ldk(2, 2);
-        for (int ks = 0; ks < nks; ks += NSB) {
-#pragma unroll
-            for (int u = 0; u < NSB; ++u) {
-                ldk(min(ks + u + 3, nks - 1), (u + 3) % NSB);
-                __builtin_amdgcn_sched_barrier(0);
-                mmk(u);
-                __builtin_amdgcn_sched_barrier(0);
-            }
-        }
-    }
-    if constexpr (MASK) {
-        float* part = lds;
-        lds_barrier();
-#pragma unroll
-        for (int q = 0; q < 3; ++q) {
-            float w4[4];
-#pragma unroll
-            for (int r = 0; r < 4; ++r) w4[r] = lds_mw[q * 32 + wco * 16 + kq * 4 + r];
-#pragma unroll
-            for (int a = 0; a < 4; ++a) {
-                float4 o;
-                float* op = &o.x;
-#pragma unroll
-                for (int c = 0; c < 4; ++c) {
-                    const f32x4 v = ysp[a * 4 + c];
-                    op[c] = v[0] * w4[0] + v[1] * w4[1] + v[2] * w4[2] + v[3] * w4[3];
-                }
-                *reinterpret_cast<float4*>(part + ((wco * 4 + kq) * 3 + q) * 512 + ot * 16 + a * 4) = o;
-            }
-        }
-        lds_barrier();
-        const int px = tid * 2;
-        const int mt = px >> 4, ms = px & 15;
-        const int my = y0 + 4 * (mt / TC) + (ms >> 2), mx = x0 + 4 * (mt % TC) + (ms & 3);
-        float lg[3][2];
-#pragma unroll
-        for (int q = 0; q < 3; ++q) {
-            float2 sum = make_float2(lds_mw[96 + q], lds_mw[96 + q]);
-#pragma unroll
-            for (int src = 0; src < 8; ++src) {
-                const float2 v = *reinterpret_cast<const float2*>(part + (src * 3 + q) * 512 + px);
-                sum.x += v.x;
-                sum.y += v.y;
-            }
-            lg[q][0] = sum.x;
-            lg[q][1] = sum.y;
-        }
-        if (my < p.mask_T) {
-            mask_pixel(p, b, my, mx, lg[0][0], lg[1][0], lg[2][0]);
-            mask_pixel(p, b, my, mx + 1, lg[0][1], lg[1][1], lg[2][1]);
-        }
-        return;
-    }
-#pragma unroll
-    for (int r = 0; r < 4; ++r) {
-        const int n = n0 + wco * 16 + kq * 4 + r;
-        float* dst = p.out + (size_t)b * p.out_bs + (size_t)n * HW + (size_t)oy * p.W + ox;
-#pragma unroll
-        for (int a = 0; a < 4; ++a) {
-            const float4 o = make_float4(ysp[a * 4 + 0][r], ysp[a * 4 + 1][r], ysp[a * 4 + 2][r], ysp[a * 4 + 3][r]);
-            if (oy + a < p.H) *reinterpret_cast<float4*>(dst + (size_t)a * p.W) = o;
-        }
-        if ((SC || RES) && p.pool_out) {
-            const int Ho = p.H / 2, Wo = p.W / 2;
-            float* pd = p.pool_out + (size_t)b * (p.pool_bs ? (size_t)p.pool_bs : (size_t)p.N * Ho * Wo) + (size_t)n * Ho * Wo +
-                        (size_t)(oy >> 1) * Wo + (ox >> 1);
-#pragma unroll
-            for (int i = 0; i < 2; ++i) {
-                float2 o;
-                float s0 = ysp[(2 * i) * 4 + 0][r] + ysp[(2 * i) * 4 + 1][r];
-                s0 += ysp[(2 * i + 1) * 4 + 0][r];
-                s0 += ysp[(2 * i + 1) * 4 + 1][r];
-                float s1 = ysp[(2 * i) * 4 + 2][r] + ysp[(2 * i) * 4 + 3][r];
-                s1 += ysp[(2 * i + 1) * 4 + 2][r];
-                s1 += ysp[(2 * i + 1) * 4 + 3][r];
-                o.x = s0 * 0.25f;
-                o.y = s1 * 0.25f;
-                if (oy + 2 * i + 1 < p.H) *reinterpret_cast<float2*>(pd + (size_t)i * Wo) = o;
-            }
+    const Wino4Split sk;
+#include "wino4_body.h"
+}
+template <int TC, int FLAGS0>
+__global__ __launch_bounds__(NTHREADS, 2) void wino4_splitk_kernel(ConvArgs p, Wino4Split sk) {
+    constexpr int FLAGS = FLAGS0 | F_SPLITK;
+#include "wino4_body.h"
+}
+
+template <int FLAGS>
+__global__ __launch_bounds__(256) void wino4_combine_kernel(ConvArgs p, Wino4Split sk) {
+    constexpr bool EPI = (FLAGS & F_EPIACT) != 0, RES = (FLAGS & F_RES) != 0;
+    static_assert(EPI != RES && (FLAGS & ~(F_EPIACT | F_RES)) == 0, "conv1 or the identity conv2");
+    const int W4 = p.W / 4, H2 = p.H / 2, HW = p.H * p.W;
+    const long idx = (long)blockIdx.x * 256 + threadIdx.x;
+    if (idx >= (long)p.B * p.N * H2 * W4) return;
+    const int xq = (int)(idx % W4), yh = (int)(idx / W4 % H2), n = (int)(idx / ((long)W4 * H2) % p.N), b = (int)(idx / ((long)W4 * H2 * p.N));
+    const size_t pix = (size_t)(2 * yh) * p.W + 4 * xq;
+    const size_t split_pitch = (size_t)p.B * p.N * HW;
+    const float* pp = sk.part + ((size_t)b * p.N + n) * HW + pix;
+    float4 v[2];
+#pragma unroll
+    for (int i = 0; i < 2; ++i) v[i] = *reinterpret_cast<const float4*>(pp + (size_t)i * p.W);
+    for (int s = 1; s < sk.n; ++s)
+#pragma unroll
+        for (int i = 0; i < 2; ++i) {
+            const float4 t = *reinterpret_cast<const float4*>(pp + (size_t)s * split_pitch + (size_t)i * p.W);
+            v[i].x += t.x; v[i].y += t.y; v[i].z += t.z; v[i].w += t.w;
+        }
+    if (EPI) {
+        const float es = p.epi_scale[n], eh = p.epi_shift[(size_t)b * p.epi_shift_bs + n];
+#pragma unroll
+        for (int i = 0; i < 2; ++i) {
+            v[i].x = leaky(fmaf(v[i].x, es, eh)); v[i].y = leaky(fmaf(v[i].y, es, eh));
+            v[i].z = leaky(fmaf(v[i].z, es, eh)); v[i].w = leaky(fmaf(v[i].w, es, eh));
+        }
+    }
+    if (RES) {
+        const float* rr = p.res + (size_t)b * p.res_bs + (size_t)n * HW + pix;
+        float4 t[2];
+#pragma unroll
+        for (int i = 0; i < 2; ++i) t[i] = *reinterpret_cast<const float4*>(rr + (size_t)i * p.W);
+#pragma unroll
+        for (int i = 0; i < 2; ++i) { v[i].x += t[i].x; v[i].y += t[i].y; v[i].z += t[i].z; v[i].w += t[i].w; }
+    }
+    float* dst = p.out + (size_t)b * p.out_bs + (size_t)n * HW + pix;
+#pragma unroll
+    for (int i = 0; i < 2; ++i) *reinterpret_cast<float4*>(dst + (size_t)i * p.W) = v[i];
+    if (RES && p.pool_out) {
+        const int Wo = p.W / 2, Ho = p.H / p.pool_h;
+        float* pd = p.pool_out + (size_t)b * (p.pool_bs ? (size_t)p.pool_bs : (size_t)p.N * Ho * Wo) + (size_t)n * Ho * Wo + 2 * xq;
+        if (p.pool_h == 2) {
+            float s0 = v[0].x + v[0].y, s1 = v[0].z + v[0].w;
+            s0 += v[1].x; s0 += v[1].y;
+            s1 += v[1].z; s1 += v[1].w;
+            *reinterpret_cast<float2*>(pd + (size_t)yh * Wo) = make_float2(s0 * 0.25f, s1 * 0.25f);
+        } else {
+#pragma unroll
+            for (int i = 0; i < 2; ++i)
+                *reinterpret_cast<float2*>(pd + (size_t)(2 * yh + i) * Wo) = make_float2((v[i].x + v[i].y) * 0.5f, (v[i].z + v[i].w) * 0.5f);
         }
     }
 }
@@ -441,16 +135,37 @@
 template <int FLAGS>
 hipError_t launch_wino4(const ConvArgs& p, hipStream_t stream) {
     if (p.W % 64 == 0 && p.H % 8 == 0) return launch_wino4_tc<16, FLAGS>(p, stream);
-    if (p.H % 16 == 0) return launch_wino4_tc<8, FLAGS>(p, stream);
+    if (p.W % 32 == 0 && p.H % 16 == 0) return launch_wino4_tc<8, FLAGS>(p, stream);
+    if constexpr (FLAGS == (F_PRO | F_EPIACT) || FLAGS == F_RES)
+        if (lass_wino4_narrow(p.H, p.W)) return launch_wino4_tc<4, FLAGS>(p, stream);
     return hipErrorInvalidValue;
 }
 
-}
-
-bool lass_wino4_supported(ConvKind kind, const ConvArgs& p) {
-    if (!(p.w_wino4 && ((p.W % 64 == 0 && p.H % 8 == 0) || (p.W % 32 == 0 && p.H % 16 == 0)) && p.Cin % KC == 0 && p.N % 32 == 0 &&
+template <int MAIN, int COMB>
+hipError_t launch_wino4_split(const ConvArgs& p0, const Wino4Split& sk, hipStream_t stream) {
+    ConvArgs p = p0;
+    p.gx = (p.W / 16) * (p.H / 32);
+    p.gy = p.N / 32;
+    p.xcd_map = ((long)p.gx * p.B * sk.n) % 8 == 0;
+    hipLaunchKernelGGL((wino4_splitk_kernel<4, MAIN>), dim3((unsigned)((long)p.gx * p.gy * p.B * sk.n)), dim3(NTHREADS), 0, stream, p, sk);
+    if (hipError_t e = hipGetLastError()) return e;
+    const long items = (long)p.B * p.N * (p.H / 2) * (p.W / 4);
+    hipLaunchKernelGGL((wino4_combine_kernel<COMB>), dim3((unsigned)((items + 255) / 256)), dim3(256), 0, stream, p, sk);
+    return hipGetLastError();
+}
+
+}
+
+bool lass_wino4_supported(ConvKind kind, const ConvArgs& p, const Wino4Split& sk) {
+    const bool narrow = lass_wino4_narrow(p.H, p.W);
+    if (!(p.w_wino4 && ((p.W % 64 == 0 && p.H % 8 == 0) || (p.W % 32 == 0 && p.H % 16 == 0) || narrow) && p.Cin % KC == 0 && p.N % 32 == 0 &&
           p.Nw % 32 == 0 && (unsigned long long)p.Cin * p.H * p.W * 4ull < 0xFFFF0000ull))
         return false;
+    if (narrow) {
+        if (sk.n != 1 && !(sk.n >= 2 && sk.n <= p.Cin / KC && sk.part && p.N == p.Nw)) return false;
+        return kind == CONV1_ACT || (kind == CONV2_IDENT && p.res && !p.mask_re && (!p.pool_out || p.pool_h == 2 || p.pool_h == 1));
+    }
+    if (sk.n != 1) return false;
     switch (kind) {
         case CONV1_ACT:
             return true;
@@ -471,14 +186,16 @@
     }
 }
 
-hipError_t lass_launch_wino4(ConvKind kind, const ConvArgs& p, hipStream_t stream) {
-    if (!lass_wino4_supported(kind, p) || !p.in || (!p.out && !p.mask_re)) return hipErrorInvalidValue;
+hipError_t lass_launch_wino4(ConvKind kind, const ConvArgs& p, hipStream_t stream, const Wino4Split& sk) {
+    if (!lass_wino4_supported(kind, p, sk) || !p.in || (!p.out && !p.mask_re)) return hipErrorInvalidValue;
     switch (kind) {
         case CONV1_ACT:
         case CONV1_ACT_PRE:
             if (!p.pro_scale || !p.pro_shift || !p.epi_scale || !p.epi_shift) return hipErrorInvalidValue;
+            if (sk.n > 1) return launch_wino4_split<F_PRO, F_EPIACT>(p, sk, stream);
             return kind == CONV1_ACT ? launch_wino4<F_PRO | F_EPIACT>(p, stream) : launch_wino4<F_PRO | F_EPIACT | F_PRECONV>(p, stream);
         case CONV2_IDENT:
+            if (sk.n > 1) return launch_wino4_split<0, F_RES>(p, sk, stream);
             return launch_wino4<F_RES>(p, stream);
         case CONV2_IDENT_PRE:
             return launch_wino4<F_RES | F_RESPRE>(p, stream);
diff --git a/lass_amd/csrc/wino4_body.h b/lass_amd/csrc/wino4_body.h
--- /dev/null
+++ b/lass_amd/csrc/wino4_body.h
@@ -0,0 +1,417 @@
+    constexpr bool PRO = (FLAGS & F_PRO) != 0, EPI = (FLAGS & F_EPIACT) != 0, SC = (FLAGS & F_PHASEB) != 0;
+    constexpr bool PRE = (FLAGS & F_PRECONV) != 0;
+    constexpr bool RESPRE = (FLAGS & F_RESPRE) != 0;
+    constexpr bool MASK = (FLAGS & F_MASK) != 0;
+    constexpr bool RES = (FLAGS & F_RES) != 0;
+    static_assert(!SC || (FLAGS & F_BIAS) != 0, "the shortcut conv has a bias");
+    static_assert(!PRE || PRO, "pre_conv is folded into the prologue's affine");
+    static_assert(!RESPRE || ((FLAGS & F_RES) != 0 && !SC && !EPI), "conv2 with the identity residual");
+    static_assert(!MASK || SC, "the output head sits behind decoder_block6's conv2 + shortcut");
+    static_assert(!RES || (!SC && !EPI), "conv2 with a residual in place of the fused shortcut");
+    constexpr bool SPLIT = (FLAGS & F_SPLITK) != 0;
+    static_assert(!SPLIT || (FLAGS & ~(F_SPLITK | F_PRO)) == 0, "a split launch has a prologue at most");
+    constexpr int TR = 32 / TC;
+    constexpr int OR_ = 4 * TR, OC = 4 * TC;
+    constexpr int NCO = 32;
+    __shared__ __attribute__((aligned(16))) float lds[U_F + V_F + 2 * NCO + (MASK ? 100 : 0)];
+    float* lu = lds;
+    float* lv = lds + U_F;
+    float* lds_es = lv + V_F;
+    float* lds_eh = lds_es + NCO;
+    float* lds_mw = lds_eh + NCO;
+
+    const int tid = threadIdx.x;
+    const int lane = tid & 63, wave = __builtin_amdgcn_readfirstlane(tid >> 6);
+    const int wco = wave >> 1, wwt = wave & 1;
+    int bx_, by_, b, ks = 0;
+    if constexpr (SPLIT) {
+        const unsigned lin = blockIdx.x, ngrp = (unsigned)(p.gx * p.B * sk.n);
+        unsigned grp;
+        if (p.xcd_map) {
+            const unsigned j = lin >> 3;
+            grp = (lin & 7u) * (ngrp >> 3) + j / (unsigned)p.gy;
+            by_ = (int)(j % (unsigned)p.gy);
+        } else {
+            grp = lin / (unsigned)p.gy;
+            by_ = (int)(lin % (unsigned)p.gy);
+        }
+        ks = (int)(grp % (unsigned)sk.n);
+        const unsigned xz = grp / (unsigned)sk.n;
+        b = (int)(xz / (unsigned)p.gx);
+        bx_ = (int)(xz % (unsigned)p.gx);
+    } else {
+        block_coords(p, bx_, by_, b);
+    }
+    const int n0 = by_ * NCO;
+    const int tiles_x = p.W / OC;
+    const int y0 = (bx_ / tiles_x) * OR_, x0 = (bx_ % tiles_x) * OC;
+    const int HW = p.H * p.W;
+    const float* in_b = p.in + (size_t)b * p.in_bs;
+    const float* sc = PRO ? p.pro_scale : nullptr;
+    const float* sh = PRO ? p.pro_shift + (size_t)b * p.pro_shift_bs : nullptr;
+
+    if (EPI && tid < NCO) {
+        lds_es[tid] = p.epi_scale[n0 + tid];
+        lds_eh[tid] = p.epi_shift[(size_t)b * p.epi_shift_bs + n0 + tid];
+    }
+    if (SC && tid < NCO) lds_es[tid] = p.bias[n0 + tid];
+    if (RESPRE && tid < 32) {
+        lds_es[tid] = p.pre_w[n0 + tid];
+        lds_eh[tid] = p.pre_b[n0 + tid];
+    }
+    if (MASK && tid < 99) lds_mw[tid] = tid < 96 ? p.mask_w[tid] : p.mask_b[tid - 96];
+
+    f32x4 acc[NXI];
+#pragma unroll
+    for (int xi = 0; xi < NXI; ++xi)
+#pragma unroll
+        for (int r = 0; r < 4; ++r) acc[xi][r] = 0.f;
+
+    const int kq = lane >> 4, l15 = lane & 15;
+    const float* afrag = lu + (wco >> 1) * U_F + (wco & 1) * 128 + (kq * 16 + l15) * 2;
+    const float* bfrag = lv + (kq * 32 + ((wwt * 16 + l15) ^ ((kq & 1) << 4))) * 2;
+    const unsigned slab_pitch = (unsigned)(p.Nw / 32) * (unsigned)(U_F * 4);
+    const unsigned slab_n0 = (unsigned)(n0 / 32) * (unsigned)(U_F * 4);
+    const unsigned lu_addr = (unsigned)(size_t)(__attribute__((address_space(3))) float*)lu;
+    const unsigned ulane = (unsigned)lane * 16u;
+    const v4i32 uw = make_rsrc_words(p.w_wino4, (unsigned)(NXI * p.Cin * p.Nw) * 4u);
+
+    const int pt = tid & 31, c8 = (tid & 255) >> 5;
+    const int pty = pt / TC, ptx = pt % TC;
+    const int gy0 = y0 + 4 * pty - 1, gx0 = x0 + 4 * ptx - 1;
+    const bool left = gx0 < 0, right = gx0 + 5 >= p.W;
+    unsigned vo_c[6], vo_l[6], vo_r[6], rowok = 0;
+#pragma unroll
+    for (int i = 0; i < 6; ++i) {
+        const int gy = gy0 + i;
+        const int row = (PRE ? 0 : c8 * HW) + min(max(gy, 0), p.H - 1) * p.W;
+        vo_c[i] = 4u * (unsigned)(row + gx0 + 1);
+        vo_l[i] = 4u * (unsigned)(row + (left ? 0 : gx0));
+        vo_r[i] = 4u * (unsigned)(row + (right ? p.W - 1 : gx0 + 5));
+        rowok |= (gy >= 0 && gy < p.H ? 1u : 0u) << i;
+    }
+    const __amdgpu_buffer_rsrc_t in_rsrc =
+        __builtin_amdgcn_make_buffer_rsrc(const_cast<float*>(in_b), 0, (int)((unsigned)(PRE ? 1 : p.Cin) * (unsigned)HW * 4u), 0x00020000);
+    const bool edge = left || right || rowok != 0x3fu;
+    float4 pc[6];
+    float pl[6], pr[6], ps = 1.f, ph = 0.f;
+    const unsigned tvo = (unsigned)c8 * 4u;
+    const auto tab_rsrc = [&](const float* t, int n) {
+        return __builtin_amdgcn_make_buffer_rsrc(const_cast<float*>(t), 0, n * 4, 0x00020000);
+    };
+    const __amdgpu_buffer_rsrc_t sc_rsrc = tab_rsrc(PRO ? sc : p.in, p.Cin), sh_rsrc = tab_rsrc(PRO ? sh : p.in, p.Cin);
+    const __amdgpu_buffer_rsrc_t pw_rsrc = tab_rsrc(PRE ? p.pre_w : p.in, 32), pb_rsrc = tab_rsrc(PRE ? p.pre_b : p.in, 32);
+    auto pload = [&](int ch) {
+        const unsigned soff = PRE ? 0u : (unsigned)(ch * KC * HW) * 4u;
+        if (!PRE || ch == 0)
+#pragma unroll
+        for (int i = 0; i < 6; ++i) {
+            pc[i] = __builtin_bit_cast(float4, __builtin_amdgcn_raw_buffer_load_b128(in_rsrc, (int)vo_c[i], (int)soff, 0));
+            pl[i] = __builtin_bit_cast(float, __builtin_amdgcn_raw_buffer_load_b32(in_rsrc, (int)vo_l[i], (int)soff, 0));
+            pr[i] = __builtin_bit_cast(float, __builtin_amdgcn_raw_buffer_load_b32(in_rsrc, (int)vo_r[i], (int)soff, 0));
+        }
+        const unsigned toff = (unsigned)(ch * KC) * 4u;
+        if (PRO) {
+            ps = __builtin_bit_cast(float, __builtin_amdgcn_raw_buffer_load_b32(sc_rsrc, (int)tvo, (int)toff, 0));
+            ph = __builtin_bit_cast(float, __builtin_amdgcn_raw_buffer_load_b32(sh_rsrc, (int)tvo, (int)toff, 0));
+        }
+        if (PRE) {
+            const float pw = __builtin_bit_cast(float, __builtin_amdgcn_raw_buffer_load_b32(pw_rsrc, (int)tvo, (int)toff, 0));
+            const float pb = __builtin_bit_cast(float, __builtin_amdgcn_raw_buffer_load_b32(pb_rsrc, (int)tvo, (int)toff, 0));
+            ph = fmaf(pb, ps, ph);
+            ps = pw * ps;
+        }
+    };
+    constexpr int NLOAD = (PRE ? 0 : 6 * 3) + (PRO ? 2 : 0) + (PRE ? 2 : 0);
+    float* vdst = lv + ((c8 & 3) * 32 + (pt ^ ((c8 & 1) << 4))) * 2 + (c8 >> 2);
+    auto pprocess = [&]() {
+        float d[6][6];
+#pragma unroll
+        for (int i = 0; i < 6; ++i) {
+            const float v[6] = {pl[i], pc[i].x, pc[i].y, pc[i].z, pc[i].w, pr[i]};
+#pragma unroll
+            for (int jx = 0; jx < 6; ++jx) d[i][jx] = PRO ? leaky(fmaf(v[jx], ps, ph)) : v[jx];
+        }
+        if (__builtin_amdgcn_ballot_w64(edge) != 0) {
+            const bool r0 = (rowok & 1u) != 0, r5 = (rowok & 32u) != 0;
+#pragma unroll
+            for (int jx = 0; jx < 6; ++jx) {
+                d[0][jx] = r0 ? d[0][jx] : 0.f;
+                d[5][jx] = r5 ? d[5][jx] : 0.f;
+            }
+#pragma unroll
+            for (int i = 0; i < 6; ++i) {
+                d[i][0] = left ? 0.f : d[i][0];
+                d[i][5] = right ? 0.f : d[i][5];
+            }
+        }
+        float tt[6][6];
+#pragma unroll
+        for (int jx = 0; jx < 6; ++jx) {
+            const float col[6] = {d[0][jx], d[1][jx], d[2][jx], d[3][jx], d[4][jx], d[5][jx]};
+            float r[6];
+            bt6(col, r);
+#pragma unroll
+            for (int i = 0; i < 6; ++i) tt[i][jx] = r[i];
+        }
+#pragma unroll
+        for (int i = 0; i < 6; ++i) {
+            float r[6];
+            bt6(tt[i], r);
+#pragma unroll
+            for (int jx = 0; jx < 6; ++jx) vdst[(i * 6 + jx) * 256] = r[jx];
+        }
+    };
+
+    const int ch0 = SPLIT ? ks * (p.Cin / KC) / sk.n : 0;
+    const int nch = SPLIT ? (ks + 1) * (p.Cin / KC) / sk.n : p.Cin / KC;
+    pload(ch0);
+    lds_barrier();
+    for (int ch = ch0; ch < nch; ++ch) {
+        lds_barrier();
+        __builtin_amdgcn_s_setprio(2);
+#pragma unroll
+        for (int i = 0; i < 6; ++i) {
+            asm volatile("" : "+v"(pc[i].x), "+v"(pc[i].y), "+v"(pc[i].z), "+v"(pc[i].w), "+v"(pl[i]), "+v"(pr[i]));
+        }
+        if (PRO) asm volatile("" : "+v"(ps), "+v"(ph));
+#pragma unroll
+        for (int i = 0; i < 9; ++i) {
+            const unsigned piece = (unsigned)(wave * 9 + i) * 1024u;
+            lds_dma_16B(uw, ulane, (unsigned)ch * slab_pitch + slab_n0 + piece, lu_addr + piece);
+        }
+        __builtin_amdgcn_sched_barrier(0);
+        pprocess();
+        __builtin_amdgcn_sched_barrier(0);
+        const bool pf = ch + 1 < nch;
+        if (pf) pload(ch + 1);
+        __builtin_amdgcn_sched_barrier(0);
+        if (pf)
+            wait_vmcnt<NLOAD>();
+        else
+            wait_vmcnt<0>();
+        lds_barrier();
+        __builtin_amdgcn_s_setprio(0);
+        constexpr int PFD = 2;
+        f32x2v av[PFD + 1][2], bv[PFD + 1][2];
+        auto rd = [&](int s) {
+#pragma unroll
+            for (int q = 0; q < 2; ++q) {
+                av[s % (PFD + 1)][q] = *reinterpret_cast<const f32x2v*>(afrag + (2 * s + q) * 256);
+                bv[s % (PFD + 1)][q] = *reinterpret_cast<const f32x2v*>(bfrag + (2 * s + q) * 256);
+            }
+        };
+#pragma unroll
+        for (int s = 0; s < PFD; ++s) rd(s);
+#pragma unroll
+        for (int s = 0; s < NXI / 2; ++s) {
+            if (s + PFD < NXI / 2) rd(s + PFD);
+            __builtin_amdgcn_sched_barrier(0);
+            const f32x2v a0 = av[s % (PFD + 1)][0], a1 = av[s % (PFD + 1)][1];
+            const f32x2v b0 = bv[s % (PFD + 1)][0], b1 = bv[s % (PFD + 1)][1];
+            acc[2 * s] = __builtin_amdgcn_mfma_f32_16x16x4f32(a0.x, b0.x, acc[2 * s], 0, 0, 0);
+            acc[2 * s + 1] = __builtin_amdgcn_mfma_f32_16x16x4f32(a1.x, b1.x, acc[2 * s + 1], 0, 0, 0);
+            acc[2 * s] = __builtin_amdgcn_mfma_f32_16x16x4f32(a0.y, b0.y, acc[2 * s], 0, 0, 0);
+            acc[2 * s + 1] = __builtin_amdgcn_mfma_f32_16x16x4f32(a1.y, b1.y, acc[2 * s + 1], 0, 0, 0);
+            __builtin_amdgcn_sched_barrier(0);
+        }
+    }
+
+    const int ot = wwt * 16 + l15;
+    const int oy = y0 + 4 * (ot / TC), ox = x0 + 4 * (ot % TC);
+    f32x4 ysp[16];
+#pragma unroll
+    for (int r = 0; r < 4; ++r) {
+        const int nl = wco * 16 + kq * 4 + r;
+        float tmp[4][6];
+#pragma unroll
+        for (int jx = 0; jx < 6; ++jx) {
+            const float m[6] = {acc[0 + jx][r], acc[6 + jx][r], acc[12 + jx][r], acc[18 + jx][r], acc[24 + jx][r], acc[30 + jx][r]};
+            float y[4];
+            at6(m, y);
+#pragma unroll
+            for (int a = 0; a < 4; ++a) tmp[a][jx] = y[a];
+        }
+        const float es = (EPI || SC) ? lds_es[nl] : 0.f, eh = EPI ? lds_eh[nl] : 0.f;
+#pragma unroll
+        for (int a = 0; a < 4; ++a) {
+            float y[4];
+            at6(tmp[a], y);
+#pragma unroll
+            for (int c = 0; c < 4; ++c) {
+                float v = y[c];
+                if (EPI) v = leaky(fmaf(v, es, eh));
+                if (SC) v += es;
+                ysp[a * 4 + c][r] = v;
+            }
+        }
+    }
+    if constexpr (SPLIT) {
+#pragma unroll
+        for (int r = 0; r < 4; ++r) {
+            const int n = n0 + wco * 16 + kq * 4 + r;
+            float* dst = sk.part + (((size_t)ks * p.B + b) * p.N + n) * HW + (size_t)oy * p.W + ox;
+#pragma unroll
+            for (int a = 0; a < 4; ++a) {
+                const float4 o = make_float4(ysp[a * 4 + 0][r], ysp[a * 4 + 1][r], ysp[a * 4 + 2][r], ysp[a * 4 + 3][r]);
+                if (oy + a < p.H) *reinterpret_cast<float4*>(dst + (size_t)a * p.W) = o;
+            }
+        }
+        return;
+    }
+    if constexpr (RESPRE) {
+        const float* xr = p.res + (size_t)b * p.res_bs + (size_t)min(oy, p.H - 4) * p.W + ox;
+        float4 xv[4];
+#pragma unroll
+        for (int a = 0; a < 4; ++a) xv[a] = *reinterpret_cast<const float4*>(xr + (size_t)a * p.W);
+#pragma unroll
+        for (int r = 0; r < 4; ++r) {
+            const float pw = lds_es[wco * 16 + kq * 4 + r], pb = lds_eh[wco * 16 + kq * 4 + r];
+#pragma unroll
+            for (int a = 0; a < 4; ++a) {
+                ysp[a * 4 + 0][r] += fmaf(xv[a].x, pw, pb);
+                ysp[a * 4 + 1][r] += fmaf(xv[a].y, pw, pb);
+                ysp[a * 4 + 2][r] += fmaf(xv[a].z, pw, pb);
+                ysp[a * 4 + 3][r] += fmaf(xv[a].w, pw, pb);
+            }
+        }
+    }
+    if constexpr (RES && !RESPRE) {
+        float4 rv[4][4];
+#pragma unroll
+        for (int r = 0; r < 4; ++r) {
+            const float* rr = p.res + (size_t)b * p.res_bs + (size_t)(n0 + wco * 16 + kq * 4 + r) * HW + (size_t)min(oy, p.H - 4) * p.W + ox;
+#pragma unroll
+            for (int a = 0; a < 4; ++a) rv[r][a] = *reinterpret_cast<const float4*>(rr + (size_t)a * p.W);
+        }
+#pragma unroll
+        for (int r = 0; r < 4; ++r)
+#pragma unroll
+            for (int a = 0; a < 4; ++a) {
+                ysp[a * 4 + 0][r] += rv[r][a].x;
+                ysp[a * 4 + 1][r] += rv[r][a].y;
+                ysp[a * 4 + 2][r] += rv[r][a].z;
+                ysp[a * 4 + 3][r] += rv[r][a].w;
+            }
+    }
+    if constexpr (SC) {
+        const float* x2 = p.in2 + (size_t)b * p.in2_bs + (size_t)min(oy, p.H - 4) * p.W + ox;
+        const float* wsc = p.w2 + n0 + wco * 16 + l15;
+        const int nks = p.Cin2 / 4;
+        constexpr int NSB = 4;
+        float4 xb[NSB][4];
+        float wa[NSB];
+        auto ldk = [&](int ks, int buf) {
+            const float* xp = x2 + (size_t)(4 * ks + kq) * HW;
+#pragma unroll
+            for (int a = 0; a < 4; ++a) xb[buf][a] = *reinterpret_cast<const float4*>(xp + (size_t)a * p.W);
+            wa[buf] = wsc[(size_t)(4 * ks + kq) * p.Nw];
+        };
+        auto mmk = [&](int buf) {
+#pragma unroll
+            for (int a = 0; a < 4; ++a) {
+                ysp[a * 4 + 0] = __builtin_amdgcn_mfma_f32_16x16x4f32(wa[buf], xb[buf][a].x, ysp[a * 4 + 0], 0, 0, 0);
+                ysp[a * 4 + 1] = __builtin_amdgcn_mfma_f32_16x16x4f32(wa[buf], xb[buf][a].y, ysp[a * 4 + 1], 0, 0, 0);
+                ysp[a * 4 + 2] = __builtin_amdgcn_mfma_f32_16x16x4f32(wa[buf], xb[buf][a].z, ysp[a * 4 + 2], 0, 0, 0);
+                ysp[a * 4 + 3] = __builtin_amdgcn_mfma_f32_16x16x4f32(wa[buf], xb[buf][a].w, ysp[a * 4 + 3], 0, 0, 0);
+            }
+        };
+        ldk(0, 0);
+        ldk(1, 1);
+        ldk(2, 2);
+        for (int ks = 0; ks < nks; ks += NSB) {
+#pragma unroll
+            for (int u = 0; u < NSB; ++u) {
+                ldk(min(ks + u + 3, nks - 1), (u + 3) % NSB);
+                __builtin_amdgcn_sched_barrier(0);
+                mmk(u);
+                __builtin_amdgcn_sched_barrier(0);
+            }
+        }
+    }
+    if constexpr (MASK) {
+        float* part = lds;
+        lds_barrier();
+#pragma unroll
+        for (int q = 0; q < 3; ++q) {
+            float w4[4];
+#pragma unroll
+            for (int r = 0; r < 4; ++r) w4[r] = lds_mw[q * 32 + wco * 16 + kq * 4 + r];
+#pragma unroll
+            for (int a = 0; a < 4; ++a) {
+                float4 o;
+                float* op = &o.x;
+#pragma unroll
+                for (int c = 0; c < 4; ++c) {
+                    const f32x4 v = ysp[a * 4 + c];
+                    op[c] = v[0] * w4[0] + v[1] * w4[1] + v[2] * w4[2] + v[3] * w4[3];
+                }
+                *reinterpret_cast<float4*>(part + ((wco * 4 + kq) * 3 + q) * 512 + ot * 16 + a * 4) = o;
+            }
+        }
+        lds_barrier();
+        const int px = tid * 2;
+        const int mt = px >> 4, ms = px & 15;
+        const int my = y0 + 4 * (mt / TC) + (ms >> 2), mx = x0 + 4 * (mt % TC) + (ms & 3);
+        float lg[3][2];
+#pragma unroll
+        for (int q = 0; q < 3; ++q) {
+            float2 sum = make_float2(lds_mw[96 + q], lds_mw[96 + q]);
+#pragma unroll
+            for (int src = 0; src < 8; ++src) {
+                const float2 v = *reinterpret_cast<const float2*>(part + (src * 3 + q) * 512 + px);
+                sum.x += v.x;
+                sum.y += v.y;
+            }
+            lg[q][0] = sum.x;
+            lg[q][1] = sum.y;
+        }
+        if (my < p.mask_T) {
+            mask_pixel(p, b, my, mx, lg[0][0], lg[1][0], lg[2][0]);
+            mask_pixel(p, b, my, mx + 1, lg[0][1], lg[1][1], lg[2][1]);
+        }
+        return;
+    }
+#pragma unroll
+    for (int r = 0; r < 4; ++r) {
+        const int n = n0 + wco * 16 + kq * 4 + r;
+        float* dst = p.out + (size_t)b * p.out_bs + (size_t)n * HW + (size_t)oy * p.W + ox;
+#pragma unroll
+        for (int a = 0; a < 4; ++a) {
+            const float4 o = make_float4(ysp[a * 4 + 0][r], ysp[a * 4 + 1][r], ysp[a * 4 + 2][r], ysp[a * 4 + 3][r]);
+            if (oy + a < p.H) *reinterpret_cast<float4*>(dst + (size_t)a * p.W) = o;
+        }
+        if constexpr (TC == 4 && RES) {
+            if (p.pool_out && p.pool_h == 1) {
+                const int Wo = p.W / 2;
+                float* pd = p.pool_out + (size_t)b * (p.pool_bs ? (size_t)p.pool_bs : (size_t)p.N * p.H * Wo) + (size_t)n * p.H * Wo +
+                            (size_t)oy * Wo + (ox >> 1);
+#pragma unroll
+                for (int a = 0; a < 4; ++a) {
+                    float2 o;
+                    o.x = (ysp[a * 4 + 0][r] + ysp[a * 4 + 1][r]) * 0.5f;
+                    o.y = (ysp[a * 4 + 2][r] + ysp[a * 4 + 3][r]) * 0.5f;
+                    if (oy + a < p.H) *reinterpret_cast<float2*>(pd + (size_t)a * Wo) = o;
+                }
+                continue;
+            }
+        }
+        if ((SC || RES) && p.pool_out) {
+            const int Ho = p.H / 2, Wo = p.W / 2;
+            float* pd = p.pool_out + (size_t)b * (p.pool_bs ? (size_t)p.pool_bs : (size_t)p.N * Ho * Wo) + (size_t)n * Ho * Wo +
+                        (size_t)(oy >> 1) * Wo + (ox >> 1);
+#pragma unroll
+            for (int i = 0; i < 2; ++i) {
+                float2 o;
+                float s0 = ysp[(2 * i) * 4 + 0][r] + ysp[(2 * i) * 4 + 1][r];
+                s0 += ysp[(2 * i + 1) * 4 + 0][r];
+                s0 += ysp[(2 * i + 1) * 4 + 1][r];
+                float s1 = ysp[(2 * i) * 4 + 2][r] + ysp[(2 * i) * 4 + 3][r];
+                s1 += ysp[(2 * i + 1) * 4 + 2][r];
+                s1 += ysp[(2 * i + 1) * 4 + 3][r];
+                o.x = s0 * 0.25f;
+                o.y = s1 * 0.25f;
+                if (oy + 2 * i + 1 < p.H) *reinterpret_cast<float2*>(pd + (size_t)i * Wo) = o;
+            }
+        }
+    }
```
